# Perception4D/LidarSlam

Hardware: AMD Instinct MI355X
Metric: LiDAR frames/sec (AddFrame end-to-end), VLS-128 scan (higher is better)
Workload: dtype f32+f64; 1 GPU; VLS-128 synthetic spinning scan, street canyon, 5 m/s, EgoMotion=MOTION_EXTRAPOLATION_AND_REGISTRATION, Undistortion=REFINED, library defaults; points_per_frame=255802, sequences=1, parallelism=1 sequence per GPU x 1, frames_resident_in_hbm=False

## Files before the change

### include/lidarslam_amd.h

```cpp
#ifndef LIDARSLAM_AMD_H
#define LIDARSLAM_AMD_H

#include <stddef.h>
#include <stdint.h>

#ifdef __cplusplus
extern "C" {
#endif

#define LSA_OK 0
#define LSA_E_NO_DEVICE (-1)
#define LSA_E_HIP (-2)
#define LSA_E_ARG (-3)
#define LSA_E_STATE (-4)
#define LSA_E_CAPACITY (-5)
#define LSA_E_GATE (-6)

#define LSA_EDGE 0
#define LSA_PLANE 1
#define LSA_BLOB 2

typedef struct lsa_point_t
{
  float x, y, z, w;
// ... 151 lines not shown

int lsa_download_match(lsa_ctx* ctx, int type, uint8_t* status, double* weights, double* records, int capacity);
int lsa_upload_match(lsa_ctx* ctx, int type, const uint8_t* status, const double* records, int n, double saturation);
#define LSA_KNN_MAX 16
int lsa_download_knn(lsa_ctx* ctx, int type, int* idx, float* d2, int* cnt, int capacity);

int lsa_accumulate(lsa_ctx* ctx, unsigned type_mask, const double w[6], int want_jacobian, double* cost, double g[6],
                   double H[36], int* n_valid);
int lsa_mailbox_active(const lsa_ctx* ctx);

int lsa_solve(lsa_ctx* ctx, unsigned type_mask, const double prior[16], int lm_max_iter, int two_d_mode, double optimized[16],
              int summary[4], double costs[2]);
typedef struct lsa_solve_result
{
  double pose[6];
  double initial_cost, final_cost;
  double cost, g[6], H[36];
  int num_successful_steps;
  int num_unsuccessful_steps;
  int num_iterations;
  int num_evaluations;
  int num_matches;
  int skipped;
  int termination;
  const char* message;
} lsa_solve_result_t;
int lsa_solve_device(lsa_ctx* ctx, unsigned type_mask, const double prior[6], int two_d_mode, int lm_max_iter, int min_matches,
                     lsa_solve_result_t* out);
int lsa_solve_device_begin(lsa_ctx* ctx, unsigned type_mask, const double prior[6], int two_d_mode, int lm_max_iter, int min_matches);
int lsa_solve_device_end(lsa_ctx* ctx, lsa_solve_result_t* out);
int lsa_solve_device_drop(lsa_ctx* ctx);

int lsa_icp_gate(lsa_ctx* ctx);
int lsa_icp_post(lsa_ctx* ctx, int ticket, const double pose[16], const double prior[6], const double H0[16], const double H1[16], double t0, double t1);
int lsa_icp_cancel(lsa_ctx* ctx, int ticket);
int lsa_icp_abandon(lsa_ctx* ctx);
int lsa_match_types_gated(lsa_ctx* ctx, int slot, unsigned type_mask, int query_set, const lsa_match_params_t* p, int undistort);

typedef struct lsa_icp_link
{
  int refine_undistortion;
  int first;
  int have_log;
  double prev_time, cur_time;
  double max_extrapolation_ratio;
  double previous_world[16];
  double motion[16];
} lsa_icp_link_t;
int lsa_icp_link(lsa_ctx* ctx);
int lsa_solve_device_begin_linked(lsa_ctx* ctx, unsigned type_mask, const double prior[6], int two_d_mode, int lm_max_iter, int min_matches,
                                  int leave_ticket, const lsa_icp_link_t* link);
int lsa_icp_link_peek(lsa_ctx* ctx, int ticket, unsigned long long words[64]);
int lsa_icp_link_expected(const double x[6], int skipped, int successful_steps, const lsa_icp_link_t* link, unsigned long long words[64], double motion_after[16]);

int lsa_solve_device_trace(lsa_ctx* ctx, unsigned long long out[12]);
int lsa_debug_set(lsa_ctx* ctx, const char* name, int value);
int lsa_solve_device_shape(const lsa_ctx* ctx, int out[4]);
int lsa_accumulate_shape(const lsa_ctx* ctx, int out[4]);
int lsa_solve_device_fallbacks(const lsa_ctx* ctx);
int lsa_solve_device_interlude(lsa_ctx* ctx, void (*fn)(void*), void* arg);
int lsa_registration_error(lsa_ctx* ctx, unsigned type_mask, const double pose[16], int two_d_mode, double cov[36], double err[2]);

typedef struct lsa_sensor_terms_t
{
  int wheel;
  double wheel_weight;
  double p[3];
  double d;
  int gravity;
  double gravity_weight;
  double g_ref[3];
  double g_cur[3];
} lsa_sensor_terms_t;
int lsa_set_sensor_terms(lsa_ctx* ctx, const lsa_sensor_terms_t* terms);
int lsa_sensor_terms_eval(const lsa_sensor_terms_t* terms, const double w[6], double sums[29]);

typedef struct lsa_sensors lsa_sensors;
lsa_sensors* lsa_sensors_create(void);
void lsa_sensors_destroy(lsa_sensors* s);
int lsa_sensors_add_wheel_odom(lsa_sensors* s, double time, double distance);
int lsa_sensors_add_gravity(lsa_sensors* s, double time, const double acc[3]);
int lsa_sensors_set_weights(lsa_sensors* s, double wheel_weight, double gravity_weight);
int lsa_sensors_set_time_offset(lsa_sensors* s, double offset);
int lsa_sensors_clear(lsa_sensors* s);
int lsa_sensors_compute(lsa_sensors* s, double lidar_time, lsa_sensor_terms_t* out);
int lsa_sensors_gravity_ref(const lsa_sensors* s, double g[3]);


int lsa_reset_working_keypoints(lsa_ctx* ctx);

int lsa_undistort(lsa_ctx* ctx, const double H0[16], const double H1[16], double t0, double t1);

int lsa_localization_begin(lsa_ctx* ctx, const double H0[16], const double H1[16], double t0, double t1, const double box_pose[16]);
int lsa_arm_localization_boxes(lsa_ctx* ctx);

int lsa_working_time_range(lsa_ctx* ctx, double* tmin, double* tmax);
int lsa_keypoint_time_range(lsa_ctx* ctx, int set, double* tmin, double* tmax);
int lsa_working_bbox(lsa_ctx* ctx, int type, const double pose[16], float mn[3], float mx[3]);
int lsa_working_bboxes(lsa_ctx* ctx, const double pose[16], float mn[9], float mx[9]);
int lsa_keypoint_bboxes_begin(lsa_ctx* ctx, int set, const double pose[16]);
int lsa_keypoint_bboxes_begin_interp(lsa_ctx* ctx, int set, const double H0[16], const double H1[16], double t0, double t1);
int lsa_keypoint_bboxes_end(lsa_ctx* ctx, float mn[9], float mx[9]);
int lsa_keypoint_boxes_predicted_mark(lsa_ctx* ctx);
int lsa_keypoint_boxes_predicted(lsa_ctx* ctx, int set, const double H0[16], const double H1[16], double t0, double t1);

int lsa_download_transformed(lsa_ctx* ctx, int set, int type, const double pose[16], lsa_point_t* out, int capacity);
// ... 50 lines not shown
int lsa_slam_add_frames(lsa_slam* s, const lsa_point_t* const* pts, const int* n, const uint64_t* stamp_us, const uint32_t* seq, int nframes);
int lsa_slam_set_extractor_param(lsa_slam* s, int device_id, const char* name, double value);
int lsa_slam_get_extractor_param(const lsa_slam* s, int device_id, const char* name, double* value);
int lsa_slam_set_base_to_lidar_offset(lsa_slam* s, const double T[16], int device_id);
int lsa_slam_get_base_to_lidar_offset(const lsa_slam* s, double T[16], int device_id);
int lsa_slam_set_world_transform_from_guess(lsa_slam* s, const double T[16]);
int lsa_slam_get_trajectory(const lsa_slam* s, double* poses, double* covariances, int capacity);
int lsa_slam_get_debug_information(lsa_slam* s, double out[10]);
int lsa_slam_get_map(lsa_slam* s, int type, int clean, lsa_point_t* out, int capacity);
int lsa_slam_get_target_submap(lsa_slam* s, int type, lsa_point_t* out, int capacity);
lsa_ctx* lsa_slam_context(lsa_slam* s);
int lsa_slam_add_wheel_odom_measurement(lsa_slam* s, double time, double distance);
int lsa_slam_add_gravity_measurement(lsa_slam* s, double time, const double acc[3]);
int lsa_slam_clear_sensor_measurements(lsa_slam* s);
int lsa_slam_sensor_terms(const lsa_slam* s, lsa_sensor_terms_t* out);
int lsa_slam_add_map_points(lsa_slam* s, int type, const lsa_point_t* pts, int n, int fixed, double time);
int lsa_slam_save_maps_pcd(lsa_slam* s, const char* prefix, int format, int filtered);
int lsa_slam_load_maps_pcd(lsa_slam* s, const char* prefix, int reset_maps, double time);
int lsa_slam_map_io_counts(const lsa_slam* s, int counts[3]);
int lsa_slam_set_trajectory_and_rebuild_maps(lsa_slam* s, const double* poses17, int n);
int lsa_slam_logged_frames(const lsa_slam* s);
int lsa_slam_get_logged_keypoints(lsa_slam* s, int frame, int type, lsa_point_t* out, int capacity);


typedef struct lsa_device_grid lsa_device_grid;
int lsa_device_grid_create(lsa_ctx* ctx, lsa_device_grid** out);
void lsa_device_grid_destroy(lsa_device_grid* g);
int lsa_device_grid_set(lsa_device_grid* g, const char* name, double value);
double lsa_device_grid_get_param(const lsa_device_grid* g, const char* name);
int lsa_device_grid_reset(lsa_device_grid* g, const float position[3]);
int lsa_device_grid_clear(lsa_device_grid* g);
int lsa_device_grid_size(lsa_device_grid* g);
int lsa_device_grid_add(lsa_device_grid* g, const lsa_point_t* pts, int n, int fixed, double time, int roll);
int lsa_device_grid_add_keypoints(lsa_device_grid* g, int set, int type, const double pose[16], double time);
int lsa_device_grid_stage_keypoints(lsa_device_grid* g, int set, int type, const double pose[16]);
int lsa_device_grid_add_staged(lsa_device_grid* g, double time);
int lsa_device_grid_stage_keypoints_all(lsa_device_grid* const* grids, const int* types, int count, int set, const double pose[16]);
int lsa_device_grid_add_staged_all(lsa_device_grid* const* grids, int count, double time);
int lsa_device_grid_roll(lsa_device_grid* g, const float min_point[3], const float max_point[3]);
int lsa_device_grid_clear_old_points(lsa_device_grid* g, double current_time);
int lsa_device_grid_get(lsa_device_grid* g, int clean, lsa_point_t* out, int capacity);
int lsa_device_grid_build_submap(lsa_device_grid* g, const float min_point[3], const float max_point[3], int min_nb_points, int slot, int type);
int lsa_device_grid_build_submap_begin(lsa_device_grid* g, const float min_point[3], const float max_point[3], int min_nb_points, int slot, int type);
int lsa_device_grid_build_submap_begin_for_keypoints(lsa_device_grid* g, int box_type, int min_nb_points, int slot, int type);
int lsa_device_grid_build_submap_end(lsa_device_grid* g);
int lsa_device_grid_submap_valid(lsa_device_grid* g);
int lsa_device_grid_submap_ahead_begin(lsa_device_grid* g, int box_type, int min_nb_points, int type);
int lsa_device_grid_submap_ahead_poll(lsa_device_grid* g);
int lsa_device_grid_submap_ahead_poll_all(lsa_device_grid* const* grids, int count);
int lsa_device_grid_submap_ahead_wait(lsa_device_grid* g);
int lsa_device_grid_submap_ahead_take(lsa_device_grid* g, int box_type, int min_nb_points, int slot, int type, int* taken);
int lsa_device_grid_submap_ahead_take_begin(lsa_device_grid* g, int box_type, int min_nb_points, int slot, int type);
int lsa_device_grid_submap_ahead_take_end(lsa_device_grid* g, int* taken);
int lsa_device_grid_add_pcd(lsa_device_grid* g, const char* path, int fixed, double time, int roll_first);
int lsa_device_grid_save_pcd(lsa_device_grid* g, const char* path, int format, int clean);
int lsa_pcd_io_times(const lsa_ctx* ctx, double out[8]);

int lsa_kplog_append(lsa_ctx* ctx);
int lsa_kplog_append_points(lsa_ctx* ctx, const lsa_point_t* const pts[3], const int n[3]);
int lsa_kplog_pop_front(lsa_ctx* ctx);
int lsa_kplog_clear(lsa_ctx* ctx);
int lsa_kplog_size(const lsa_ctx* ctx);
int lsa_kplog_count(const lsa_ctx* ctx, int frame, int type);
int lsa_kplog_get(lsa_ctx* ctx, int frame, int type, lsa_point_t* out, int capacity);
unsigned long long lsa_kplog_bytes(const lsa_ctx* ctx);
int lsa_kplog_stopped(const lsa_ctx* ctx);
int lsa_kplog_replay(lsa_ctx* ctx, unsigned type_mask, const double* poses, const double* times, int n, int undistort, lsa_point_t* const out[3],
                     float last_min[3][3], float last_max[3][3]);
long long lsa_kplog_replayed(const lsa_ctx* ctx, int type, const lsa_point_t** pts);
int lsa_kplog_replay_to_grids(lsa_ctx* ctx, unsigned type_mask, const double* poses, const double* times, int n, int undistort, lsa_device_grid* const grids[3],
                              float last_min[3][3], float last_max[3][3]);

typedef struct lsa_rolling_grid lsa_rolling_grid;
lsa_rolling_grid* lsa_rolling_grid_create(void);
void lsa_rolling_grid_destroy(lsa_rolling_grid* g);
int lsa_rolling_grid_set(lsa_rolling_grid* g, const char* name, double value);
void lsa_rolling_grid_reset(lsa_rolling_grid* g, const float position[3]);
void lsa_rolling_grid_clear(lsa_rolling_grid* g);
int lsa_rolling_grid_size(const lsa_rolling_grid* g);
void lsa_rolling_grid_roll(lsa_rolling_grid* g, const float min_point[3], const float max_point[3]);
int lsa_rolling_grid_add(lsa_rolling_grid* g, const lsa_point_t* pts, int n, int fixed, double current_time, int roll);
void lsa_rolling_grid_clear_old_points(lsa_rolling_grid* g, double current_time);
int lsa_rolling_grid_get(const lsa_rolling_grid* g, int clean, lsa_point_t* out, int capacity);
int lsa_rolling_grid_build_submap(lsa_rolling_grid* g, const float min_point[3], const float max_point[3], int min_nb_points);
int lsa_rolling_grid_submap_valid(const lsa_rolling_grid* g);
int lsa_rolling_grid_submap(const lsa_rolling_grid* g, lsa_point_t* out, int capacity);

int lsa_pcd_info(const char* path, int* n, int* format);
int lsa_pcd_read(const char* path, lsa_point_t* out, int capacity);
int lsa_pcd_write(const char* path, const lsa_point_t* pts, int n, int format);
const char* lsa_pcd_last_error(void);
int lsa_lzf_compress(const void* in, size_t n, void* out, size_t capacity, size_t* written);
int lsa_lzf_decompress(const void* in, size_t n, void* out, size_t capacity, size_t* written);

int lsa_synth_sensor(int model, int* nrings, int* ncols, double* el_min_deg, double* el_max_deg);
int lsa_synth_frame(int model, uint64_t seed, int frame, lsa_point_t* out, int capacity, uint64_t* stamp_us);
void lsa_synth_pose(int frame, double T[16]);

#ifdef __cplusplus
}
#endif
#endif
```

### lidarslam_amd/__init__.py

```python
import ctypes as C
import os

import numpy as np

from ._native import (
    BLOB,
    EDGE,
    LIB_PATH,
    MATCH_NSTATUS,
    PLANE,
    POINT_DTYPE,
    SET_RAW_CURRENT,
    SET_RAW_PREVIOUS,
    SET_WORKING,
    ExtractParams,
    KernelStat,
    MatchParams,
    pose16,
    ptr,
    synth_frame,
    synth_pose,
)

__all__ = ["Context", "Slam", "ExtractParams", "MatchParams", "POINT_DTYPE", "lib", "LsaError", "read_pcd", "write_pcd"]

TARGET_MAP, TARGET_PREVIOUS = 0, 1
KNN_MAX = 16

DEBUG_INFORMATION_NAMES = [
    "EgoMotion: edges used", "EgoMotion: planes used", "Localization: edges used", "Localization: planes used",
    "Localization: blobs used", "Localization: position error", "Localization: orientation error",
    "Confidence: overlap", "Confidence: comply motion limits", "latency",
]

DEBUG_NAMES = [
    "sin_angle", "saliency", "depth_gap", "intensity_gap", "edge_keypoint", "plane_keypoint", "blob_keypoint",
    "edge_validity", "plane_validity", "blob_validity",
]

ABI_SYMBOLS = [
    "lsa_device_count", "lsa_bind_host_to_device", "lsa_ctx_create", "lsa_ctx_destroy", "lsa_last_error", "lsa_sync", "lsa_upload_frame", "lsa_upload_wire_frame", "lsa_upload_polydata_frame",
    "lsa_frame_store_put", "lsa_frame_store_use", "lsa_frame_size", "lsa_get_azimuthal_resolution",
    "lsa_set_azimuthal_resolution", "lsa_extract_keypoints", "lsa_extract_keypoints_more", "lsa_extract_prefetch", "lsa_extract_prefetch_adopted", "lsa_transform_frame_at", "lsa_set_keypoint_types", "lsa_download_keypoints", "lsa_keypoint_count",
    "lsa_download_debug", "lsa_nb_laser_rings", "lsa_transform_keypoints", "lsa_set_target", "lsa_set_target_from_set", "lsa_prepare_previous_targets", "lsa_prepared_targets_adopted", "lsa_target_staging", "lsa_set_target_staged", "lsa_stage_target_ahead", "lsa_drop_target_ahead", "lsa_staged_targets_adopted",
    "lsa_target_size", "lsa_download_target", "lsa_set_target_cell_size", "lsa_set_knn_lanes", "lsa_set_fused_match", "lsa_set_knn_rounds", "lsa_match_slow_queries", "lsa_match_exhaustive_queries", "lsa_match_route_stats", "lsa_match_trace", "lsa_set_keypoints", "lsa_match", "lsa_match_types", "lsa_match_types_undistorted",
    "lsa_download_match", "lsa_upload_match", "lsa_download_knn", "lsa_overlap", "lsa_accumulate", "lsa_mailbox_active", "lsa_solve", "lsa_solve_device", "lsa_solve_device_fallbacks", "lsa_solve_device_begin", "lsa_solve_device_end", "lsa_solve_device_drop", "lsa_icp_gate", "lsa_icp_link", "lsa_solve_device_begin_linked", "lsa_icp_link_peek", "lsa_icp_link_expected", "lsa_icp_post", "lsa_icp_cancel", "lsa_icp_abandon", "lsa_debug_set", "lsa_solve_device_shape", "lsa_accumulate_shape", "lsa_match_types_gated", "lsa_solve_device_trace", "lsa_registration_error", "lsa_selftest_math", "lsa_selftest_numerics", "lsa_selftest_labels", "lsa_reset_working_keypoints", "lsa_undistort", "lsa_working_time_range",
    "lsa_working_bbox", "lsa_working_bboxes", "lsa_localization_begin", "lsa_arm_localization_boxes", "lsa_keypoint_bboxes_begin", "lsa_keypoint_bboxes_begin_interp", "lsa_keypoint_boxes_predicted_mark", "lsa_keypoint_boxes_predicted", "lsa_keypoint_time_range", "lsa_keypoint_bboxes_end", "lsa_download_transformed", "lsa_stage_transformed", "lsa_staged_transformed", "lsa_transform_frame", "lsa_profile_enable", "lsa_profile_select", "lsa_profile_reset",
    "lsa_profile_get", "lsa_slam_create", "lsa_slam_destroy", "lsa_slam_last_error", "lsa_slam_set_param",
    "lsa_slam_get_param", "lsa_slam_reset", "lsa_slam_clear_maps", "lsa_slam_add_frame", "lsa_slam_store_frame", "lsa_slam_add_stored_frame", "lsa_slam_hint_next_stored_frame", "lsa_slam_hint_next_frame", "lsa_upload_frame_begin", "lsa_upload_frame_ready", "lsa_upload_frame_adopt", "lsa_upload_frame_forget", "lsa_profile_event_overhead_us", "lsa_upload_robosense_frame", "lsa_pin_host_memory", "lsa_unpin_host_memory", "lsa_collect_garbage", "lsa_uploads_adopted", "lsa_extract_prefetch_uploaded",
    "lsa_slam_get_world_transform", "lsa_slam_get_covariance", "lsa_slam_get_keypoints", "lsa_slam_get_registered_frame",
    "lsa_slam_get_match_status", "lsa_slam_get_stats", "lsa_slam_context", "lsa_slam_get_latency_compensated_world_transform",
    "lsa_slam_set_world_transform_from_guess", "lsa_slam_get_trajectory", "lsa_slam_get_debug_information", "lsa_slam_get_map",
    "lsa_slam_get_target_submap", "lsa_slam_set_base_to_lidar_offset", "lsa_slam_get_base_to_lidar_offset", "lsa_slam_add_frames", "lsa_slam_set_extractor_param", "lsa_slam_get_extractor_param", "lsa_match_serial", "lsa_match_histogram", "lsa_synth_sensor", "lsa_synth_frame",
    "lsa_synth_pose",
    "lsa_selftest_keep_busy", "lsa_solve_device_interlude", "lsa_device_grid_create", "lsa_device_grid_destroy", "lsa_device_grid_set", "lsa_device_grid_get_param", "lsa_device_grid_reset", "lsa_device_grid_clear",
    "lsa_device_grid_size", "lsa_device_grid_add", "lsa_device_grid_add_keypoints", "lsa_device_grid_roll", "lsa_device_grid_clear_old_points",
    "lsa_device_grid_get", "lsa_device_grid_build_submap", "lsa_device_grid_submap_valid", "lsa_device_grid_stage_keypoints", "lsa_device_grid_stage_keypoints_all", "lsa_device_grid_add_staged", "lsa_device_grid_add_staged_all",
    "lsa_device_grid_build_submap_begin", "lsa_device_grid_build_submap_begin_for_keypoints", "lsa_device_grid_build_submap_end",
    "lsa_device_grid_submap_ahead_begin", "lsa_device_grid_submap_ahead_poll", "lsa_device_grid_submap_ahead_poll_all", "lsa_device_grid_submap_ahead_wait", "lsa_device_grid_submap_ahead_take", "lsa_device_grid_submap_ahead_take_begin", "lsa_device_grid_submap_ahead_take_end",
    "lsa_rolling_grid_create", "lsa_rolling_grid_destroy", "lsa_rolling_grid_set", "lsa_rolling_grid_reset", "lsa_rolling_grid_clear",
    "lsa_rolling_grid_size", "lsa_rolling_grid_roll", "lsa_rolling_grid_add", "lsa_rolling_grid_clear_old_points", "lsa_rolling_grid_get",
    "lsa_rolling_grid_build_submap", "lsa_rolling_grid_submap_valid", "lsa_rolling_grid_submap",
    "lsa_set_sensor_terms", "lsa_sensor_terms_eval", "lsa_sensors_create", "lsa_sensors_destroy", "lsa_sensors_add_wheel_odom",
    "lsa_sensors_add_gravity", "lsa_sensors_set_weights", "lsa_sensors_set_time_offset", "lsa_sensors_clear", "lsa_sensors_compute",
    "lsa_sensors_gravity_ref", "lsa_slam_add_wheel_odom_measurement", "lsa_slam_add_gravity_measurement",
    "lsa_slam_clear_sensor_measurements", "lsa_slam_sensor_terms",
    "lsa_pcd_info", "lsa_pcd_read", "lsa_pcd_write", "lsa_pcd_last_error", "lsa_lzf_compress", "lsa_lzf_decompress",
    "lsa_device_grid_add_pcd", "lsa_device_grid_save_pcd", "lsa_pcd_io_times",
    "lsa_slam_add_map_points", "lsa_slam_save_maps_pcd", "lsa_slam_load_maps_pcd", "lsa_slam_map_io_counts",
    "lsa_kplog_append", "lsa_kplog_append_points", "lsa_kplog_pop_front", "lsa_kplog_clear", "lsa_kplog_size", "lsa_kplog_count", "lsa_kplog_get",
    "lsa_kplog_bytes", "lsa_kplog_stopped", "lsa_kplog_replay", "lsa_kplog_replayed", "lsa_kplog_replay_to_grids",
    "lsa_slam_set_trajectory_and_rebuild_maps", "lsa_slam_logged_frames", "lsa_slam_get_logged_keypoints",
]

PCD_ASCII, PCD_BINARY, PCD_BINARY_COMPRESSED = 0, 1, 2
PCD_FORMAT_NAMES = ["ascii", "binary", "binary_compressed"]


class LsaError(RuntimeError):
    code = None


E_NO_DEVICE, E_HIP, E_ARG, E_STATE, E_CAPACITY = -1, -2, -3, -4, -5


def _error(what, rc, message):
    e = LsaError(f"{what} failed ({rc}): {message}")
    e.code = rc
    return e


class IcpLink(C.Structure):

    _fields_ = [
        ("refine_undistortion", C.c_int), ("first", C.c_int), ("have_log", C.c_int),
        ("prev_time", C.c_double), ("cur_time", C.c_double), ("max_extrapolation_ratio", C.c_double),
        ("previous_world", C.c_double * 16), ("motion", C.c_double * 16),
    ]

# ... 1241 lines not shown
```

### lidarslam_amd/csrc/host/lsa_slam_core.cpp

```cpp
#include "lsa_slam_core.h"
#include <algorithm>
#include <chrono>
#include <cmath>
#include <cstdlib>
#include <cstdio>
#include <cstring>
#include <ctime>
#include "lsa_pcd.h"

namespace lsa
{
namespace host
{
constexpr unsigned kChainMax = 6;
namespace
{
#define ICP_TRACE(...) do { if (lsa_icp_trace_on()) std::fprintf(stderr, __VA_ARGS__); } while (0)
struct Tick
{
  std::chrono::steady_clock::time_point t0 = std::chrono::steady_clock::now();
  double Stop() const { return std::chrono::duration<double>(std::chrono::steady_clock::now() - t0).count(); }
};
inline double StampToSec(uint64_t us) { return us * 1e-6; }
}
// ... 529 lines not shown
  return lsa_prepare_previous_targets(Ctx, (1u << LSA_EDGE) | (1u << LSA_PLANE));
}

lsa_match_params_t SlamCore::EgoMatchParams() const
{
  lsa_match_params_t p;
  std::memset(&p, 0, sizeof(p));
  p.single_edge_per_ring = 1;
  p.max_neighbors_distance = EgoMotionMaxNeighborsDistance;
  p.edge_nb_neighbors = EgoMotionEdgeNbNeighbors;
  p.edge_min_nb_neighbors = EgoMotionEdgeMinNbNeighbors;
  p.edge_max_model_error = EgoMotionEdgeMaxModelError;
  p.plane_nb_neighbors = EgoMotionPlaneNbNeighbors;
  p.planarity_threshold = EgoMotionPlanarityThreshold;
  p.plane_max_model_error = EgoMotionPlaneMaxModelError;
  p.blob_nb_neighbors = 10;
  p.saturation_distance = 1.;
  return p;
}
lsa_match_params_t SlamCore::LocMatchParams() const
{
  lsa_match_params_t p;
  std::memset(&p, 0, sizeof(p));
  p.single_edge_per_ring = 0;
  p.max_neighbors_distance = LocalizationMaxNeighborsDistance;
  p.edge_nb_neighbors = LocalizationEdgeNbNeighbors;
  p.edge_min_nb_neighbors = LocalizationEdgeMinNbNeighbors;
  p.edge_max_model_error = LocalizationEdgeMaxModelError;
  p.plane_nb_neighbors = LocalizationPlaneNbNeighbors;
  p.planarity_threshold = LocalizationPlanarityThreshold;
  p.plane_max_model_error = LocalizationPlaneMaxModelError;
  p.blob_nb_neighbors = LocalizationBlobNbNeighbors;
  p.saturation_distance = 1.;
  return p;
}

struct SlamCore::IcpLoopSpec
{
  const char* name;
  int target, set;
  unsigned matchMask, solveMask;
  unsigned maxIter, lmMaxIter;
  double initSaturation, finalSaturation;
  lsa_match_params_t match;
  int loopBit;
  bool linksOk, gatesOk;
  int undistortAhead;
  lsa_icp_link_t link;
  long long* matchSerial;
  double FrameStats::*icpSeconds;
  double FrameStats::*lmSeconds;
  int FrameStats::*iterations;
  bool countSkippedEvals;
};
struct SlamCore::IcpUndistortion
{
  Pose d0 = Pose::Identity(), d1 = Pose::Identity();
  bool pending = false;
  bool posted = false;
};

namespace
{
constexpr auto kNothing = [](auto&&...) { return LSA_OK; };
const bool kAheadWithHostMaps = std::getenv("LSA_ICP_AHEAD_HOSTMAPS") != nullptr;
const int kAheadLoops = std::getenv("LSA_ICP_AHEAD_LOOPS") ? std::atoi(std::getenv("LSA_ICP_AHEAD_LOOPS")) : 3;
const bool kGateDebug = std::getenv("LSA_GATE_DEBUG") != nullptr;
}

template <class Top, class Enqueued, class Solved, class Skipped, class Accepted, class Finished>
int SlamCore::RunIcpLoop(const IcpLoopSpec& spec, Pose& pose, const Top& top, const Enqueued& enqueued, const Solved& solved, const Skipped& skipped,
                         const Accepted& accepted, const Finished& finished)
{
  TotalMatchedKeypoints = 0;
  lsa_match_params_t mp = spec.match;
  auto saturation = [&](unsigned icpIter) {
    const double iterRatio = icpIter / static_cast<double>(spec.maxIter - 1);
    return (1 - iterRatio) * spec.initSaturation + iterRatio * spec.finalSaturation;
  };
  const bool aheadOk = ICPAhead >= 1 && DeviceLM && FusedMatch && (kAheadLoops & spec.loopBit);
  bool chain = aheadOk && ICPAhead >= 2 && spec.maxIter <= kChainMax && spec.linksOk;
  bool ahead = aheadOk && !chain && spec.gatesOk;
  if (ahead || chain) lsa_icp_abandon(Ctx);
  unsigned chained = 0;
  long long chainSerial[kChainMax][3] = {};
  bool enqueuedAhead = false;
  long long aheadSerial[3] = {0, 0, 0};
  int ticket = -1;
  IcpUndistortion undistortion;
  unsigned icpIter = 0;

  auto callOffRest = [&](bool all) {
    if (ticket >= 0)
    {
      lsa_icp_cancel(Ctx, ticket);
      lsa_solve_device_drop(Ctx);
      ticket = -1;
    }
    if (all || icpIter + 1 < chained)
    {
      lsa_icp_abandon(Ctx);
      chained = 0;
    }
  };
  struct AtExit { decltype(callOffRest)& callOffRest; bool failed; ~AtExit() { callOffRest(failed); } } atExit{callOffRest, true};

  auto takeSerials = [&](long long* serial) {
    for (int k = 0; k < 3; ++k)
      if ((spec.matchMask >> k) & 1u) serial[k] = lsa_match_serial(Ctx, k);
  };
  auto setSerials = [&](const long long* serial) {
    for (int k = 0; k < 3; ++k)
      if ((spec.matchMask >> k) & 1u) spec.matchSerial[k] = serial[k];
  };
  auto matchInLine = [&]() -> int {
    if (undistortion.pending)
      LSA_TRY(lsa_match_types_undistorted(Ctx, spec.target, spec.matchMask, &mp, pose.m, nullptr, undistortion.d0.m, undistortion.d1.m, Motion.Time0, Motion.Time1));
    else
      LSA_TRY(lsa_match_types(Ctx, spec.target, spec.matchMask, spec.set, &mp, pose.m, nullptr));
    undistortion.pending = false;
    takeSerials(spec.matchSerial);
    return LSA_OK;
  };
  auto matchAhead = [&](unsigned iter, long long* serial) -> int {
    lsa_match_params_t next = mp;
    next.saturation_distance = saturation(iter);
    const int rc = lsa_match_types_gated(Ctx, spec.target, spec.matchMask, spec.set, &next, spec.undistortAhead);
    if (rc == 0) takeSerials(serial);
    return rc;
  };

  for (; icpIter < spec.maxIter; ++icpIter)
  {
    Tick ticp;
    if (const int rc = top(icpIter); rc < 0) return rc;
    mp.saturation_distance = saturation(icpIter);
    LocalOptimizer optimizer(Ctx);
    optimizer.SetDeviceLoop(DeviceLM);
    optimizer.SetTwoDMode(TwoDMode);
    optimizer.SetLMMaxIter(spec.lmMaxIter);
    optimizer.SetMinMatches(MinNbMatchedKeypoints);
    optimizer.UseDeviceResiduals(spec.solveMask);
    optimizer.SetPosePrior(pose);
    bool begun = enqueuedAhead;
    if (icpIter < chained)
    {
      begun = true;
      setSerials(chainSerial[icpIter]);
    }
    else if (!enqueuedAhead)
    {
      if (const int rc = matchInLine(); rc < 0) return rc;
      if (chain)
      {
        double prior[6];
        ToXYZRPY(pose, prior);
        lsa_icp_link_t link = spec.link;
        for (unsigned j = icpIter; j < spec.maxIter; ++j)
        {
          int leave = j + 1 < spec.maxIter ? lsa_icp_link(Ctx) : -1;
          if (leave < 0) leave = -1;
          link.first = j == icpIter ? 1 : 0;
          const int rc = lsa_solve_device_begin_linked(Ctx, spec.solveMask, j == icpIter ? prior : nullptr, TwoDMode ? 1 : 0, static_cast<int>(spec.lmMaxIter), static_cast<int>(MinNbMatchedKeypoints), leave,
                                                       leave >= 0 ? &link : nullptr);
          if (rc < 0) return Fail(rc, "lsa_solve_device_begin_linked");
          chained = j + 1;
          if (leave < 0) break;
          const int mrc = matchAhead(j + 1, chainSerial[j + 1]);
          if (mrc < 0) return Fail(mrc, "lsa_match_types_gated");
          if (mrc != 0) { lsa_icp_cancel(Ctx, leave); break; }
        }
        chain = false;
        begun = true;
      }
      else if (ahead)
      {
        LSA_TRY(optimizer.Begin(false));
        begun = true;
      }
    }
    else
      setSerials(aheadSerial);
    ICP_TRACE("[%s %u] top: ahead %d begun %d enqueued %d\n", spec.name, icpIter, (int)ahead, (int)begun, (int)enqueuedAhead);
    enqueuedAhead = false;
    if (ahead && begun && icpIter + 1 < spec.maxIter)
    {
      ticket = lsa_icp_gate(Ctx);
      ICP_TRACE("[%s %u] gate ticket %d\n", spec.name, icpIter, ticket);
      if (ticket < 0) { ticket = -1; ahead = false; }
      else
      {
        const char* call = "lsa_match_types_gated";
        int rc = matchAhead(icpIter + 1, aheadSerial);
        if (rc == 0)
        {
          call = "lsa_solve_device_begin";
          rc = lsa_solve_device_begin(Ctx, spec.solveMask, nullptr, TwoDMode ? 1 : 0, static_cast<int>(spec.lmMaxIter), static_cast<int>(MinNbMatchedKeypoints));
        }
        if (rc != 0)
        {
          lsa_icp_cancel(Ctx, ticket);
          ticket = -1;
          ahead = false;
          if (rc < 0) return Fail(rc, call);
        }
      }
    }
    if (const int rc = enqueued(icpIter); rc < 0) return rc;
    if (!begun) ArmLookaheadInterlude();
    Stats.*spec.icpSeconds += ticp.Stop();
    (Stats.*spec.iterations)++;

    Tick tlm;
    SolveSummary summary;
    if (begun)
    {
      Tick tdbg;
      const int irc = InterludeWork();
      const double dbgInterlude = tdbg.Stop();
      int rc = optimizer.End(summary);
      ICP_TRACE("[%s %u] End rc %d irc %d ticket %d\n", spec.name, icpIter, rc, irc, ticket);
      if (kGateDebug && tdbg.Stop() > 0.01)
        std::fprintf(stderr, "[gate debug] %s iteration %u: enqueue %.3f ms, interlude %.3f ms, until the result %.3f ms, rc %d\n", spec.name, icpIter, 1e3 * Stats.*spec.icpSeconds, 1e3 * dbgInterlude,
                     1e3 * tdbg.Stop(), rc);
      if (rc == LSA_E_GATE)
      {
        callOffRest(true);
        ahead = false;
        IcpGateTimeouts++;
        undistortion.pending = undistortion.posted;
        rc = matchInLine();
        if (rc < 0) return rc;
        rc = optimizer.Solve(summary);
      }
      if (rc < 0) return Fail(rc, "LocalOptimizer::End / Solve");
      if (rc == 1) { ticket = -1; ahead = false; chained = 0; }
      if (irc < 0) return irc;
    }
    else
    {
      LSA_TRY(optimizer.Solve(summary));
      LSA_TRY(FinishLookaheadInterlude());
    }
    TotalMatchedKeypoints = summary.num_matches;
    if (lsa_icp_trace_on())
      std::fprintf(stderr, "[icp] frame %u %s %u: matches %d evals %d steps %d cost %.17g -> %.17g%s\n", NbrFrameProcessed, spec.name, icpIter, summary.num_matches, summary.num_evaluations,
                   summary.num_successful_steps, summary.initial_cost, summary.final_cost, summary.skipped ? " skipped" : "");
    if (const int rc = solved(); rc < 0) return rc;
    if (!summary.skipped || spec.countSkippedEvals) Stats.lm_evals += summary.num_evaluations;
    if (!summary.skipped) pose = optimizer.GetOptimizedPose();
    const bool last = summary.skipped || summary.num_successful_steps == 1 || icpIter + 1 == spec.maxIter;
    if (last) callOffRest(false);
    const int rc = summary.skipped ? skipped() : accepted(last, undistortion);
    Stats.*spec.lmSeconds += tlm.Stop();
    if (rc < 0) return rc;
    if (last)
    {
      if (const int frc = summary.skipped ? LSA_OK : finished(optimizer); frc < 0) return frc;
      break;
    }
    if (ticket >= 0)
    {
      double prior[6];
      ToXYZRPY(pose, prior);
      const int prc = lsa_icp_post(Ctx, ticket, pose.m, prior, undistortion.pending ? undistortion.d0.m : nullptr, undistortion.pending ? undistortion.d1.m : nullptr, Motion.Time0, Motion.Time1);
      if (prc < 0) return Fail(prc, "lsa_icp_post");
      ticket = -1;
      undistortion.posted = undistortion.pending;
      undistortion.pending = false;
      enqueuedAhead = true;
    }
    else if (icpIter + 1 < chained)
      undistortion.pending = false;
  }
  atExit.failed = false;
  return LSA_OK;
}

int SlamCore::DownloadMatchDebug(int set, unsigned typeMask, MatchDebug* debug)
{
  for (int k = 0; k < 3; ++k)
  {
    if (!((typeMask >> k) & 1u)) continue;
    const int n = lsa_keypoint_count(Ctx, set, k);
    debug[k].status.assign(n, LSA_MATCH_UNKOWN);
    debug[k].weights.assign(n, 0.);
    if (n > 0) LSA_TRY(lsa_download_match(Ctx, k, debug[k].status.data(), debug[k].weights.data(), nullptr, n));
  }
  return LSA_OK;
}

int SlamCore::ComputeEgoMotion()
{
  Tick tpre;
  Trelative = Pose::Identity();
  if (AheadStatus < 0) { const int rc = AheadStatus; AheadStatus = 0; return Fail(rc, "lsa_prepare_previous_targets (look-ahead thread)"); }
  if (LogTrajectory.size() >= 2 &&
      (EgoMotion == EgoMotionMode::MOTION_EXTRAPOLATION || EgoMotion == EgoMotionMode::MOTION_EXTRAPOLATION_AND_REGISTRATION))
  {
    const double t = StampToSec(CurrentStamp);
    const double t1 = LogTrajectory[LogTrajectory.size() - 1].time;
    const double t0 = LogTrajectory[LogTrajectory.size() - 2].time;
    if (!(std::abs((t - t1) / (t1 - t0)) > MaxExtrapolationRatio))
    {
      const Pose next = LinearInterpolation(PreviousTworld, Tworld, t, t0, t1);
      Trelative = Inverse(Tworld) * next;
    }
  }
  const bool registers = EgoMotion == EgoMotionMode::REGISTRATION || EgoMotion == EgoMotionMode::MOTION_EXTRAPOLATION_AND_REGISTRATION;
  {
    const int rc = BeginSubMapSpeculation(Tworld * Trelative);
    if (rc < 0) return rc;
    HoldLookahead = false;
  }
  if (!registers) return LSA_OK;

  for (int k : {LSA_EDGE, LSA_PLANE})
  {
    lsa_set_target_cell_size(Ctx, LSA_TARGET_PREVIOUS, k, static_cast<float>(k == LSA_EDGE ? KnnCellSizeEgoMotionEdges : KnnCellSizeEgoMotion));
    LSA_TRY(lsa_set_target_from_set(Ctx, LSA_TARGET_PREVIOUS, k, LSA_SET_RAW_PREVIOUS));
  }
  IcpLoopSpec spec = {};
  spec.name = "ego";
  spec.target = LSA_TARGET_PREVIOUS;
  spec.set = LSA_SET_RAW_CURRENT;
  spec.matchMask = spec.solveMask = (1u << LSA_EDGE) | (1u << LSA_PLANE);
  spec.maxIter = EgoMotionICPMaxIter;
  spec.lmMaxIter = EgoMotionLMMaxIter;
  spec.initSaturation = EgoMotionInitSaturationDistance;
  spec.finalSaturation = EgoMotionFinalSaturationDistance;
  spec.match = EgoMatchParams();
  spec.loopBit = 1;
  spec.linksOk = true;
  spec.gatesOk = DeviceMapsInUse() || MapUpdate == MappingMode::NONE || kAheadWithHostMaps;
  spec.matchSerial = EgoMatchSerial;
  spec.icpSeconds = &FrameStats::ego_icp;
  spec.lmSeconds = &FrameStats::ego_lm;
  spec.iterations = &FrameStats::ego_iters;
  spec.countSkippedEvals = true;
  auto enqueued = [&](unsigned icpIter) -> int {
    if (icpIter == 0 && BuildTargetsAhead)
    {
      AheadStatus = 0;
      AheadWorker.Submit([this] { AheadStatus = PrepareNextEgoMotionTargets(); });
    }
    if (!SpecPending) LSA_TRY(StageSpeculativeSubMaps());
    return LSA_OK;
  };
  auto solved = [&]() -> int { return SpecPending ? FinishSubMapSpeculation() : LSA_OK; };
  DbgAcc[2] += tpre.Stop();
  if (const int rc = RunIcpLoop(spec, Trelative, kNothing, enqueued, solved, kNothing, kNothing, kNothing); rc < 0) return rc;
  if (KeepMatchDebug) return DownloadMatchDebug(LSA_SET_RAW_CURRENT, spec.matchMask, EgoDebug);
  return LSA_OK;
}

int SlamCore::Localization()
{
  Tick tloc;
  struct AtExit { SlamCore* c; Tick* t; ~AtExit() { c->DbgAcc[5] += t->Stop() - (c->Stats.loc_icp + c->Stats.loc_lm + c->Stats.submap + c->Stats.undistort); } } atExit{this, &tloc};
  const bool sensorTerms = LocSensorTerms.wheel || LocSensorTerms.gravity;
  if (sensorTerms) lsa_set_sensor_terms(Ctx, &LocSensorTerms);
  struct SensorTermsGuard { lsa_ctx* ctx; bool on; ~SensorTermsGuard() { if (on) lsa_set_sensor_terms(ctx, nullptr); } } sensorGuard{Ctx, sensorTerms};
  PreviousTworld = Tworld;
  Tworld = PreviousTworld * Trelative;
  const bool oneLaunch = LocalizationStartFused && DeviceMapsInUse() && MapUpdate != MappingMode::NONE;
  bool boxesEnqueued = false;
  if (oneLaunch)
  {
    Tick t;
    Pose d0 = Pose::Identity(), d1 = Pose::Identity();
    if (Undistortion)
    {
      double t0, t1;
      LSA_TRY(lsa_keypoint_time_range(Ctx, LSA_SET_RAW_CURRENT, &t0, &t1));
      InitUndistortion(t0, t1);
      RefineUndistortion(&d0, &d1);
    }
    LSA_TRY(lsa_localization_begin(Ctx, Undistortion ? d0.m : nullptr, Undistortion ? d1.m : nullptr, Motion.Time0, Motion.Time1, Tworld.m));
    boxesEnqueued = true;
    Stats.undistort += t.Stop();
  }
  else
  {
    LSA_TRY(lsa_reset_working_keypoints(Ctx));
    if (Undistortion)
    {
      Tick t;
      int rc = InitUndistortion();
      if (rc < 0) return rc;
      rc = RefineUndistortion();
      if (rc < 0) return rc;
      Stats.undistort += t.Stop();
    }
  }

  if (DeviceMapsInUse())
  {
    Tick t;
    for (auto& w : MapWorker) w.Wait();
    {
      Tick tw;
      while (DevSpecRunning.load(std::memory_order_acquire)) std::this_thread::yield();
      const bool tried = DevSpec[0] || DevSpec[1] || DevSpec[2];
      if (tried && SubMapsAheadAdaptive && tw.Stop() > 80e-6)
      {
        DevSpecGood = 0;
        if (++DevSpecLate >= 2)
        {
          DevSpecBackoff = DevSpecPenalty;
          DevSpecPenalty = std::min(2 * DevSpecPenalty, 64);
          DevSpecLate = 0;
        }
      }
      else if (tried)
      {
        DevSpecLate = 0;
        if (++DevSpecGood >= 8) DevSpecPenalty = 4;
      }
    }
    Stats.maps_wait = t.Stop();
    if (DevSpecStatus < 0) { const int rc = DevSpecStatus; DevSpecStatus = 0; return Fail(rc, "sub-maps ahead of time (look-ahead thread)"); }
    Stats.maps_async = std::max(MapJobSeconds[0], std::max(MapJobSeconds[1], MapJobSeconds[2]));
    for (int k = 0; k < 3; ++k)
      if (MapJobFailed[k]) { MapJobFailed[k] = 0; return Fail(LSA_E_HIP, "lsa_device_grid_add_staged (map worker)"); }
    bool need[3], checking[3] = {false, false, false}, any = false;
    for (int k = 0; k < 3; ++k)
    {
      need[k] = UseKeypoints[k] && !lsa_device_grid_submap_valid(DevMaps[k]);
      any = any || need[k];
    }
    if (any && MapUpdate != MappingMode::NONE && !boxesEnqueued) LSA_TRY(lsa_keypoint_bboxes_begin(Ctx, LSA_SET_WORKING, Tworld.m));
    for (int k = 0; k < 3; ++k)
    {
      if (!need[k]) continue;
      lsa_set_target_cell_size(Ctx, LSA_TARGET_MAP, k, static_cast<float>((k == LSA_EDGE ? KnnCellScaleMapsEdges : KnnCellScaleMaps) * LocalMaps[k]->GetLeafSize()));
      if (MapUpdate == MappingMode::NONE) LSA_TRY(lsa_device_grid_build_submap_begin(DevMaps[k], nullptr, nullptr, -1, LSA_TARGET_MAP, k));
      else
      {
        if (DevSpec[k] && lsa_device_grid_submap_ahead_take_begin(DevMaps[k], k, KeypointCounts[k] / 2, LSA_TARGET_MAP, k) == 1) { checking[k] = true; continue; }
        if (LocalMaps[k]->IsTimeThreshold()) LSA_TRY(lsa_device_grid_clear_old_points(DevMaps[k], CurrentTime));
        LSA_TRY(lsa_device_grid_build_submap_begin_for_keypoints(DevMaps[k], k, KeypointCounts[k] / 2, LSA_TARGET_MAP, k));
      }
    }
    for (int k = 0; k < 3; ++k)
    {
      if (!checking[k]) continue;
      int taken = 0;
      LSA_TRY(lsa_device_grid_submap_ahead_take_end(DevMaps[k], &taken));
      if (taken) { need[k] = false; Stats.submap_spec_hits++; SubMapSpecHitsTotal++; continue; }
      if (LocalMaps[k]->IsTimeThreshold()) LSA_TRY(lsa_device_grid_clear_old_points(DevMaps[k], CurrentTime));
      LSA_TRY(lsa_device_grid_build_submap_begin_for_keypoints(DevMaps[k], k, KeypointCounts[k] / 2, LSA_TARGET_MAP, k));
    }
    for (bool& b : DevSpec) b = false;
    for (int k = 0; k < 3; ++k)
      if (need[k]) LSA_TRY(lsa_device_grid_build_submap_end(DevMaps[k]));
    Stats.submap += t.Stop();
    HoldLookahead = false;
  }
  else
  {
    Tick t;
    if (SpecPending)
    {
      const int rc = FinishSubMapSpeculation();
      if (rc < 0) return rc;
    }
    WaitMaps();
    Stats.maps_wait = t.Stop();
    Stats.maps_async = std::max(MapJobSeconds[0], std::max(MapJobSeconds[1], MapJobSeconds[2]));
    bool fresh[3], rebuild[3] = {false, false, false};
    bool any = false;
    for (int k = 0; k < 3; ++k)
    {
      fresh[k] = UseKeypoints[k] && SpecBuilt[k];
      rebuild[k] = UseKeypoints[k] && !fresh[k] && !LocalMaps[k]->IsSubMapValid();
      any = any || fresh[k] || rebuild[k];
      SpecBuilt[k] = false;
    }
    float mn[9], mx[9];
    if (any && MapUpdate != MappingMode::NONE) LSA_TRY(lsa_working_bboxes(Ctx, Tworld.m, mn, mx));
    for (int k = 0; k < 3; ++k)
    {
      const bool holds = fresh[k] && MapUpdate != MappingMode::NONE && LocalMaps[k]->SubMapBuiltFor(mn + 3 * k, mx + 3 * k, KeypointCounts[k] / 2);
      if (SpecStaged[k] && !holds) LSA_TRY(lsa_drop_target_ahead(Ctx, LSA_TARGET_MAP, k));
      SpecStaged[k] = false;
      SpecDone[k].store(false);
    }
    for (int k = 0; k < 3; ++k)
    {
      if (!fresh[k] && !rebuild[k]) continue;
      RollingGrid* map = LocalMaps[k].get();
      const int minPts = KeypointCounts[k] / 2;
      if (fresh[k])
      {
        if (map->SubMapBuiltFor(mn + 3 * k, mx + 3 * k, minPts)) { Stats.submap_spec_hits++; SubMapSpecHitsTotal++; rebuild[k] = true; continue; }
        rebuild[k] = true;
      }

      if (MapUpdate == MappingMode::NONE)
        MapWorker[k].Submit([map] { map->BuildSubMap(); });
      else
      {
        const bool clear = map->IsTimeThreshold();
        const double now = CurrentTime;
        const float* lo3 = mn + 3 * k;
        const float* hi3 = mx + 3 * k;
        MapWorker[k].Submit([map, clear, now, minPts, mn0 = lo3[0], mn1 = lo3[1], mn2 = lo3[2], mx0 = hi3[0], mx1 = hi3[1], mx2 = hi3[2]] {
          if (clear) map->ClearOldPoints(now);
          const float lo[3] = {mn0, mn1, mn2}, hi[3] = {mx0, mx1, mx2};
          map->BuildSubMap(lo, hi, minPts);
        });
      }
    }
    for (int k = 0; k < 3; ++k)
    {
      if (!rebuild[k]) continue;
      MapWorker[k].Wait();
      lsa_set_target_cell_size(Ctx, LSA_TARGET_MAP, k, static_cast<float>((k == LSA_EDGE ? KnnCellScaleMapsEdges : KnnCellScaleMaps) * LocalMaps[k]->GetLeafSize()));
      LSA_TRY(lsa_set_target_staged(Ctx, LSA_TARGET_MAP, k, static_cast<int>(LocalMaps[k]->SubMapSize())));
    }
    Stats.submap += t.Stop();
  }

  const bool refined = Undistortion == UNDISTORTION_REFINED;
  IcpLoopSpec spec = {};
  spec.name = "loc";
  spec.target = LSA_TARGET_MAP;
  spec.set = LSA_SET_WORKING;
  for (int k = 0; k < 3; ++k)
    if (UseKeypoints[k]) spec.matchMask |= 1u << k;
  spec.solveMask = 7u;
  spec.maxIter = LocalizationICPMaxIter;
  spec.lmMaxIter = LocalizationLMMaxIter;
  spec.initSaturation = LocalizationInitSaturationDistance;
  spec.finalSaturation = LocalizationFinalSaturationDistance;
  spec.match = LocMatchParams();
  spec.loopBit = 2;
  spec.linksOk = spec.gatesOk = !refined || UndistortInSearch;
  spec.undistortAhead = refined ? 1 : 0;
  spec.link.refine_undistortion = refined ? 1 : 0;
  spec.link.have_log = LogTrajectory.empty() ? 0 : 1;
  spec.link.prev_time = LogTrajectory.empty() ? 0. : LogTrajectory.back().time;
  spec.link.cur_time = StampToSec(CurrentStamp);
  spec.link.max_extrapolation_ratio = MaxExtrapolationRatio;
  std::memcpy(spec.link.previous_world, PreviousTworld.m, sizeof(spec.link.previous_world));
  {
    double* m = spec.link.motion;
    m[0] = Motion.Time0; m[1] = Motion.Time1;
    m[2] = Motion.Rot0.w; m[3] = Motion.Rot0.x; m[4] = Motion.Rot0.y; m[5] = Motion.Rot0.z;
    m[6] = Motion.Rot1.w; m[7] = Motion.Rot1.x; m[8] = Motion.Rot1.y; m[9] = Motion.Rot1.z;
    for (int i = 0; i < 3; ++i) { m[10 + i] = Motion.Trans0[i]; m[13 + i] = Motion.Trans1[i]; }
  }
  spec.matchSerial = LocMatchSerial;
  spec.icpSeconds = &FrameStats::loc_icp;
  spec.lmSeconds = &FrameStats::loc_lm;
  spec.iterations = &FrameStats::loc_iters;
  spec.countSkippedEvals = false;
  auto top = [&](unsigned icpIter) -> int {
    if (WorkerPrewake && DeviceMapsInUse() && icpIter + 1 == LocalizationICPMaxIter && MapUpdate != MappingMode::NONE) MapWorker[0].Expect(300e-6);
    return LSA_OK;
  };
  auto skipped = [&]() -> int {
    Trelative = Pose::Identity();
    Tworld = PreviousTworld;
    if (Undistortion) Motion.SetTransforms(Pose::Identity(), Pose::Identity());
    LastError = "Not enough keypoints matched, Localization skipped for this frame.";
    return LSA_OK;
  };
  auto accepted = [&](bool last, IcpUndistortion& undistortion) -> int {
    Trelative = Inverse(PreviousTworld) * Tworld;
    if (!refined) return LSA_OK;
    if (UndistortInSearch && !last)
    {
      undistortion.pending = true;
      return RefineUndistortion(&undistortion.d0, &undistortion.d1);
    }
    return RefineUndistortion();
  };
  auto finished = [&](LocalOptimizer& optimizer) -> int {
    Tick terr;
    LSA_TRY(optimizer.EstimateRegistrationError(LocalizationUncertainty));
    DbgAcc[4] += terr.Stop();
    return LSA_OK;
  };
  if (const int rc = RunIcpLoop(spec, Tworld, top, kNothing, kNothing, skipped, accepted, finished); rc < 0) return rc;
  if (KeepMatchDebug) return DownloadMatchDebug(LSA_SET_WORKING, 7u, LocDebug);
  return LSA_OK;
}

int SlamCore::BeginSubMapSpeculation(const Pose& predicted)
{
  SpecPending = false;
  for (bool& b : DevSpec) b = false;
  if (MapUpdate == MappingMode::NONE) return LSA_OK;
  const bool onDevice = DeviceMapsInUse();
  if (onDevice)
  {
    bool any = false;
    for (int k = 0; k < 3; ++k) any = any || (UseKeypoints[k] && KeypointCounts[k] > 0);
    if (!SubMapsAhead || !any || LocalMaps[0]->IsTimeThreshold()) return LSA_OK;
    if (DevSpecBackoff > 0) { --DevSpecBackoff; return LSA_OK; }
  }
  bool interpolated = false;
  Pose begin = predicted, end = predicted;
  double t0 = 0., t1 = 0.;
  if (Undistortion && !LogTrajectory.empty())
  {
    LSA_TRY(lsa_keypoint_time_range(Ctx, LSA_SET_RAW_CURRENT, &t0, &t1));
    const double prevPoseTime = LogTrajectory.back().time;
    const double currPoseTime = StampToSec(CurrentStamp);
    if (t1 - t0 >= 1e-6 && currPoseTime != prevPoseTime)
    {
      auto scanPose = [&](double time) {
        if (std::abs(time / (currPoseTime - prevPoseTime)) > MaxExtrapolationRatio) return predicted;
        return LinearInterpolation(Tworld, predicted, currPoseTime + time, prevPoseTime, currPoseTime);
      };
      begin = scanPose(t0);
      end = scanPose(t1);
      interpolated = true;
    }
  }
  if (onDevice)
  {
    int minPts[3];
    bool use[3];
    for (int k = 0; k < 3; ++k)
    {
      use[k] = UseKeypoints[k] && KeypointCounts[k] > 0;
      minPts[k] = KeypointCounts[k] / 2;
      if (use[k]) lsa_set_target_cell_size(Ctx, LSA_TARGET_MAP, k, static_cast<float>((k == LSA_EDGE ? KnnCellScaleMapsEdges : KnnCellScaleMaps) * LocalMaps[k]->GetLeafSize()));
      DevSpec[k] = use[k];
    }
    DevSpecStatus = 0;
    LSA_TRY(lsa_keypoint_boxes_predicted_mark(Ctx));
    DevSpecRunning.store(true, std::memory_order_release);
    AheadWorker.Submit([this, interpolated, begin, end, t0, t1, use0 = use[0], use1 = use[1], use2 = use[2], m0 = minPts[0], m1 = minPts[1], m2 = minPts[2]] {
      const bool use[3] = {use0, use1, use2};
      const int minPts[3] = {m0, m1, m2};
      for (auto& w : MapWorker) w.Wait();
// ... 506 lines not shown
  if (!HaveFrame) return 0;
  if (!CurrentFrames.empty())
  {
    size_t total = 0;
    for (const HeldFrame& f : CurrentFrames) total += static_cast<size_t>(f.n);
    out.resize(total);
    size_t at = 0;
    for (const HeldFrame& f : CurrentFrames)
    {
      LSA_TRY(lsa_frame_store_use(Ctx, f.slot));
      const Pose offset = GetBaseToLidarOffset(f.device);
      if (Undistortion)
      {
        const Pose H0 = (Tworld * Motion.GetH0()) * offset;
        const Pose H1 = (Tworld * Motion.GetH1()) * offset;
        LSA_TRY(lsa_transform_frame_at(Ctx, 1, H0.m, H1.m, Motion.Time0, Motion.Time1, f.timeOffset, out.data() + at, f.n));
      }
      else
      {
        const Pose tf = Tworld * offset;
        LSA_TRY(lsa_transform_frame_at(Ctx, 0, tf.m, nullptr, 0., 0., f.timeOffset, out.data() + at, f.n));
      }
      at += static_cast<size_t>(f.n);
    }
    return static_cast<int>(total);
  }
  const int n = lsa_frame_size(Ctx);
  if (n <= 0) return 0;
  out.resize(n);
  if (Undistortion)
  {
    const Pose H0 = (Tworld * Motion.GetH0()) * BaseToLidarOffset;
    const Pose H1 = (Tworld * Motion.GetH1()) * BaseToLidarOffset;
    LSA_TRY(lsa_transform_frame(Ctx, 1, H0.m, H1.m, Motion.Time0, Motion.Time1, out.data(), n));
  }
  else
  {
    const Pose tf = Tworld * BaseToLidarOffset;
    LSA_TRY(lsa_transform_frame(Ctx, 0, tf.m, nullptr, 0., 0., out.data(), n));
  }
  return n;
}

#define LSA_PARAMS(X)                                                                                   \
  X("UseBlobs", UseKeypoints[LSA_BLOB], bool)                                                          \
  X("UseEdges", UseKeypoints[LSA_EDGE], bool)                                                          \
  X("UsePlanes", UseKeypoints[LSA_PLANE], bool)                                                        \
  X("TwoDMode", TwoDMode, bool)                                                                        \
  X("BuildTargetsAhead", BuildTargetsAhead, bool)                                                      \
  X("DeviceLM", DeviceLM, bool)                                                                        \
  X("MapsOnDevice", MapsOnDevice, bool)                                                                \
  X("SubMapsAhead", SubMapsAhead, bool)                                                                \
  X("SubMapsAheadAdaptive", SubMapsAheadAdaptive, bool)                                                \
  X("LocalizationStartFused", LocalizationStartFused, bool)                                            \
  X("WorkerPrewake", WorkerPrewake, bool)                                                              \
  X("ICPAhead", ICPAhead, int)                                                                         \
  X("UndistortInSearch", UndistortInSearch, bool)                                                      \
  X("SpecBoxesOnLookahead", SpecBoxesOnLookahead, bool)                                                \
  X("SpecGridsTogether", SpecGridsTogether, bool)                                                      \
  X("FusedMatch", FusedMatch, bool)                                                                    \
  X("EgoMotionICPMaxIter", EgoMotionICPMaxIter, unsigned)                                              \
  X("LocalizationICPMaxIter", LocalizationICPMaxIter, unsigned)                                        \
  X("EgoMotionLMMaxIter", EgoMotionLMMaxIter, unsigned)                                                \
  X("LocalizationLMMaxIter", LocalizationLMMaxIter, unsigned)                                          \
  X("EgoMotionMaxNeighborsDistance", EgoMotionMaxNeighborsDistance, double)                            \
  X("LocalizationMaxNeighborsDistance", LocalizationMaxNeighborsDistance, double)                      \
  X("EgoMotionEdgeNbNeighbors", EgoMotionEdgeNbNeighbors, unsigned)                                    \
  X("EgoMotionEdgeMinNbNeighbors", EgoMotionEdgeMinNbNeighbors, unsigned)                              \
  X("EgoMotionEdgeMaxModelError", EgoMotionEdgeMaxModelError, double)                                  \
  X("EgoMotionPlaneNbNeighbors", EgoMotionPlaneNbNeighbors, unsigned)                                  \
  X("EgoMotionPlanarityThreshold", EgoMotionPlanarityThreshold, double)                                \
  X("EgoMotionPlaneMaxModelError", EgoMotionPlaneMaxModelError, double)                                \
  X("EgoMotionInitSaturationDistance", EgoMotionInitSaturationDistance, double)                        \
  X("EgoMotionFinalSaturationDistance", EgoMotionFinalSaturationDistance, double)                      \
  X("LocalizationEdgeNbNeighbors", LocalizationEdgeNbNeighbors, unsigned)                              \
  X("LocalizationEdgeMinNbNeighbors", LocalizationEdgeMinNbNeighbors, unsigned)                        \
  X("LocalizationEdgeMaxModelError", LocalizationEdgeMaxModelError, double)                            \
  X("LocalizationPlaneNbNeighbors", LocalizationPlaneNbNeighbors, unsigned)                            \
  X("LocalizationPlanarityThreshold", LocalizationPlanarityThreshold, double)                          \
  X("LocalizationPlaneMaxModelError", LocalizationPlaneMaxModelError, double)                          \
  X("LocalizationBlobNbNeighbors", LocalizationBlobNbNeighbors, unsigned)                              \
  X("LocalizationInitSaturationDistance", LocalizationInitSaturationDistance, double)                  \
  X("LocalizationFinalSaturationDistance", LocalizationFinalSaturationDistance, double)                \
  X("MaxExtrapolationRatio", MaxExtrapolationRatio, double)                                            \
  X("MinNbMatchedKeypoints", MinNbMatchedKeypoints, unsigned)                                          \
  X("KfDistanceThreshold", KfDistanceThreshold, double)                                                \
  X("KfAngleThreshold", KfAngleThreshold, double)                                                      \
  X("KeepMatchDebug", KeepMatchDebug, bool)                                                            \
  X("KnnCellSizeEgoMotion", KnnCellSizeEgoMotion, double)                                              \
  X("KnnCellScaleMaps", KnnCellScaleMaps, double)                                                      \
  X("KnnCellSizeEgoMotionEdges", KnnCellSizeEgoMotionEdges, double)                                    \
  X("KnnCellScaleMapsEdges", KnnCellScaleMapsEdges, double)                                            \
  X("KnnLanesEdges", KnnLanesEdges, int)                                                               \
  X("KnnLanesPlanes", KnnLanesPlanes, int)                                                             \
  X("KnnLanesBlobs", KnnLanesBlobs, int)                                                               \
  X("KnnRoundsEdges", KnnRoundsEdges, int)                                                             \
  X("KnnRoundsPlanes", KnnRoundsPlanes, int)                                                           \
  X("KnnRoundsBlobs", KnnRoundsBlobs, int)                                                             \
  X("NeighborWidth", ExtractParams.neighbor_width, int)                                                \
  X("MinDistanceToSensor", ExtractParams.min_distance_to_sensor, float)                                \
  X("MinBeamSurfaceAngle", ExtractParams.min_beam_surface_angle, float)                                \
  X("PlaneSinAngleThreshold", ExtractParams.plane_sin_angle_threshold, float)                          \
  X("EdgeSinAngleThreshold", ExtractParams.edge_sin_angle_threshold, float)                            \
  X("DistToLineThreshold", ExtractParams.dist_to_line_threshold, float)                                \
  X("EdgeDepthGapThreshold", ExtractParams.edge_depth_gap_threshold, float)                            \
  X("EdgeSaliencyThreshold", ExtractParams.edge_saliency_threshold, float)                             \
// ... 76 lines not shown
  auto dev = [&](int k, const char* what, double value) { if (DevMaps[k]) lsa_device_grid_set(DevMaps[k], what, value); };
  if (name == "VoxelGridLeafSizeEdges") { LocalMaps[LSA_EDGE]->SetLeafSize(v); dev(LSA_EDGE, "LeafSize", v); return LSA_OK; }
  if (name == "VoxelGridLeafSizePlanes") { LocalMaps[LSA_PLANE]->SetLeafSize(v); dev(LSA_PLANE, "LeafSize", v); return LSA_OK; }
  if (name == "VoxelGridLeafSizeBlobs") { LocalMaps[LSA_BLOB]->SetLeafSize(v); dev(LSA_BLOB, "LeafSize", v); return LSA_OK; }
  if (name == "VoxelGridSize") { for (int k = 0; k < 3; ++k) { LocalMaps[k]->SetGridSize(static_cast<int>(v)); dev(k, "GridSize", v); } return LSA_OK; }
  if (name == "VoxelGridResolution") { for (int k = 0; k < 3; ++k) { LocalMaps[k]->SetVoxelResolution(v); dev(k, "VoxelResolution", v); } return LSA_OK; }
  if (name == "VoxelGridMinFramesPerVoxel") { for (int k = 0; k < 3; ++k) { LocalMaps[k]->SetMinFramesPerVoxel(static_cast<unsigned>(v)); dev(k, "MinFramesPerVoxel", v); } return LSA_OK; }
  if (name == "VoxelGridDecayingThreshold") { for (int k = 0; k < 3; ++k) { LocalMaps[k]->SetDecayingThreshold(v); dev(k, "DecayingThreshold", v); } return LSA_OK; }
  if (name == "VoxelGridSamplingMode") { for (int k = 0; k < 3; ++k) { LocalMaps[k]->SetSampling(static_cast<SamplingMode>(static_cast<int>(v))); dev(k, "Sampling", v); } return LSA_OK; }
  if (name == "OrderedMaps")
  {
    OrderedMaps = v != 0;
    for (auto& m : LocalMaps) m->SetOrdered(OrderedMaps);
    for (int k = 0; k < 3; ++k)
      if (DevMaps[k] && lsa_device_grid_set(DevMaps[k], "Ordered", OrderedMaps ? 1. : 0.) != LSA_OK) return Fail(LSA_E_HIP, "lsa_device_grid_set(Ordered)");
    return LSA_OK;
  }
  LastError = "unknown parameter " + name;
  return LSA_E_ARG;
}

int SlamCore::GetParam(const std::string& name, double* v) const
{
  if (!v) return LSA_E_ARG;
#define X(NAME, MEMBER, TYPE) if (name == NAME) { *v = static_cast<double>(MEMBER); return LSA_OK; }
  LSA_PARAMS(X)
#undef X
  if (name == "EgoMotion") { *v = static_cast<int>(EgoMotion); return LSA_OK; }
  if (name == "Undistortion") { *v = static_cast<int>(Undistortion); return LSA_OK; }
  if (name == "MapUpdate") { *v = static_cast<int>(MapUpdate); return LSA_OK; }
  if (name == "WheelOdomWeight") { *v = SensorManagers.GetWheelOdomWeight(); return LSA_OK; }
  if (name == "GravityWeight") { *v = SensorManagers.GetGravityWeight(); return LSA_OK; }
  if (name == "SensorTimeOffset") { *v = SensorManagers.GetTimeOffset(); return LSA_OK; }
  if (name == "AzimuthalResolution") { *v = Ctx ? lsa_get_azimuthal_resolution(Ctx) : 0.; return LSA_OK; }
  if (name == "VoxelGridLeafSizeEdges") { *v = LocalMaps[LSA_EDGE]->GetLeafSize(); return LSA_OK; }
  if (name == "VoxelGridLeafSizePlanes") { *v = LocalMaps[LSA_PLANE]->GetLeafSize(); return LSA_OK; }
  if (name == "VoxelGridLeafSizeBlobs") { *v = LocalMaps[LSA_BLOB]->GetLeafSize(); return LSA_OK; }
  if (name == "VoxelGridSize") { *v = LocalMaps[0]->GetGridSize(); return LSA_OK; }
  if (name == "VoxelGridResolution") { *v = LocalMaps[0]->GetVoxelResolution(); return LSA_OK; }
  if (name == "VoxelGridSamplingMode") { *v = static_cast<int>(LocalMaps[0]->GetSampling()); return LSA_OK; }
  if (name == "VoxelGridDecayingThreshold") { *v = LocalMaps[0]->GetDecayingThreshold(); return LSA_OK; }
  if (name == "VoxelGridMinFramesPerVoxel") { *v = LocalMaps[0]->GetMinFramesPerVoxel(); return LSA_OK; }
  if (name == "NbrFrameProcessed") { *v = NbrFrameProcessed; return LSA_OK; }
  if (name == "TotalMatchedKeypoints") { *v = TotalMatchedKeypoints; return LSA_OK; }
  if (name == "OverlapSamplingRatio") { *v = OverlapSamplingRatio; return LSA_OK; }
  if (name == "OverlapEstimation") { *v = OverlapEstimation; return LSA_OK; }
  if (name == "SubMapSpeculationHits") { *v = SubMapSpecHitsTotal; return LSA_OK; }
  if (name == "LookaheadAdopted") { *v = Ctx ? lsa_extract_prefetch_adopted(Ctx) : 0; return LSA_OK; }
  if (name == "OrderedMaps") { *v = OrderedMaps ? 1. : 0.; return LSA_OK; }
  if (name == "DeviceMapsInUse") { *v = DeviceMapsInUse() ? 1. : 0.; return LSA_OK; }
  if (name == "UploadsAdopted") { *v = Ctx ? lsa_uploads_adopted(Ctx) : 0; return LSA_OK; }
  if (name == "DeviceSolveFallbacks") { *v = Ctx ? lsa_solve_device_fallbacks(Ctx) : 0; return LSA_OK; }
  if (name == "IcpGateTimeouts") { *v = IcpGateTimeouts; return LSA_OK; }
  if (name == "TargetsBuiltAheadAdopted") { *v = Ctx ? lsa_prepared_targets_adopted(Ctx) : 0; return LSA_OK; }
  if (name == "SubMapsStagedAheadAdopted") { *v = Ctx ? lsa_staged_targets_adopted(Ctx) : 0; return LSA_OK; }
  if (name == "MapAddThreads") { *v = LocalMaps[LSA_PLANE]->GetAddThreads(); return LSA_OK; }
  if (name == "MapAddThreadsEdges") { *v = LocalMaps[LSA_EDGE]->GetAddThreads(); return LSA_OK; }
  if (name == "LoggingTimeout") { *v = LoggingTimeout; return LSA_OK; }
  if (name == "LoggingStorage") { *v = LoggingStorage; return LSA_OK; }
  if (name == "LoggedKeypointsBytes") { *v = Ctx ? static_cast<double>(lsa_kplog_bytes(Ctx)) : 0.; return LSA_OK; }
  if (name == "LoggedFrames") { *v = LoggedFrames(); return LSA_OK; }
  if (name == "TimeWindowDuration") { *v = TimeWindowDuration; return LSA_OK; }
  if (name == "VelocityLimitLinear") { *v = VelocityLimits[0]; return LSA_OK; }
  if (name == "VelocityLimitAngular") { *v = VelocityLimits[1]; return LSA_OK; }
  if (name == "AccelerationLimitLinear") { *v = AccelerationLimits[0]; return LSA_OK; }
  if (name == "AccelerationLimitAngular") { *v = AccelerationLimits[1]; return LSA_OK; }
  if (name == "ComplyMotionLimits") { *v = ComplyMotionLimits ? 1. : 0.; return LSA_OK; }
  if (name == "Latency") { *v = Latency; return LSA_OK; }
  return LSA_E_ARG;
}

}
}
```

### lidarslam_amd/csrc/host/lsa_slam_core.h

```cpp
#pragma once
#include <array>
#include <atomic>
#include <condition_variable>
#include <deque>
#include <limits>
#include <map>
#include <functional>
#include <memory>
#include <mutex>
#include <string>
#include <thread>
#include <vector>
#include "../../../include/lidarslam_amd.h"
#include "lsa_hostmath.h"
#include "lsa_lm.h"
#include "lsa_rolling_grid.h"
#include "lsa_sensor_constraints.h"

namespace lsa
{
namespace host
{

enum UndistortionMode { UNDISTORTION_NONE = 0, UNDISTORTION_ONCE = 1, UNDISTORTION_REFINED = 2 };
// ... 126 lines not shown
  float OverlapSamplingRatio = 0.f;
  float OverlapEstimation = -1.f;
  float VelocityLimits[2] = {std::numeric_limits<float>::max(), std::numeric_limits<float>::max()};
  float AccelerationLimits[2] = {std::numeric_limits<float>::max(), std::numeric_limits<float>::max()};
  float TimeWindowDuration = 0.f;
  bool ComplyMotionLimits = true;
  double LoggingTimeout = 0.;
  int LoggingStorage = 0;
  double Latency = 0.;
  Pose BaseToLidarOffset = Pose::Identity();
  lsa_extract_params_t ExtractParams;
  struct DeviceExtractor
  {
    lsa_extract_params_t params;
    float azimuthalResolution = 0.f;
  };
  std::map<int, DeviceExtractor> OtherExtractors;
  std::map<int, Pose> OtherBaseToLidarOffsets;
  double KnnCellSizeEgoMotion = 0.25;
  double KnnCellSizeEgoMotionEdges = 0.5;
  double KnnCellScaleMaps = 1.0;
  double KnnCellScaleMapsEdges = 2.5;
  int KnnLanesEdges = 16, KnnLanesPlanes = 8, KnnLanesBlobs = 8;
  int KnnRoundsEdges = 2, KnnRoundsPlanes = 2, KnnRoundsBlobs = 2;
  bool BuildTargetsAhead = true;
  bool DeviceLM = true;
  bool FusedMatch = true;
  bool KeepMatchDebug = false;

  std::shared_ptr<RollingGrid> LocalMaps[3];
  lsa_device_grid* DevMaps[3] = {nullptr, nullptr, nullptr};
  bool MapsOnDevice = true;
  bool SubMapsAhead = true;
  bool SubMapsAheadAdaptive = true;
  bool LocalizationStartFused = true;
  int IcpGateTimeouts = 0;
  int ICPAhead = 2;
  bool UndistortInSearch = true;
  bool SpecBoxesOnLookahead = true;
  bool SpecGridsTogether = true;
  bool DevSpec[3] = {false, false, false};
  bool OrderedMaps = true;
  bool DeviceMapsInUse() const { return MapsOnDevice && DevMaps[0]; }
  int MigrateMaps(bool fromDevice);
  int SetParamValue(const std::string& name, double v);
  int GetMap(int k, bool clean, std::vector<lsa_point_t>& out);
  int GetTargetSubMap(int k, std::vector<lsa_point_t>& out);

  Pose Tworld, PreviousTworld, Trelative;
  RegistrationError LocalizationUncertainty;
  unsigned TotalMatchedKeypoints = 0;
  unsigned NbrFrameProcessed = 0;
  unsigned SubMapSpecHitsTotal = 0;
  int KfCounter = 0;
  FrameStats Stats;
  std::deque<StampedPose> LogTrajectory;
  std::deque<std::array<double, 36>> LogCovariances;
  int KeypointCounts[3] = {0, 0, 0};

private:
  int ProcessCurrentFrame(uint64_t stampUs);
  int ExtractKeypoints();
  int ComputeEgoMotion();
  int Localization();
  struct IcpLoopSpec;
  struct IcpUndistortion;
  template <class Top, class Enqueued, class Solved, class Skipped, class Accepted, class Finished>
  int RunIcpLoop(const IcpLoopSpec& spec, Pose& pose, const Top& top, const Enqueued& enqueued, const Solved& solved, const Skipped& skipped,
                 const Accepted& accepted, const Finished& finished);
  int DownloadMatchDebug(int set, unsigned typeMask, MatchDebug* debug);
  SensorConstraints SensorManagers;
  lsa_sensor_terms_t LocSensorTerms = {};
  int UpdateMapsUsingTworld();
  int EstimateOverlap();
  void CheckMotionLimits();
  float PreviousVelocity[2] = {0.f, 0.f};
  long long EgoMatchSerial[3] = {0, 0, 0}, LocMatchSerial[3] = {0, 0, 0};
  void LogCurrentFrameState(double time);
  bool KpLogStopped = false;
  Pose InterpolateScanPose(double time) const;
  int InitUndistortion();
  void InitUndistortion(double t0, double t1);
  int RefineUndistortion(Pose* outD0 = nullptr, Pose* outD1 = nullptr);
  int Fail(int rc, const char* where);
  lsa_match_params_t EgoMatchParams() const;
  lsa_match_params_t LocMatchParams() const;

  struct HeldFrame
  {
    int slot;
    int n;
    int device;
    double timeOffset;
  };
  std::vector<HeldFrame> CurrentFrames;
  float Device0AzimuthalResolution = 0.f;
  int ExtractFrames();
  int PrepareNextEgoMotionTargets();
  void ArmLookaheadInterlude();
  int InterludeWork();
  int DevSpecStatus = 0;
  std::atomic<bool> DevSpecRunning{false};
  int DevSpecBackoff = 0;
  int DevSpecLate = 0;
  int DevSpecGood = 0, DevSpecPenalty = 4;
  int FinishLookaheadInterlude();
// ... 37 lines not shown
```

### lidarslam_amd/csrc/lsa_ctx.h

```cpp
#pragma once
#include <hip/hip_runtime.h>
#include <cstdint>
#include <cstdio>
#include <cstdlib>
#include <cstring>
#include <string>
#include <atomic>
#include <condition_variable>
#include <deque>
#include <mutex>
#include <thread>
#include <vector>
#include "../../include/lidarslam_amd.h"

namespace lsa
{

constexpr int kMaxRings = 512;
constexpr int kMaxRingPoints = 8192;
constexpr int kBucketChunk = 1024;
constexpr int kGridLevels = 3;
constexpr int kCellCap = 1 << 22;
__host__ __device__ constexpr int grid_level_cells(int level) { return level == 0 ? kCellCap : level == 1 ? (kCellCap >> 6) + 64 : (kCellCap >> 12) + 64; }
constexpr int kKnnMax = 16;
constexpr int kAccumBlocks = 96;
constexpr int kAccumBlocksMax = 256;
constexpr int kMailboxStride = 64;
constexpr int kLmBlocksMax = 128;
constexpr int kLmBlocks = 64;
constexpr int kLmThreads = 512;
constexpr int kLmOut = 48;
constexpr int kLmMailRing = 8;
constexpr int kHistRing = 256;
constexpr int kAccumVals = 29;
constexpr int kGateRing = 8;
constexpr int kGateWords = 64;
constexpr int kGateGranules = 128;

struct GridDesc
{
  float origin[3];
  float cell;
  float inv_cell;
  int dims[3];
  int ncells;
  int npoints;
};

struct GridLevel
{
  float4* sorted = nullptr;
  uint32_t* cell_of = nullptr;
  uint32_t* cell_start = nullptr;
  uint32_t* cell_fill = nullptr;
  uint32_t* block_sums = nullptr;
  int max_cells = 0;
};

struct Target
{
  lsa_point_t* pts = nullptr;
  float4* xyzl = nullptr;
  GridLevel lv[kGridLevels];
  GridDesc* desc = nullptr;
  int* bbox_bits = nullptr;
  int m = 0;
  int cap = 0;
  float cell_hint = 1.0f;
  bool dirty = false;
};

struct MatchBuf
{
  double* rec = nullptr;
  uint8_t* status = nullptr;
  int* knn_idx = nullptr;
  float* knn_d2 = nullptr;
  int* knn_cnt = nullptr;
  int* slow_list = nullptr;
  float4* slow_pts = nullptr;
  int k = 0;
  int knn_n = 0;
  int knn_k = 0;
  int cap = 0;
  double sat = 1.0;
  bool valid = false;
};

struct FrameInbox
// ... 69 lines not shown
  int* extract_out_next = nullptr;
  int* host_next = nullptr;
  bool prefetch_pending = false;
  int prefetch_adopted = 0;
  const lsa_point_t* prefetch_frame = nullptr;
  int prefetch_n = 0;
  lsa_extract_params_t prefetch_params{};
  float prefetch_az = 0.f;
  unsigned prefetch_mask = 0;
  int* ring_meta = nullptr;
  float* score[4] = {nullptr, nullptr, nullptr, nullptr};
  uint8_t* valid = nullptr;
  uint8_t* label = nullptr;
  int* ring_counts = nullptr;
  int* kp_count_dev = nullptr;
  unsigned kp_type_mask = 7;

  lsa_point_t* kp[3][3] = {};
  int kp_n[3][3] = {};
  double kp_time[3][2] = {};
  bool kp_time_valid[3] = {false, false, false};

  lsa_point_t* tstage[6] = {};
  int tstage_cap[6] = {};
  lsa::Target target[12];
  bool map_ahead_ready[3] = {false, false, false};
  int map_ahead_adopted = 0;
  hipEvent_t ev_map_ahead[3] = {nullptr, nullptr, nullptr};
  unsigned long long kp_clock = 0;
  unsigned long long kp_ver[3][3] = {{0, 0, 0}, {0, 0, 0}, {0, 0, 0}};
  unsigned long long spare_ver[3] = {0, 0, 0};
  bool spare_ready[3] = {false, false, false};
  int spare_adopted = 0;
  hipEvent_t ev_spare = nullptr, ev_kp_ready = nullptr;
  lsa::MatchBuf match[3];

  int accum_blocks = lsa::kAccumBlocks;
  double* partials = nullptr;
  double* reduce_out = nullptr;
  double* host_pinned = nullptr;
  unsigned long long* mailbox = nullptr;
  unsigned long long mailbox_seq = 0;
  bool mailbox_check = false;
  unsigned long long* lm_xchg = nullptr;
  unsigned long long* lm_mailbox = nullptr;
  unsigned lm_tag = 0;
  unsigned long long lm_seq = 0;
  int lm_blocks = lsa::kLmBlocks;
  unsigned long long* gate_host = nullptr;
  unsigned long long* gate_dev = nullptr;
  unsigned gate_seq = 0;
  int gate_current = -1;
  struct GateSaved { double sat[3]; int hist_pos[3]; long long hist_serial[3]; int k[3]; bool valid[3]; unsigned mask; bool used; bool link; unsigned seq; } gate_saved[lsa::kGateRing] = {};
  double* motion_dev = nullptr;
  int debug_gate_give_up_every = 0;
  int debug_lm_give_up_block = -1;
  std::deque<unsigned> lm_pending;
  std::deque<int> lm_pending_wait;
  hipStream_t map_stream = nullptr;
  int map_stream_users = 0;
  void (*solve_hook)(void*) = nullptr;
  void* solve_hook_arg = nullptr;
  int lm_records = 512;
  int lm_cache_slots = 0;
  int lm_cache_capacity = 0;
  struct ShapeKnobs { int lm_blocks, lm_records, lm_cache_slots, accum_blocks; bool mailbox_check; } created_knobs = {};
  int lm_shape[4] = {0, 0, 0, 0};
  int accum_shape[4] = {0, 0, 0, 0};
  int lm_fallbacks = 0;
  lsa_sensor_terms_t sensor_terms = {};
  int* hist_dev = nullptr;
  int hist_pos[3] = {0, 0, 0};
  long long hist_serial[3] = {0, 0, 0};
  int last_match_type = 0;
  int knn_lanes[3] = {16, 8, 8};
  int knn_rounds[3] = {2, 2, 2};
  bool fused_match = true;
  bool fused_model = true;
  void* trace_dev = nullptr;
  bool route_stats = false;
  hipStream_t side_stream[2] = {nullptr, nullptr};
  hipEvent_t ev_fork = nullptr, ev_join[2] = {nullptr, nullptr};
  void* scratch_out = nullptr;
  size_t scratch_cap = 0;
  unsigned long long* range_bits = nullptr;
  hipEvent_t ev_bbox = nullptr;
  hipEvent_t ev_pred = nullptr;
  lsa_point_t* stage[3] = {nullptr, nullptr, nullptr};
  int stage_cap[3] = {0, 0, 0}, stage_n[3] = {0, 0, 0};
  hipEvent_t ev_stage = nullptr;
  bool stage_pending = false;
  bool bbox_pending = false;
  bool bbox_copied = true;
  bool loc_boxes = false;
  bool loc_armed = false;
  bool pred_on_lookahead = false;
  void* pcd_pinned[2] = {nullptr, nullptr};
  void* pcd_dev[2] = {nullptr, nullptr};
  size_t pcd_piece = 0;
  hipEvent_t pcd_ev_copy[2] = {nullptr, nullptr}, pcd_ev_kernel[2] = {nullptr, nullptr};
  int pcd_lds = -1;
  double pcd_times[8] = {0, 0, 0, 0, 0, 0, 0, 0};
  std::mutex prof_mutex;
  std::mutex grave_mutex;
  std::vector<void*> grave_dev, grave_host;
  int bbox_n[3] = {0, 0, 0};
// ... 90 lines not shown
```

### lidarslam_amd/csrc/lsa_ctx.hip

```cpp
#include <algorithm>
#include <cctype>
#include <sched.h>
#include "lsa_ctx.h"

using namespace lsa;

namespace lsa
{

template <typename T> static hipError_t dev_alloc(lsa_ctx* ctx, T** p, size_t count)
{
  if (*p) { retire_dev(ctx, *p); *p = nullptr; }
  return hipMalloc((void**)p, std::max<size_t>(count, 1) * sizeof(T));
}

int ensure_capacity(lsa_ctx* ctx, int n)
{
  if (n <= ctx->cap_n) return LSA_OK;
  int cap = std::max(n + n / 8, 4096);
  LSA_HIP(ctx, hipStreamSynchronize(ctx->stream));
  if (ctx->prefetch_stream) LSA_HIP(ctx, hipStreamSynchronize(ctx->prefetch_stream));
  ctx->prefetch_pending = false;
  for (int k = 0; k < 3; ++k) LSA_HIP(ctx, dev_alloc(ctx, &ctx->kp_next[k], (size_t)cap));
  lsa_point_t* old_kp[3][3];
// ... 116 lines not shown
  if (hipGetDeviceCount(&n) != hipSuccess) return 0;
  return n;
}

int lsa_ctx_create(int device_id, lsa_ctx** out)
{
  if (!out) return LSA_E_ARG;
  *out = nullptr;
  int n = 0;
  if (hipGetDeviceCount(&n) != hipSuccess || n <= 0 || device_id < 0 || device_id >= n)
    return LSA_E_NO_DEVICE;
  if (hipSetDevice(device_id) != hipSuccess) return LSA_E_HIP;
  lsa_ctx* ctx = new lsa_ctx;
  ctx->device = device_id;
  g_live_contexts.fetch_add(1, std::memory_order_relaxed);
  if (hipStreamCreateWithFlags(&ctx->stream, hipStreamNonBlocking) != hipSuccess) { g_live_contexts.fetch_sub(1, std::memory_order_relaxed); delete ctx; return LSA_E_HIP; }
  bool ok = true;
  ok &= hipStreamCreateWithFlags(&ctx->prefetch_stream, hipStreamNonBlocking) == hipSuccess;
  ok &= hipStreamCreateWithFlags(&ctx->copy_stream, hipStreamNonBlocking) == hipSuccess;
  for (int i = 0; i < 2; ++i) ok &= hipEventCreateWithFlags(&ctx->ev_join[i], hipEventDisableTiming) == hipSuccess;
  ok &= hipEventCreateWithFlags(&ctx->ev_fork, hipEventDisableTiming) == hipSuccess;
  ok &= hipEventCreateWithFlags(&ctx->ev_bbox, hipEventDisableTiming) == hipSuccess;
  ok &= hipEventCreateWithFlags(&ctx->ev_pred, hipEventDisableTiming) == hipSuccess;
  ok &= hipEventCreateWithFlags(&ctx->ev_stage, hipEventDisableTiming) == hipSuccess;
  ok &= hipMalloc((void**)&ctx->ring_start, (kMaxRings + 1) * sizeof(int)) == hipSuccess;
  ok &= hipMalloc((void**)&ctx->ring_len, kMaxRings * sizeof(int)) == hipSuccess;
  ok &= hipMalloc((void**)&ctx->extract_out, 16 * sizeof(int)) == hipSuccess;
  ok &= hipMalloc((void**)&ctx->extract_out_next, 16 * sizeof(int)) == hipSuccess;
  ok &= hipHostMalloc((void**)&ctx->host_next, 16 * sizeof(int), hipHostMallocDefault) == hipSuccess;
  ok &= hipEventCreateWithFlags(&ctx->ev_prefetch, hipEventDisableTiming) == hipSuccess;
  ok &= hipEventCreateWithFlags(&ctx->ev_spare, hipEventDisableTiming) == hipSuccess;
  for (int k = 0; k < 3; ++k) ok &= hipEventCreateWithFlags(&ctx->ev_map_ahead[k], hipEventDisableTiming) == hipSuccess;
  ok &= hipEventCreateWithFlags(&ctx->ev_kp_ready, hipEventDisableTiming) == hipSuccess;
  if (ok) { ctx->kp_count_dev = ctx->extract_out; ctx->ring_meta = ctx->extract_out + 4; }
  ok &= hipMalloc((void**)&ctx->ring_counts, kMaxRings * 3 * sizeof(int)) == hipSuccess;
  ok &= hipMalloc((void**)&ctx->partials, (size_t)kAccumBlocksMax * kAccumVals * sizeof(double)) == hipSuccess;
  ok &= hipMalloc((void**)&ctx->reduce_out, 64 * sizeof(double)) == hipSuccess;
  if (ok) ok &= hipMemset(ctx->reduce_out, 0, 64 * sizeof(double)) == hipSuccess;
  ok &= hipMalloc((void**)&ctx->hist_dev, 3 * kHistRing * 16 * sizeof(int)) == hipSuccess;
  if (ok) ok &= hipMemset(ctx->hist_dev, 0, 3 * kHistRing * 16 * sizeof(int)) == hipSuccess;
  ok &= hipMalloc((void**)&ctx->range_bits, 48 * sizeof(unsigned long long)) == hipSuccess;
  ok &= hipHostMalloc((void**)&ctx->host_pinned, 512 * sizeof(double), hipHostMallocDefault) == hipSuccess;
  if (hipHostMalloc((void**)&ctx->mailbox, (size_t)kAccumBlocksMax * kMailboxStride * sizeof(unsigned long long), hipHostMallocCoherent | hipHostMallocMapped) == hipSuccess)
    std::memset(ctx->mailbox, 0, (size_t)kAccumBlocksMax * kMailboxStride * sizeof(unsigned long long));
  else
    ctx->mailbox = nullptr;
  if (hipHostMalloc((void**)&ctx->lm_mailbox, (size_t)kLmMailRing * 2 * kLmOut * sizeof(unsigned long long), hipHostMallocCoherent | hipHostMallocMapped) == hipSuccess)
    std::memset(ctx->lm_mailbox, 0, (size_t)kLmMailRing * 2 * kLmOut * sizeof(unsigned long long));
  else
    ctx->lm_mailbox = nullptr;
  if (ctx->lm_mailbox && hipHostMalloc((void**)&ctx->gate_host, (size_t)kGateRing * kGateGranules * sizeof(unsigned long long), hipHostMallocCoherent | hipHostMallocMapped) == hipSuccess)
  {
    std::memset(ctx->gate_host, 0, (size_t)kGateRing * kGateGranules * sizeof(unsigned long long));
    if (hipMalloc((void**)&ctx->gate_dev, (size_t)kGateRing * kGateWords * sizeof(unsigned long long)) != hipSuccess ||
        hipMemset(ctx->gate_dev, 0, (size_t)kGateRing * kGateWords * sizeof(unsigned long long)) != hipSuccess)
    {
      (void)hipHostFree(ctx->gate_host);
      ctx->gate_host = nullptr;
      ctx->gate_dev = nullptr;
    }
  }
  else
    ctx->gate_host = nullptr;
  if (ctx->gate_dev && (hipMalloc((void**)&ctx->motion_dev, 16 * sizeof(double)) != hipSuccess || hipMemset(ctx->motion_dev, 0, 16 * sizeof(double)) != hipSuccess))
    ctx->motion_dev = nullptr;
  ok &= hipMalloc((void**)&ctx->lm_xchg, (size_t)2 * kLmBlocksMax * kMailboxStride * sizeof(unsigned long long)) == hipSuccess;
  if (ok) ok &= hipMemset(ctx->lm_xchg, 0, (size_t)2 * kLmBlocksMax * kMailboxStride * sizeof(unsigned long long)) == hipSuccess;
  if (const char* e = std::getenv("LSA_ACCUM_BLOCKS")) ctx->accum_blocks = std::min(std::max(std::atoi(e), 1), kAccumBlocksMax);
  ctx->lm_cache_capacity = lm_cache_capacity();
  ctx->lm_cache_slots = ctx->lm_cache_capacity;
  if (const char* e = std::getenv("LSA_LM_CACHE")) ctx->lm_cache_slots = std::min(std::max(std::atoi(e), 0), ctx->lm_cache_slots);
  if (const char* e = std::getenv("LSA_LM_BLOCKS")) ctx->lm_blocks = std::min(std::max(std::atoi(e), 1), kLmBlocksMax);
  if (const char* e = std::getenv("LSA_LM_RECORDS")) ctx->lm_records = std::min(std::max(std::atoi(e), 256), 4096);
  if (const char* e = std::getenv("LSA_ROUTE_STATS")) ctx->route_stats = std::atoi(e) != 0;
  if (ctx->route_stats) ok &= hipMalloc(&ctx->trace_dev, ((size_t)8192 * 12 + 16) * sizeof(unsigned long long)) == hipSuccess && hipMemset(ctx->trace_dev, 0, ((size_t)8192 * 12 + 16) * sizeof(unsigned long long)) == hipSuccess;
  if (const char* e = std::getenv("LSA_FUSED_MATCH")) ctx->fused_match = std::atoi(e) != 0;
  if (const char* e = std::getenv("LSA_FUSED_MODEL")) ctx->fused_model = std::atoi(e) != 0;
  if (const char* e = std::getenv("LSA_MAILBOX_CHECK")) ctx->mailbox_check = std::atoi(e) != 0;
  ctx->created_knobs = {ctx->lm_blocks, ctx->lm_records, ctx->lm_cache_slots, ctx->accum_blocks, ctx->mailbox_check};
  if (!ok) { lsa_ctx_destroy(ctx); return LSA_E_HIP; }
  *out = ctx;
  return LSA_OK;
}

void lsa_ctx_destroy(lsa_ctx* ctx)
{
  if (!ctx) return;
  (void)hipSetDevice(ctx->device);
  if (ctx->stream) (void)hipStreamSynchronize(ctx->stream);
  for (int i = 0; i < 2; ++i)
    if (ctx->side_stream[i]) (void)hipStreamSynchronize(ctx->side_stream[i]);
  if (ctx->prefetch_stream) (void)hipStreamSynchronize(ctx->prefetch_stream);
  if (ctx->uploader.joinable())
  {
    {
      std::lock_guard<std::mutex> l(ctx->up_mutex);
      ctx->up_quit = true;
    }
    ctx->up_cv.notify_all();
    ctx->up_help_cv.notify_all();
    ctx->up_help_done.notify_all();
    ctx->uploader.join();
    for (auto& h : ctx->up_helpers) h.join();
    ctx->up_helpers.clear();
  }
  (void)lsa_collect_garbage(ctx);
  if (ctx->copy_stream) { (void)hipStreamSynchronize(ctx->copy_stream); (void)hipStreamDestroy(ctx->copy_stream); }
  for (auto& in : ctx->inbox)
// ... 130 lines not shown
```

### lidarslam_amd/csrc/lsa_device_grid.hip

```cpp
#include <algorithm>
#include <cfloat>
#include <cmath>
#include <chrono>
#include <cstdlib>
#include <cstring>
#include <limits>
#include <string.h>
#include <vector>
#include "lsa_ctx.h"
#include "lsa_compact.h"
#include "lsa_device_grid_io.h"
#include "host/lsa_map_order.h"
#include "lsa_device_math.h"

using namespace lsa;

namespace lsa
{
__global__ void k_copy_int(int* __restrict__ dst, const int* __restrict__ src) { if (threadIdx.x == 0 && blockIdx.x == 0) *dst = *src; }
}

namespace
{
constexpr u64 kNoKey = ~0ull;
// ... 848 lines not shown
    if (range)
    {
#pragma unroll
      for (int d = 0; d < 3; ++d)
        if (c[d] < range[d] || c[d] > range[3 + d]) return false;
    }
    else
#pragma unroll
    for (int d = 0; d < 3; ++d)
    {
      const float lo_f = ctx_box ? ordered_to_float(ctx_box[d]) : box.mn[d];
      const float hi_f = ctx_box ? ordered_to_float(ctx_box[3 + d]) : box.mx[d];
      const float origin = __int_as_float(st[kStPosX + d]) - (float)((double)(g / 2) * resolution_d);
      const int lo = round_to_int((lo_f - origin) / resolution), hi = round_to_int((hi_f - origin) / resolution);
      if (c[d] < (lo > 0 ? lo : 0) || c[d] > (hi < g - 1 ? hi : g - 1)) return false;
    }
    if (mode == 0) return true;
    const unsigned label = (__float_as_uint(pts[2 * (size_t)i + 1].w) >> 24) & 0xffu;
    if (mode == 1) return count[i] >= min_frames || label == 1;
    return st[kStSubFirst] < min_points && count[i] < min_frames && label != 1;
  }
};
struct PointEmit
{
  const float4* pts;
  float4* out;
  __device__ void operator()(int i, int at) const
  {
    out[2 * (size_t)at] = pts[2 * (size_t)i];
    out[2 * (size_t)at + 1] = pts[2 * (size_t)i + 1];
  }
};
__global__ void k_set_int(int* __restrict__ p, int v) { if (threadIdx.x == 0 && blockIdx.x == 0) *p = v; }
__device__ __forceinline__ void box_voxels(const unsigned* __restrict__ words, int grid_size, float resolution, double resolution_d, const int* __restrict__ st, int lo[3],
                                           int hi[3])
{
#pragma unroll
  for (int d = 0; d < 3; ++d)
  {
    const float origin = __int_as_float(st[kStPosX + d]) - (float)((double)(grid_size / 2) * resolution_d);
    const int a = round_to_int((ordered_to_float(words[d]) - origin) / resolution), b = round_to_int((ordered_to_float(words[3 + d]) - origin) / resolution);
    lo[d] = a > 0 ? a : 0;
    hi[d] = b < grid_size - 1 ? b : grid_size - 1;
  }
}
__global__ void k_pred_box(const unsigned* __restrict__ words, int grid_size, float resolution, double resolution_d, int* __restrict__ st)
{
  if (threadIdx.x != 0 || blockIdx.x != 0) return;
  int lo[3], hi[3];
  box_voxels(words, grid_size, resolution, resolution_d, st, lo, hi);
  for (int d = 0; d < 3; ++d) { st[kStPred + d] = lo[d]; st[kStPred + 3 + d] = hi[d]; }
}
__global__ void k_box_check(const unsigned* __restrict__ words, int grid_size, float resolution, double resolution_d, int* __restrict__ st, u64* __restrict__ host_out,
                            unsigned tag)
{
  if (threadIdx.x != 0 || blockIdx.x != 0) return;
  int lo[3], hi[3];
  box_voxels(words, grid_size, resolution, resolution_d, st, lo, hi);
  bool same = true;
  for (int d = 0; d < 3; ++d) same = same && lo[d] == st[kStPred + d] && hi[d] == st[kStPred + 3 + d];
  if (same) st[kStUpdated] = 0;
  __hip_atomic_store(host_out, ((u64)tag << 32) | (same ? 1u : 0u), __ATOMIC_RELAXED, __HIP_MEMORY_SCOPE_SYSTEM);
}

}

struct lsa_device_grid
{
  lsa_ctx* ctx = nullptr;
  int GridSize = 50;
  double VoxelResolution = 10.;
  double LeafSize = 0.2;
  unsigned MinFramesPerVoxel = 0;
  int Sampling = 2;
  double DecayingThreshold = -1.;
  MapView buf[2] = {};
  int cur = 0;
  int cap = 0;
  int n_upper = 0;
  int* st = nullptr;
  int* host_st = nullptr;
  hipEvent_t ev_state = nullptr;
  hipStream_t stream = nullptr;
  bool own_stream = false, shared_stream = false;
  hipEvent_t ev_in = nullptr, ev_out = nullptr, ev_sub = nullptr, ev_ahead = nullptr;
  u64* host_sub = nullptr;
  unsigned sub_tag = 0;
  int sub_target = -1;
  bool sub_pending = false;
  u64* host_ahead = nullptr;
  unsigned ahead_tag = 0;
  int ahead_phase = 0;
  int ahead_type = -1, ahead_min = 0, ahead_m = 0;
  bool take_pending = false;
  int take_slot = 0;
  int staged = 0;
  bool submap_valid = false;
  int submap_count = 0;
  int bcap = 0;
  float4* batch = nullptr;
  u64 *bkeys = nullptr, *skeys = nullptr;
  unsigned *border = nullptr, *sorder = nullptr;
  int *heads = nullptr, *fresh_flag = nullptr, *chunks = nullptr;
  int* vrank = nullptr;
  int* old_local = nullptr;
  MapView fresh = {};
  int chunk_cap = 0;
  bool Ordered = true;
  lsa::host::KeyShadow shadow;
  int rec_kind = 0;
  int rec_grid = 0;
  int rec_voxels = 0;
  hipEvent_t ev_rec = nullptr;
  int* rec_st = nullptr;
// ... 946 lines not shown
    if (g->ahead_phase != 1) continue;
    if (ctx && (g->ctx != ctx || g->stream != st)) return g->ctx->fail(LSA_E_ARG, "lsa_device_grid_submap_ahead_poll_all: maps of different contexts or streams");
    ctx = g->ctx;
    st = g->stream;
    v[i] = __atomic_load_n(g->host_ahead, __ATOMIC_ACQUIRE);
    if ((unsigned)(v[i] >> 32) != g->ahead_tag) return 1;
    pending[i] = any = true;
  }
  if (!any) return 2;
  LSA_HIP(ctx, hipSetDevice(ctx->device));
  int tis[3], nt = 0;
  for (int i = 0; i < count; ++i)
  {
    if (!pending[i]) continue;
    lsa_device_grid* g = grids[i];
    const int type = g->ahead_type;
    Target& t = ctx->target[9 + type];
    g->ahead_m = (int)(unsigned)(v[i] & 0xffffffffull);
    t.m = g->ahead_m;
    t.cell_hint = ctx->target[LSA_TARGET_MAP * 3 + type].cell_hint;
    t.dirty = false;
    if (t.m > 0) tis[nt++] = 9 + type;
  }
  if (nt > 0)
  {
    const int rc = build_target_grids(ctx, tis, nt, st);
    if (rc) return rc;
  }
  for (int i = 0; i < count; ++i)
  {
    if (!pending[i]) continue;
    LSA_HIP(ctx, hipEventRecord(ctx->ev_map_ahead[grids[i]->ahead_type], st));
    grids[i]->ahead_phase = 2;
  }
  return 2;
}
int lsa_device_grid_submap_ahead_wait(lsa_device_grid* g)
{
  if (!g) return LSA_E_ARG;
  const auto t0 = std::chrono::steady_clock::now();
  unsigned spins = 0;
  while (g->ahead_phase == 1)
  {
    const int rc = lsa_device_grid_submap_ahead_poll(g);
    if (rc < 0) return rc;
    if (rc == 1 && (++spins & 255u) == 0 && std::chrono::steady_clock::now() - t0 > std::chrono::milliseconds(500))
      return g->ctx->fail(LSA_E_HIP, "lsa_device_grid_submap_ahead_wait: the extraction's size did not arrive");
#if defined(__x86_64__)
    __builtin_ia32_pause();
#endif
  }
  return g->ahead_phase;
}
int lsa_device_grid_submap_ahead_take_begin(lsa_device_grid* g, int box_type, int min_nb_points, int slot, int type)
{
  if (!g || box_type < 0 || box_type > 2 || slot < 0 || slot > 1 || type < 0 || type > 2)
    return g ? g->ctx->fail(LSA_E_ARG, "lsa_device_grid_submap_ahead_take: bad argument") : LSA_E_ARG;
  lsa_ctx* ctx = g->ctx;
  g->take_pending = false;
  if (g->ahead_phase == 1)
  {
    const int rc = lsa_device_grid_submap_ahead_poll(g);
    if (rc < 0) return rc;
  }
  const bool fits = g->ahead_phase == 2 && g->ahead_type == type && g->ahead_min == min_nb_points && g->sub_target < 0 &&
                    ctx->target[9 + type].cell_hint == ctx->target[slot * 3 + type].cell_hint;
  g->ahead_phase = 0;
  if (!fits) return 0;
  G_HIP(hipSetDevice(ctx->device));
  G_HIP(hipStreamWaitEvent(ctx->stream, ctx->ev_map_ahead[type], 0));
  const unsigned tag = ++g->ahead_tag;
  const unsigned* words = lsa::current_box_words(ctx) + 6 * box_type;
  hipLaunchKernelGGL(k_box_check, dim3(1), dim3(64), 0, ctx->stream, words, g->GridSize, (float)g->VoxelResolution, g->VoxelResolution, g->st, g->host_ahead + 1, tag);
  g->take_pending = true;
  g->take_slot = slot;
  return 1;
}
int lsa_device_grid_submap_ahead_take_end(lsa_device_grid* g, int* taken)
{
  if (!g || !taken) return LSA_E_ARG;
  *taken = 0;
  if (!g->take_pending) return LSA_OK;
  g->take_pending = false;
  lsa_ctx* ctx = g->ctx;
  const int type = g->ahead_type, slot = g->take_slot;
  const unsigned tag = g->ahead_tag;
  const auto t0 = std::chrono::steady_clock::now();
  unsigned spins = 0;
  u64 v;
  while ((unsigned)((v = __atomic_load_n(g->host_ahead + 1, __ATOMIC_ACQUIRE)) >> 32) != tag)
    if ((++spins & 1023u) == 0 && std::chrono::steady_clock::now() - t0 > std::chrono::seconds(2))
    {
      G_HIP(hipStreamSynchronize(ctx->stream));
      return ctx->fail(LSA_E_HIP, "lsa_device_grid_submap_ahead_take: the comparison did not arrive");
    }
  if (!(v & 1ull)) return LSA_OK;
  ctx->bbox_pending = false;
  std::swap(ctx->target[slot * 3 + type], ctx->target[9 + type]);
  ctx->target[slot * 3 + type].dirty = false;
  g->submap_valid = true;
  g->submap_count = g->ahead_m;
  G_HIP(hipEventSynchronize(g->ev_state));
  g->host_st[kStUpdated] = 0;
  G_HIP(hipEventRecord(g->ev_sub, ctx->stream));
  *taken = 1;
  return g->ahead_m;
}
int lsa_device_grid_submap_ahead_take(lsa_device_grid* g, int box_type, int min_nb_points, int slot, int type, int* taken)
{
  if (!taken) return LSA_E_ARG;
  *taken = 0;
  const int rc = lsa_device_grid_submap_ahead_take_begin(g, box_type, min_nb_points, slot, type);
  return rc <= 0 ? rc : lsa_device_grid_submap_ahead_take_end(g, taken);
}

int lsa_device_grid_submap_valid(lsa_device_grid* g)
{
  if (!g) return 0;
  if (hipSetDevice(g->ctx->device) != hipSuccess || hipEventSynchronize(g->ev_state) != hipSuccess) return 0;
  if (g->host_st[kStUpdated]) g->submap_valid = false;
  return g->submap_valid && g->submap_count > 0 ? 1 : 0;
}

static int readd_everything(lsa_device_grid* g, int ordered)
{
  std::vector<lsa_point_t> all(std::max(g->n_upper, 1));
  const int n = g->n_upper > 0 ? lsa_device_grid_get(g, 0, all.data(), (int)all.size()) : 0;
  if (n < 0) return n;
  if (ordered >= 0)
  {
    if (!ordered)
    {
      g->shadow.Fresh();
      g->rec_kind = 0;
      g->rec_voxels = 0;
      g->order_stale = true;
// ... 11 lines not shown
```

### lidarslam_amd/csrc/lsa_lm.hip

```cpp
#include <chrono>
#include <cmath>
#include "lsa_accum.h"
#include "lsa_device_math.h"
#include "lsa_sensor_terms.h"
#include "../../include/lsa_pmath.h"

using namespace lsa;

namespace
{

typedef unsigned long long u64;
#ifndef LSA_RECORD_PREFETCH
#define LSA_RECORD_PREFETCH 1
#endif
constexpr bool kRecordPrefetch = LSA_RECORD_PREFETCH != 0;

struct LmParams
{
  RecordSet set;
  double x0[6];
  int two_d;
  int max_iter;
  int min_matches;
  unsigned tag_base;
  int cslots;
  int give_up_block;
  const IcpGate* gate;
  IcpGate* leave;
  int link_refine;
  int motion_from_args;
  posemath::ScanPoseClock clock;
  Rigid previous_world;
  double motion0[16];
  double* motion_dev;
  lsa_sensor_terms_t sensors;
  int sensors_on;
};

constexpr int kResPose = 0, kResInitial = 6, kResFinal = 7, kResSums = 8, kResSuccessful = 37, kResUnsuccessful = 38, kResIterations = 39,
              kResEvaluations = 40, kResSkipped = 41, kResCode = 42, kResMatches = 43, kResFailed = 44, kResCount = 45;
static_assert(kResCount <= kLmOut, "result does not fit the mailbox");

__device__ __forceinline__ constexpr int hidx(int a, int b) { return 7 + a * 6 - (a * (a - 1)) / 2 + (b - a); }
__device__ __forceinline__ constexpr int hsym(int a, int b) { return a <= b ? hidx(a, b) : hidx(b, a); }

struct LmState
{
  int cur_buf;
  double x[6], scale[6], diag[6];
  double radius, decrease_factor, x_norm, model_cost_change, delta_norm, initial_cost;
  int reuse_diagonal, consecutive_invalid, iter;
  int evaluations, successful, unsuccessful, iterations, code, skipped, matches;
};

struct Shared
{
  double wsum[kLmThreads / 64][kAccumVals];
  double part[kAccumVals][8];
  double sums[2][kAccumVals];
  double Hs[36], gs[6];
  double w[6];
  double rot[39];
  LmState lm;
  int failed;
  int stop;
  unsigned long long lap[6], tk;
  unsigned long long sub[4], st0;
};

__device__ __forceinline__ double uniform(double v)
{
  const long long b = __double_as_longlong(v);
  const int lo = __builtin_amdgcn_readfirstlane((int)(b & 0xffffffffll)), hi = __builtin_amdgcn_readfirstlane((int)(b >> 32));
  return __longlong_as_double(((long long)hi << 32) | (long long)(unsigned)lo);
}

__device__ __forceinline__ double lane_value(double v, int lane)
{
  const long long b = __double_as_longlong(v);
  const int lo = __shfl((int)(b & 0xffffffffll), lane), hi = __shfl((int)(b >> 32), lane);
  return __longlong_as_double(((long long)hi << 32) | (long long)(unsigned)lo);
}

__device__ __forceinline__ void lm_lap(Shared& sh, int slot)
{
  if (threadIdx.x == 0)
  {
// ... 335 lines not shown
  if (part == 1 && !p.link_refine) return;
  const double half = lm.x[3 + (lane < 6 ? lane % 3 : 0)] * 0.5;
  const double v = lane < 3 ? lsa_cos(half) : lsa_sin(half);
  const double cx = lane_value(v, 0), cy = lane_value(v, 1), cz = lane_value(v, 2);
  const double sx = lane_value(v, 3), sy = lane_value(v, 4), sz = lane_value(v, 5);
  double x[6];
#pragma unroll
  for (int a = 0; a < 6; ++a) x[a] = lm.x[a];
  const Pose T = FromXYZRPYTrig(x, cx, sx, cy, sy, cz, sz);
  if (part == 0)
  {
    if (lane != 0) return;
    double x0[6];
    ToXYZRPY(T, x0);
    g->in.pose = ToRigid(T);
#pragma unroll
    for (int a = 0; a < 6; ++a) g->in.x0[a] = x0[a];
    g->go = 1ull;
    return;
  }
  WithinFrameMotion m;
  double mv[16];
#pragma unroll
  for (int i = 0; i < 16; ++i) mv[i] = p.motion0[i];
  if (!p.motion_from_args)
  {
#pragma unroll
    for (int i = 0; i < 16; ++i) mv[i] = p.motion_dev[i];
  }
  m.Time0 = mv[0]; m.Time1 = mv[1];
  m.Rot0 = {mv[2], mv[3], mv[4], mv[5]};
  m.Rot1 = {mv[6], mv[7], mv[8], mv[9]};
#pragma unroll
  for (int i = 0; i < 3; ++i) { m.Trans0[i] = mv[10 + i]; m.Trans1[i] = mv[13 + i]; }
  const Pose previous = FromRigid(p.previous_world);
  const Pose mine = InterpolateScanPose(p.clock, previous, T, lane == 1 ? m.Time1 : m.Time0);
  Pose worldToBaseEnd = Pose::Identity();
#pragma unroll
  for (int i = 0; i < 3; ++i)
#pragma unroll
    for (int j = 0; j < 4; ++j) worldToBaseEnd(i, j) = lane_value(mine(i, j), 1);
  if (lane != 0) return;
  Pose d0, d1;
  RefineUndistortionFrom(m, mine, worldToBaseEnd, T, d0, d1);
  g->in.ic = MakeInterpConst(d0, d1, m.Time0, m.Time1);
  double* o = p.motion_dev;
  o[0] = m.Time0; o[1] = m.Time1;
  o[2] = m.Rot0.w; o[3] = m.Rot0.x; o[4] = m.Rot0.y; o[5] = m.Rot0.z;
  o[6] = m.Rot1.w; o[7] = m.Rot1.x; o[8] = m.Rot1.y; o[9] = m.Rot1.z;
#pragma unroll
  for (int i = 0; i < 3; ++i) { o[10 + i] = m.Trans0[i]; o[13 + i] = m.Trans1[i]; }
}

__global__ __launch_bounds__(kLmThreads) void k_lm_solve(LmParams p, u64* __restrict__ xchg, u64* __restrict__ mailbox, unsigned out_tag, unsigned long long* trace)
{
  __shared__ Shared sh;
  extern __shared__ double lm_cache[];
  const bool tr = trace != nullptr && blockIdx.x == 0;
  RecordRegs pre;
  if (kRecordPrefetch && p.cslots > 0) record_load(p.set, blockIdx.x * blockDim.x + threadIdx.x, pre);
  if (p.gate)
  {
    const unsigned long long go = p.gate->go;
    if (go != 1ull)
    {
      if (go == 2ull && blockIdx.x == 0 && threadIdx.x < 2 * kResCount)
      {
        const double r = (threadIdx.x >> 1) == kResFailed ? 2. : 0.;
        const u64 bits = (u64)__double_as_longlong(r);
        const unsigned word = (threadIdx.x & 1) ? (unsigned)(bits >> 32) : (unsigned)(bits & 0xffffffffull);
        __hip_atomic_store(mailbox + threadIdx.x, ((u64)out_tag << 32) | word, __ATOMIC_RELAXED, __HIP_MEMORY_SCOPE_SYSTEM);
      }
      if (p.leave && blockIdx.x == 0 && threadIdx.x == 0) p.leave->go = 0ull;
      return;
    }
  }
  if (threadIdx.x == 0)
  {
    for (int i = 0; i < 6; ++i) sh.lap[i] = 0;
    for (int i = 0; i < 4; ++i) sh.sub[i] = 0;
    sh.st0 = 0;
    sh.tk = wall_clock64();
    sh.lap[5] = sh.tk;
    LmState& lm = sh.lm;
#pragma unroll
    for (int v = 0; v < kAccumVals; ++v) sh.sums[0][v] = 0.;
    lm.cur_buf = 0;
    double x0[6];
#pragma unroll
    for (int a = 0; a < 6; ++a) x0[a] = p.x0[a];
    if (p.gate)
    {
#pragma unroll
      for (int a = 0; a < 6; ++a) x0[a] = p.gate->in.x0[a];
    }
#pragma unroll
    for (int a = 0; a < 6; ++a) { lm.x[a] = x0[a]; lm.scale[a] = 1.; lm.diag[a] = 0.; }
    lm.radius = 1e4; lm.decrease_factor = 2.0; lm.x_norm = 0.; lm.model_cost_change = 0.; lm.delta_norm = 0.; lm.initial_cost = 0.;
    lm.reuse_diagonal = 0; lm.consecutive_invalid = 0; lm.iter = 0;
    lm.evaluations = 1; lm.successful = 0; lm.unsuccessful = 0; lm.iterations = 0; lm.code = kCodeNone; lm.skipped = 0; lm.matches = 0;
    set_point(sh, x0);
    sh.stop = 0;
  }
  if (threadIdx.x < 64) finish_point(sh);
  if (kRecordPrefetch && p.cslots > 0) record_stash(pre, lm_cache, p.cslots * kLmThreads, threadIdx.x);
  __syncthreads();
  bool failed = false;
  for (unsigned epoch = 1;; ++epoch)
  {
    if (!lm_evaluate(p, epoch, xchg, sh, lm_cache, tr)) { failed = true; break; }
    if (threadIdx.x < 64)
    {
      if (threadIdx.x == 0 && tr) sh.st0 = wall_clock64();
      if (p.two_d) lm_step<3>(p, sh, epoch == 1);
      else lm_step<6>(p, sh, epoch == 1);
      asm volatile("s_waitcnt lgkmcnt(0)" ::: "memory");
      if (!sh.stop) finish_point(sh);
    }
    __syncthreads();
    if (tr) lm_lap(sh, 3);
    if (sh.stop) break;
  }
  if (blockIdx.x != 0) return;
  if (tr && threadIdx.x == 0)
  {
    for (int i = 0; i < 4; ++i) trace[i] += sh.lap[i];
    trace[4] += (unsigned long long)sh.lm.evaluations;
    trace[5] += wall_clock64() - sh.lap[5];
    trace[6] += 1;
    trace[7] += sh.lap[4];
    for (int i = 0; i < 4; ++i) trace[8 + i] += sh.sub[i];
  }
  if (p.leave && threadIdx.x >= 64 && threadIdx.x < 192) leave_link(p, sh.lm, failed, (threadIdx.x >> 6) - 1);
  if (threadIdx.x < 2 * kResCount)
  {
    const LmState& lm = sh.lm;
    const int v = threadIdx.x >> 1, half = threadIdx.x & 1;
    double r = 0.;
    if (v < kResInitial) r = lm.x[v - kResPose];
    else if (v == kResInitial) r = lm.initial_cost;
    else if (v == kResFinal) r = sh.sums[lm.cur_buf][0];
    else if (v < kResSums + kAccumVals) r = sh.sums[lm.cur_buf][v - kResSums];
    else if (v == kResSuccessful) r = lm.successful;
    else if (v == kResUnsuccessful) r = lm.unsuccessful;
    else if (v == kResIterations) r = lm.iterations;
    else if (v == kResEvaluations) r = lm.evaluations;
    else if (v == kResSkipped) r = lm.skipped;
    else if (v == kResCode) r = lm.code;
    else if (v == kResMatches) r = lm.matches;
    else if (v == kResFailed) r = failed ? 1. : 0.;
    const u64 bits = (u64)__double_as_longlong(r);
    const unsigned word = half ? (unsigned)(bits >> 32) : (unsigned)(bits & 0xffffffffull);
    __hip_atomic_store(mailbox + threadIdx.x, ((u64)out_tag << 32) | word, __ATOMIC_RELAXED, __HIP_MEMORY_SCOPE_SYSTEM);
  }
}

__global__ __launch_bounds__(kGateGranules) void k_icp_gate(const u64* __restrict__ host_granules, u64* __restrict__ dev_words, unsigned seq, int give_up)
{
  __shared__ unsigned halves[kGateGranules];
  __shared__ int state;
  const int t = threadIdx.x;
  if (t == 0) state = give_up ? 2 : 0;
  __syncthreads();
  const unsigned long long t0 = wall_clock64();
  while (state == 0)
  {
    const u64 g = __hip_atomic_load(host_granules + t, __ATOMIC_RELAXED, __HIP_MEMORY_SCOPE_SYSTEM);
    const bool mine = (unsigned)(g >> 32) == seq;
    if (mine) halves[t] = (unsigned)(g & 0xffffffffull);
    const int all = __syncthreads_and(mine ? 1 : 0);
    if (t == 0)
    {
      if (all) state = 1;
      else if (wall_clock64() - t0 > 5000000ull) state = 2;
    }
    __syncthreads();
    if (state == 0) __builtin_amdgcn_s_sleep(1);
  }
  if (state == 1)
  {
    if (t < kGateWords)
    {
      const u64 w = ((u64)halves[2 * t + 1] << 32) | halves[2 * t];
      if (t == 0 || (halves[0] | halves[1]) != 0u) dev_words[t] = w;
    }
  }
  else if (t == 0)
    dev_words[0] = 2ull;
}

const char* const kMessages[] = {"", "not enough matches", "gradient tolerance (iteration 0)", "max iterations", "gradient tolerance",
                                 "min trust region radius", "too many invalid steps", "parameter tolerance", "function tolerance"};

}

namespace lsa
{
std::atomic<int> g_live_contexts{0};
int lm_blocks_share()
{
  static const int cus = [] {
    hipDeviceProp_t prop;
    int dev = 0;
    if (hipGetDevice(&dev) != hipSuccess || hipGetDeviceProperties(&prop, dev) != hipSuccess) return 256;
    return std::max(prop.multiProcessorCount, 8);
  }();
  static const int queues = [] {
    const char* e = std::getenv("GPU_MAX_HW_QUEUES");
    const int q = e ? std::atoi(e) : 4;
    return std::max(q, 1);
  }();
  const int side_by_side = std::max(1, std::min(g_live_contexts.load(std::memory_order_relaxed), queues));
  return std::max(cus / side_by_side, 8);
}
InterpConst make_interp_const(const double H0[16], const double H1[16], double t0, double t1);
int lm_cache_capacity()
{
  const size_t layer = (size_t)17 * kLmThreads * sizeof(double);
  size_t limit = 0, static_bytes = 0;
  {
    hipDeviceProp_t prop;
    int dev = 0;
    if (hipGetDevice(&dev) == hipSuccess && hipGetDeviceProperties(&prop, dev) == hipSuccess) limit = std::max(prop.sharedMemPerBlock, (size_t)prop.maxSharedMemoryPerMultiProcessor);
    hipFuncAttributes attr;
    if (hipFuncGetAttributes(&attr, reinterpret_cast<const void*>(k_lm_solve)) == hipSuccess) static_bytes = attr.sharedSizeBytes;
  }
  int slots = 0;
  for (int want = 3; want >= 1 && slots == 0; --want)
    if ((limit == 0 || static_bytes + want * layer <= limit) &&
        hipFuncSetAttribute(reinterpret_cast<const void*>(k_lm_solve), hipFuncAttributeMaxDynamicSharedMemorySize, (int)(want * layer)) == hipSuccess)
      slots = want;
  (void)hipGetLastError();
  return slots;
}
}

extern "C" {

static int solve_device_begin(lsa_ctx* ctx, unsigned type_mask, const double prior[6], int two_d_mode, int lm_max_iter, int min_matches, int leave_ticket, const lsa_icp_link_t* link)
{
  if (!ctx) return LSA_E_ARG;
  if (leave_ticket >= 0 && (leave_ticket >= kGateRing || !link || !ctx->gate_dev || !ctx->gate_saved[leave_ticket].used || !ctx->gate_saved[leave_ticket].link))
    return ctx->fail(LSA_E_ARG, "lsa_solve_device_begin_linked: no such link (lsa_icp_link)");
  if (!prior && ctx->gate_current < 0) return ctx->fail(LSA_E_ARG, "lsa_solve_device_begin: no start point and no gate to wait behind");
  if (!ctx->lm_mailbox) return ctx->fail(LSA_E_STATE, "lsa_solve_device: no coherent host memory for the result");
  LSA_HIP(ctx, hipSetDevice(ctx->device));
  LmParams p;
  int total = 0;
  for (int k = 0; k < 3; ++k)
  {
    MatchBuf& mb = ctx->match[k];
    const bool use = (type_mask >> k) & 1u && mb.valid && mb.k > 0;
    p.set.rec[k] = mb.rec; p.set.status[k] = mb.status; p.set.cap[k] = mb.cap;
    p.set.count[k] = use ? mb.k : 0;
    p.set.sat2[k] = mb.sat * mb.sat;
    total += p.set.count[k];
  }
  for (int a = 0; a < 6; ++a) p.x0[a] = prior ? prior[a] : 0.;
  p.give_up_block = ctx->debug_lm_give_up_block;
  ctx->debug_lm_give_up_block = -1;
  p.gate = prior ? nullptr : reinterpret_cast<const IcpGate*>(ctx->gate_dev + (size_t)ctx->gate_current * kGateWords);
  p.leave = nullptr;
  p.link_refine = 0;
  p.motion_from_args = 0;
  p.motion_dev = ctx->motion_dev;
  std::memset(&p.clock, 0, sizeof(p.clock));
  std::memset(&p.previous_world, 0, sizeof(p.previous_world));
  std::memset(p.motion0, 0, sizeof(p.motion0));
  if (leave_ticket >= 0)
  {
    p.leave = reinterpret_cast<IcpGate*>(ctx->gate_dev + (size_t)leave_ticket * kGateWords);
    p.link_refine = link->refine_undistortion ? 1 : 0;
    p.motion_from_args = link->first ? 1 : 0;
    p.clock.have_log = link->have_log ? 1 : 0;
    p.clock.prev_time = link->prev_time;
    p.clock.cur_time = link->cur_time;
    p.clock.max_ratio = link->max_extrapolation_ratio;
    row_major_to_rt(link->previous_world, p.previous_world.R, p.previous_world.t);
    std::memcpy(p.motion0, link->motion, sizeof(p.motion0));
  }
  p.sensors = ctx->sensor_terms;
  p.sensors_on = (ctx->sensor_terms.wheel || ctx->sensor_terms.gravity) ? 1 : 0;
  p.two_d = two_d_mode ? 1 : 0;
  p.max_iter = lm_max_iter < 0 ? 0 : lm_max_iter;
  p.min_matches = min_matches;
  p.tag_base = ctx->lm_tag;
  ctx->lm_tag += (unsigned)p.max_iter + 4u;
  const unsigned out_tag = (unsigned)(++ctx->lm_seq);
  const int nb = std::min(std::max((total + ctx->lm_records - 1) / ctx->lm_records, 1), std::min(std::min(ctx->lm_blocks, kLmBlocksMax), lm_blocks_share()));
  const int per_thread = (total + nb * kLmThreads - 1) / (nb * kLmThreads);
  const size_t slot_bytes = (size_t)17 * kLmThreads * sizeof(double);
  p.cslots = std::min(per_thread, std::max(ctx->lm_cache_slots, 0));
  ctx->lm_shape[0] = nb; ctx->lm_shape[1] = per_thread; ctx->lm_shape[2] = p.cslots; ctx->lm_shape[3] = total;
  {
    ProfScope ps(ctx, "lm_solve", 0.);
    hipLaunchKernelGGL(k_lm_solve, dim3(nb), dim3(kLmThreads), p.cslots * slot_bytes, ctx->stream, p, ctx->lm_xchg, ctx->lm_mailbox + (size_t)(out_tag % kLmMailRing) * 2 * kLmOut, out_tag,
                       ctx->route_stats && ctx->trace_dev ? reinterpret_cast<unsigned long long*>(ctx->trace_dev) + (size_t)8192 * 12 : nullptr);
  }
  ctx->lm_pending.push_back(out_tag);
  ctx->lm_pending_wait.push_back(prior ? -1 : ctx->gate_current);
  if (leave_ticket >= 0) ctx->gate_current = leave_ticket;
  if (lsa_icp_trace_on()) std::fprintf(stderr, "[lm begin] tag %u gated %d leaves %d sat2 %.6g %.6g counts %d %d\n", out_tag, prior ? 0 : 1, leave_ticket, p.set.sat2[0], p.set.sat2[1], p.set.count[0], p.set.count[1]);
  return LSA_OK;
}

int lsa_solve_device_begin(lsa_ctx* ctx, unsigned type_mask, const double prior[6], int two_d_mode, int lm_max_iter, int min_matches)
{
  return solve_device_begin(ctx, type_mask, prior, two_d_mode, lm_max_iter, min_matches, -1, nullptr);
}

int lsa_solve_device_begin_linked(lsa_ctx* ctx, unsigned type_mask, const double prior[6], int two_d_mode, int lm_max_iter, int min_matches, int leave_ticket, const lsa_icp_link_t* link)
{
  if (ctx && (int)ctx->lm_pending.size() >= kLmMailRing - 1) return ctx->fail(LSA_E_STATE, "lsa_solve_device_begin_linked: too many solves in flight");
  return solve_device_begin(ctx, type_mask, prior, two_d_mode, lm_max_iter, min_matches, leave_ticket, link);
}

int lsa_solve_device_drop(lsa_ctx* ctx)
{
  if (!ctx || ctx->lm_pending.empty()) return LSA_E_ARG;
  ctx->lm_pending.pop_back();
  ctx->lm_pending_wait.pop_back();
  return LSA_OK;
}

int lsa_solve_device_end(lsa_ctx* ctx, lsa_solve_result_t* out)
{
  if (!ctx || !out) return ctx ? ctx->fail(LSA_E_ARG, "lsa_solve_device_end: bad argument") : LSA_E_ARG;
  if (ctx->lm_pending.empty()) return ctx->fail(LSA_E_STATE, "lsa_solve_device_end: no solve in flight");
  const unsigned out_tag = ctx->lm_pending.front();
  ctx->lm_pending.pop_front();
  const int waited_behind = ctx->lm_pending_wait.front();
  ctx->lm_pending_wait.pop_front();
  if (lsa_icp_trace_on()) std::fprintf(stderr, "[lm end] waits for tag %u (%zu more in flight)\n", out_tag, ctx->lm_pending.size());
  double res[kResCount];
  const unsigned long long* box = ctx->lm_mailbox + (size_t)(out_tag % kLmMailRing) * 2 * kLmOut;
  {
    const auto t0 = std::chrono::steady_clock::now();
    unsigned spins = 0;
    for (int v = 0; v < kResCount; ++v)
    {
      unsigned long long g[2];
      for (int h = 0; h < 2; ++h)
        while (((g[h] = __atomic_load_n(box + 2 * v + h, __ATOMIC_RELAXED)) >> 32) != out_tag)
        {
          if ((++spins & 0x3ff) == 0 && std::chrono::steady_clock::now() - t0 > std::chrono::milliseconds(2000))
          {
            (void)lsa_icp_abandon(ctx);
            LSA_HIP(ctx, hipStreamSynchronize(ctx->stream));
            return ctx->fail(LSA_E_STATE, "lsa_solve_device: no result from the device");
          }
#if defined(__x86_64__)
          __builtin_ia32_pause();
#endif
        }
      const unsigned long long bits = ((g[1] & 0xffffffffull) << 32) | (g[0] & 0xffffffffull);
      std::memcpy(&res[v], &bits, sizeof(double));
    }
  }
  if (lsa_icp_trace_on()) std::fprintf(stderr, "[lm end] tag %u: failed %g code %g evals %g matches %g\n", out_tag, res[kResFailed], res[kResCode], res[kResEvaluations], res[kResMatches]);
  if (res[kResFailed] == 2.) return ctx->fail(LSA_E_GATE, "lsa_solve_device: the gate in front of the solve gave up waiting for the host");
  if (res[kResFailed] != 0.)
  {
    (void)lsa_icp_abandon(ctx);
    LSA_HIP(ctx, hipStreamSynchronize(ctx->stream));
    ctx->lm_fallbacks++;
    return ctx->fail(LSA_E_STATE, "lsa_solve_device: a block waited too long for the others");
  }
// ... 134 lines not shown
  for (int i = 0; i < kGateWords; ++i)
  {
    __atomic_store_n(g + 2 * i, ((unsigned long long)seq << 32) | (words[i] & 0xffffffffull), __ATOMIC_RELAXED);
    __atomic_store_n(g + 2 * i + 1, ((unsigned long long)seq << 32) | (words[i] >> 32), __ATOMIC_RELAXED);
  }
  if (lsa_icp_trace_on()) std::fprintf(stderr, "[gate] ticket %d seq %u %s\n", ticket, seq, block ? "posted" : "called off");
  ctx->gate_saved[ticket].used = false;
  if (ctx->gate_current == ticket) ctx->gate_current = -1;
  return LSA_OK;
}

int lsa_icp_post(lsa_ctx* ctx, int ticket, const double pose[16], const double prior[6], const double H0[16], const double H1[16], double t0, double t1)
{
  if (!ctx || !pose || !prior || ((H0 == nullptr) != (H1 == nullptr))) return ctx ? ctx->fail(LSA_E_ARG, "lsa_icp_post: bad argument") : LSA_E_ARG;
  IcpGate g;
  std::memset(&g, 0, sizeof(g));
  g.go = 1;
  row_major_to_rt(pose, g.in.pose.R, g.in.pose.t);
  for (int a = 0; a < 6; ++a) g.in.x0[a] = prior[a];
  if (H0) g.in.ic = make_interp_const(H0, H1, t0, t1);
  return gate_release(ctx, ticket, &g);
}

int lsa_icp_cancel(lsa_ctx* ctx, int ticket)
{
  if (!ctx || ticket < 0 || ticket >= kGateRing) return LSA_E_ARG;
  const lsa_ctx::GateSaved sv = ctx->gate_saved[ticket];
  if (sv.link)
  {
    if (!sv.used) return ctx->fail(LSA_E_ARG, "lsa_icp_cancel: no such link");
    ctx->gate_saved[ticket].used = false;
    if (ctx->gate_current == ticket) ctx->gate_current = -1;
  }
  else
  {
    const int rc = gate_release(ctx, ticket, nullptr);
    if (rc) return rc;
  }
  for (int k = 0; k < 3; ++k)
    if ((sv.mask >> k) & 1u)
    {
      ctx->match[k].sat = sv.sat[k];
      ctx->match[k].k = sv.k[k];
      ctx->match[k].valid = sv.valid[k];
      ctx->hist_pos[k] = sv.hist_pos[k];
      ctx->hist_serial[k] = sv.hist_serial[k];
    }
  return LSA_OK;
}

int lsa_icp_abandon(lsa_ctx* ctx)
{
  if (!ctx) return LSA_E_ARG;
  while (true)
  {
    int youngest = -1;
    for (int t = 0; t < kGateRing; ++t)
      if (ctx->gate_saved[t].used && (youngest < 0 || (int)(ctx->gate_saved[t].seq - ctx->gate_saved[youngest].seq) > 0)) youngest = t;
    if (youngest < 0) break;
    if (lsa_icp_cancel(ctx, youngest) != LSA_OK) ctx->gate_saved[youngest].used = false;
  }
  ctx->lm_pending.clear();
  ctx->lm_pending_wait.clear();
  ctx->gate_current = -1;
  return LSA_OK;
}

int lsa_debug_set(lsa_ctx* ctx, const char* name, int value)
{
  if (!ctx || !name) return LSA_E_ARG;
  const std::string n(name);
  const lsa_ctx::ShapeKnobs& c = ctx->created_knobs;
  if (n == "gate_give_up_every") ctx->debug_gate_give_up_every = value;
  else if (n == "lm_give_up_block") ctx->debug_lm_give_up_block = value;
  else if (n == "lm_blocks") ctx->lm_blocks = value < 0 ? c.lm_blocks : std::min(std::max(value, 1), kLmBlocksMax);
  else if (n == "lm_records") ctx->lm_records = value < 0 ? c.lm_records : std::min(std::max(value, 256), 4096);
  else if (n == "lm_cache") ctx->lm_cache_slots = value < 0 ? c.lm_cache_slots : std::min(value, ctx->lm_cache_capacity);
  else if (n == "accum_blocks") ctx->accum_blocks = value < 0 ? c.accum_blocks : std::min(std::max(value, 1), kAccumBlocksMax);
  else if (n == "mailbox_check") ctx->mailbox_check = value < 0 ? c.mailbox_check : value != 0;
  else if (n == "pcd_lds") ctx->pcd_lds = value < 0 ? -1 : (value != 0);
  else if (n == "kplog_chunk_kib") ctx->kplog_chunk_bytes = value < 0 ? ((size_t)32 << 20) : (size_t)std::max(value, 1) << 10;
  else if (n == "kplog_fail_alloc") ctx->debug_kplog_fail_alloc = value > 0 ? 1 : 0;
  else return ctx->fail(LSA_E_ARG, "lsa_debug_set: no such knob");
  return LSA_OK;
}

int lsa_solve_device_shape(const lsa_ctx* ctx, int out[4])
{
  if (!ctx || !out) return LSA_E_ARG;
  std::memcpy(out, ctx->lm_shape, sizeof(ctx->lm_shape));
  return LSA_OK;
}

int lsa_accumulate_shape(const lsa_ctx* ctx, int out[4])
{
  if (!ctx || !out) return LSA_E_ARG;
  std::memcpy(out, ctx->accum_shape, sizeof(ctx->accum_shape));
  return LSA_OK;
}

int lsa_solve_device_fallbacks(const lsa_ctx* ctx) { return ctx ? ctx->lm_fallbacks : 0; }

int lsa_set_sensor_terms(lsa_ctx* ctx, const lsa_sensor_terms_t* terms)
{
  if (!ctx) return LSA_E_ARG;
  if (terms) ctx->sensor_terms = *terms;
// ... 22 lines not shown
```

### lidarslam_amd/csrc/lsa_match.hip

```cpp
#include <cmath>
#include <cstring>
#include "lsa_ctx.h"
#include "lsa_device_math.h"
#include "lsa_knn.h"
#include "lsa_match_internal.h"

using namespace lsa;

namespace
{

__global__ void k_fill_status(uint8_t* __restrict__ status, double* __restrict__ rec, int cap, int n, uint8_t v)
{
  const int i = blockIdx.x * blockDim.x + threadIdx.x;
  if (i < n) { status[i] = v; rec[(size_t)15 * cap + i] = 0.; }
}

__global__ void k_records_to_aos(const double* __restrict__ rec, const uint8_t* __restrict__ status, int cap, int n, double* __restrict__ out,
                                 double* __restrict__ weights)
{
  const int i = blockIdx.x * blockDim.x + threadIdx.x;
  if (i >= n) return;
  const bool ok = status[i] == LSA_MATCH_SUCCESS;
  if (out)
    for (int f = 0; f < 16; ++f) out[(size_t)i * 16 + f] = ok ? rec[(size_t)f * cap + i] : 0.;
  weights[i] = ok ? rec[(size_t)15 * cap + i] : 0.;
}

}

static int* hist_block(lsa_ctx* ctx, int type, int pos) { return ctx->hist_dev + ((size_t)type * kHistRing + pos) * 16; }

int lsa::next_hist_block(lsa_ctx* ctx, int type, hipStream_t st, int** hist)
{
  constexpr int half = kHistRing / 2;
  ++ctx->hist_serial[type];
  if (++ctx->hist_pos[type] >= kHistRing) ctx->hist_pos[type] = 0;
  const int pos = ctx->hist_pos[type];
  if (pos % half == 0) LSA_HIP(ctx, hipMemsetAsync(hist_block(ctx, type, pos), 0, (size_t)half * 16 * sizeof(int), st));
  *hist = hist_block(ctx, type, pos);
  return LSA_OK;
}

static hipError_t read_hist_block(lsa_ctx* ctx, int type, int pos, int offset, int* out, int n)
{
  const hipError_t e = hipStreamSynchronize(ctx->stream);
  return e != hipSuccess ? e : hipMemcpy(out, hist_block(ctx, type, pos) + offset, (size_t)n * sizeof(int), hipMemcpyDeviceToHost);
}

struct TypeParams { int k; bool bad; };
static TypeParams type_params(const lsa_match_params_t& p, int type)
{
  if (type == LSA_EDGE) return {p.edge_nb_neighbors, p.edge_nb_neighbors < 2 || p.edge_min_nb_neighbors < 2};
  if (type == LSA_PLANE) return {p.plane_nb_neighbors, p.plane_nb_neighbors < 3};
  return {p.blob_nb_neighbors, p.blob_nb_neighbors < 4};
}

extern "C" {

int lsa_set_fused_match(lsa_ctx* ctx, int on)
{
  if (!ctx) return LSA_E_ARG;
  ctx->fused_match = on != 0;
  ctx->fused_model = on != 2;
  return LSA_OK;
}

static int match_prepare(lsa_ctx* ctx, int slot, int type, int query_set, const lsa_match_params_t* p, hipStream_t st, MatchPrep& out)
{
  const int nq = ctx->kp_n[query_set][type];
  MatchBuf& mb = ctx->match[type];
  int* hist = nullptr;
  {
    const int rc = next_hist_block(ctx, type, st, &hist);
    if (rc) return rc;
  }
  mb.k = nq;
  mb.knn_n = 0;
  mb.sat = p->saturation_distance;
  mb.valid = true;
  ctx->last_match_type = type;
  if (nq == 0) return 0;
  const int ti = slot * 3 + type;
  Target& t = ctx->target[ti];
  if (t.m == 0)
  {
    hipLaunchKernelGGL(k_fill_status, dim3((nq + 255) / 256), dim3(256), 0, st, mb.status, mb.rec, mb.cap, nq, (uint8_t)LSA_MATCH_UNKOWN);
    return 0;
  }
  MatchConst mc;
  mc.type = type;
  mc.single_edge_per_ring = p->single_edge_per_ring;
  mc.min_neighbors = p->edge_min_nb_neighbors;
  mc.max_dist2 = p->max_neighbors_distance * p->max_neighbors_distance;
  mc.planarity = p->planarity_threshold;
  const TypeParams tp = type_params(*p, type);
  mc.k = tp.k;
  mc.bad_param = tp.bad ? 1 : 0;
  mc.max_model_err = type == LSA_EDGE ? p->edge_max_model_error : type == LSA_PLANE ? p->plane_max_model_error : 0.;
  const double e2 = p->edge_max_model_error * p->edge_max_model_error;
  mc.ransac_sq_inlier = (float)e2;
  if (mc.k < 1) mc.k = 1;
  float far_d2 = INFINITY;
  if (type != LSA_EDGE && t.m >= mc.k) far_d2 = (float)(mc.max_dist2 * 1.0001);
  out.type = type;
  out.ti = ti;
  out.queries = ctx->kp[query_set][type];
  out.nq = nq;
  out.mc = mc;
  out.far_d2 = far_d2;
  out.hist = hist;
  return 1;
}

static int match_check(lsa_ctx* ctx, int type, const lsa_match_params_t* p)
{
  if (type_params(*p, type).k > kKnnMax) return ctx->fail(LSA_E_ARG, "lsa_match: more than 16 neighbours requested");
  return LSA_OK;
}

int lsa_match(lsa_ctx* ctx, int slot, int type, int query_set, const lsa_match_params_t* p, const double pose[16], int histogram[LSA_MATCH_NSTATUS])
{
  if (!ctx || !p || !pose || slot < 0 || slot > 1 || type < 0 || type > 2 || query_set < 0 || query_set > 2)
    return ctx ? ctx->fail(LSA_E_ARG, "lsa_match: bad argument") : LSA_E_ARG;
  int hist3[3 * LSA_MATCH_NSTATUS];
  const int rc = lsa_match_types(ctx, slot, 1u << type, query_set, p, pose, histogram ? hist3 : nullptr);
  if (rc == LSA_OK && histogram) std::memcpy(histogram, hist3 + type * LSA_MATCH_NSTATUS, LSA_MATCH_NSTATUS * sizeof(int));
  return rc;
}

static int match_types_impl(lsa_ctx* ctx, int slot, unsigned type_mask, int query_set, const lsa_match_params_t* p, const double pose[16], int* histograms,
                            const InterpConst* undistort, int gate = -1, bool gate_undistorts = false)
{
  if (!ctx || !p || (!pose && gate < 0) || slot < 0 || slot > 1 || (type_mask & ~7u) || query_set < 0 || query_set > 2)
    return ctx ? ctx->fail(LSA_E_ARG, "lsa_match_types: bad argument") : LSA_E_ARG;
  LSA_HIP(ctx, hipSetDevice(ctx->device));
  if (histograms) std::memset(histograms, 0, 3 * LSA_MATCH_NSTATUS * sizeof(int));
  int types[3], nt = 0;
  for (int k = 0; k < 3; ++k)
    if ((type_mask >> k) & 1u)
    {
      int rc = match_check(ctx, k, p);
      if (rc) return rc;
      rc = ensure_match(ctx, k, ctx->kp_n[query_set][k]);
      if (rc) return rc;
      types[nt++] = k;
    }
  if (nt == 0) return LSA_OK;
  {
    const int rc = flush_grids(ctx);
    if (rc) return rc;
  }
  if (ctx->fused_match)
  {
    MatchPrep preps[3];
    int np = 0;
    for (int i = 0; i < nt; ++i)
    {
      if (gate >= 0)
      {
        lsa_ctx::GateSaved& sv = ctx->gate_saved[gate];
        const int k = types[i];
        sv.mask |= 1u << k;
        sv.sat[k] = ctx->match[k].sat; sv.k[k] = ctx->match[k].k; sv.valid[k] = ctx->match[k].valid;
        sv.hist_pos[k] = ctx->hist_pos[k]; sv.hist_serial[k] = ctx->hist_serial[k];
      }
      const int rc = match_prepare(ctx, slot, types[i], query_set, p, ctx->stream, preps[np]);
      if (rc < 0) return rc;
      if (rc > 0) ++np;
    }
    if (np > 0)
    {
      const int rc = enqueue_fused_match(ctx, preps, np, pose, ctx->stream, undistort, gate, gate_undistorts);
      if (rc) return rc;
    }
  }
  else
  {
    for (int i = 0; i + 1 < nt; ++i)
      if (!ctx->side_stream[i]) LSA_HIP(ctx, hipStreamCreateWithFlags(&ctx->side_stream[i], hipStreamNonBlocking));
    if (nt > 1) LSA_HIP(ctx, hipEventRecord(ctx->ev_fork, ctx->stream));
    for (int i = 0; i < nt; ++i)
    {
      hipStream_t st = i == 0 ? ctx->stream : ctx->side_stream[i - 1];
      if (i > 0) LSA_HIP(ctx, hipStreamWaitEvent(st, ctx->ev_fork, 0));
      MatchPrep mp;
      const int rc = match_prepare(ctx, slot, types[i], query_set, p, st, mp);
      if (rc < 0) return rc;
      if (rc > 0) enqueue_staged_match(ctx, mp, pose, st);
      if (i > 0) LSA_HIP(ctx, hipEventRecord(ctx->ev_join[i - 1], st));
    }
    for (int i = 1; i < nt; ++i) LSA_HIP(ctx, hipStreamWaitEvent(ctx->stream, ctx->ev_join[i - 1], 0));
  }
  if (histograms)
  {
    int* hp = reinterpret_cast<int*>(ctx->host_pinned) + 32;
    for (int i = 0; i < nt; ++i)
      LSA_HIP(ctx, hipMemcpyAsync(hp + types[i] * 16, hist_block(ctx, types[i], ctx->hist_pos[types[i]]), 16 * sizeof(int),
                                  hipMemcpyDeviceToHost, ctx->stream));
    LSA_HIP(ctx, hipStreamSynchronize(ctx->stream));
    for (int i = 0; i < nt; ++i)
      for (int s = 0; s < LSA_MATCH_NSTATUS; ++s) histograms[types[i] * LSA_MATCH_NSTATUS + s] = hp[types[i] * 16 + s];
  }
  return LSA_OK;
}

int lsa_match_types(lsa_ctx* ctx, int slot, unsigned type_mask, int query_set, const lsa_match_params_t* p, const double pose[16], int* histograms)
{
  return match_types_impl(ctx, slot, type_mask, query_set, p, pose, histograms, nullptr);
}

static bool search_reaches_every_keypoint(lsa_ctx* ctx, int slot, unsigned type_mask, const lsa_match_params_t* p)
{
  bool reach = ctx->fused_match;
  for (int k = 0; k < 3 && reach; ++k)
  {
    if (ctx->kp_n[LSA_SET_WORKING][k] <= 0) continue;
    const TypeParams tp = type_params(*p, k);
    reach = ((type_mask >> k) & 1u) && ctx->target[slot * 3 + k].m > 0 && !tp.bad && tp.k <= kKnnMax;
  }
  return reach;
}

int lsa_match_types_undistorted(lsa_ctx* ctx, int slot, unsigned type_mask, const lsa_match_params_t* p, const double pose[16], int* histograms, const double H0[16],
                                const double H1[16], double t0, double t1)
{
  if (!ctx || !p || !pose || !H0 || !H1 || slot < 0 || slot > 1 || (type_mask & ~7u))
    return ctx ? ctx->fail(LSA_E_ARG, "lsa_match_types_undistorted: bad argument") : LSA_E_ARG;
  if (!search_reaches_every_keypoint(ctx, slot, type_mask, p))
  {
    const int rc = lsa_undistort(ctx, H0, H1, t0, t1);
    return rc ? rc : match_types_impl(ctx, slot, type_mask, LSA_SET_WORKING, p, pose, histograms, nullptr);
  }
  const InterpConst ic = make_interp_const(H0, H1, t0, t1);
  return match_types_impl(ctx, slot, type_mask, LSA_SET_WORKING, p, pose, histograms, &ic);
}

int lsa_match_types_gated(lsa_ctx* ctx, int slot, unsigned type_mask, int query_set, const lsa_match_params_t* p, int undistort)
{
  if (!ctx || !p || slot < 0 || slot > 1 || (type_mask & ~7u) || query_set < 0 || query_set > 2)
    return ctx ? ctx->fail(LSA_E_ARG, "lsa_match_types_gated: bad argument") : LSA_E_ARG;
  if (ctx->gate_current < 0) return ctx->fail(LSA_E_STATE, "lsa_match_types_gated: no gate to wait behind (lsa_icp_gate)");
  if (!ctx->fused_match || !ctx->fused_model) return 1;
  if (undistort && (query_set != LSA_SET_WORKING || !search_reaches_every_keypoint(ctx, slot, type_mask, p))) return 1;
  for (int k = 0; k < 3; ++k)
    if (((type_mask >> k) & 1u) && ctx->kp_n[query_set][k] > 0 && ctx->target[slot * 3 + k].m <= 0) return 1;
  return match_types_impl(ctx, slot, type_mask, query_set, p, nullptr, nullptr, nullptr, ctx->gate_current, undistort != 0);
}

int lsa_download_match(lsa_ctx* ctx, int type, uint8_t* status, double* weights, double* records, int capacity)
{
  if (!ctx || type < 0 || type > 2 || !status || !weights) return ctx ? ctx->fail(LSA_E_ARG, "lsa_download_match: bad argument") : LSA_E_ARG;
  MatchBuf& mb = ctx->match[type];
  if (!mb.valid) return 0;
  const int n = std::min(capacity, mb.k);
  if (n <= 0) return 0;
  const size_t bytes = (size_t)n * (16 + 1) * sizeof(double);
  int rc = ensure_scratch(ctx, bytes);
  if (rc) return rc;
  double* drec = (double*)ctx->scratch_out;
  double* dw = drec + (size_t)n * 16;
  hipLaunchKernelGGL(k_records_to_aos, dim3((n + 255) / 256), dim3(256), 0, ctx->stream, mb.rec, mb.status, mb.cap, n, records ? drec : nullptr, dw);
  if (records) LSA_HIP(ctx, hipMemcpyAsync(records, drec, (size_t)n * 16 * sizeof(double), hipMemcpyDeviceToHost, ctx->stream));
  LSA_HIP(ctx, hipMemcpyAsync(weights, dw, (size_t)n * sizeof(double), hipMemcpyDeviceToHost, ctx->stream));
  LSA_HIP(ctx, hipMemcpyAsync(status, mb.status, (size_t)n, hipMemcpyDeviceToHost, ctx->stream));
  LSA_HIP(ctx, hipStreamSynchronize(ctx->stream));
  return n;
}

int lsa_upload_match(lsa_ctx* ctx, int type, const uint8_t* status, const double* records, int n, double saturation)
{
  if (!ctx || type < 0 || type > 2 || n < 0 || (n > 0 && (!status || !records)) || !std::isfinite(saturation))
    return ctx ? ctx->fail(LSA_E_ARG, "lsa_upload_match: bad argument") : LSA_E_ARG;
  LSA_HIP(ctx, hipSetDevice(ctx->device));
  MatchBuf& mb = ctx->match[type];
  int rc = ensure_match(ctx, type, n);
  if (rc) return rc;
  if (n > 0)
  {
    std::vector<double> soa((size_t)16 * n);
    for (int i = 0; i < n; ++i)
      for (int f = 0; f < 16; ++f) soa[(size_t)f * n + i] = records[(size_t)i * 16 + f];
    LSA_HIP(ctx, hipMemcpy2DAsync(mb.rec, (size_t)mb.cap * sizeof(double), soa.data(), (size_t)n * sizeof(double), (size_t)n * sizeof(double), 16,
                                  hipMemcpyHostToDevice, ctx->stream));
    LSA_HIP(ctx, hipMemcpyAsync(mb.status, status, (size_t)n, hipMemcpyHostToDevice, ctx->stream));
    LSA_HIP(ctx, hipStreamSynchronize(ctx->stream));
  }
  mb.k = n;
  mb.sat = saturation;
  mb.valid = true;
  return LSA_OK;
}

int lsa_download_knn(lsa_ctx* ctx, int type, int* idx, float* d2, int* cnt, int capacity)
{
  static_assert(LSA_KNN_MAX == kKnnMax, "the header's row length is the buffers'");
  if (!ctx || type < 0 || type > 2 || !idx || !d2 || !cnt) return ctx ? ctx->fail(LSA_E_ARG, "lsa_download_knn: bad argument") : LSA_E_ARG;
  LSA_HIP(ctx, hipSetDevice(ctx->device));
  const MatchBuf& mb = ctx->match[type];
  const int n = std::min(capacity, mb.knn_n);
// ... 66 lines not shown
```

### lidarslam_amd/csrc/lsa_transform.hip

```cpp
#include <cfloat>
#include <cmath>
#include <limits>
#include "lsa_ctx.h"
#include "lsa_device_math.h"

using namespace lsa;

namespace
{

__device__ __forceinline__ double point_time(const float4& b) { return __hiloint2double(__float_as_int(b.y), __float_as_int(b.x)); }

struct KpSetsRW
{
  float4* pts[3];
  int n[3];
};
__global__ __launch_bounds__(256) void k_undistort(KpSetsRW s, InterpConst c)
{
  float4* __restrict__ pts = s.pts[blockIdx.y];
  const int i = blockIdx.x * blockDim.x + threadIdx.x;
  if (i >= s.n[blockIdx.y]) return;
  float4 a = pts[2 * (size_t)i];
  const float4 b = pts[2 * (size_t)i + 1];
// ... 209 lines not shown

__global__ __launch_bounds__(256) void k_loc_start(StageOut s, int undistort, InterpConst c, int boxes, Rigid T0, unsigned* __restrict__ bits)
{
  __shared__ unsigned slo[4][3], shi[4][3];
  const int t = blockIdx.y;
  const int n = s.n[t];
  if ((int)(blockIdx.x * blockDim.x) >= n) return;
  const int i = blockIdx.x * blockDim.x + threadIdx.x;
  unsigned lo[3] = {~0u, ~0u, ~0u}, hi[3] = {0u, 0u, 0u};
  if (i < n)
  {
    float4 a = s.in[t][2 * (size_t)i];
    const float4 b = s.in[t][2 * (size_t)i + 1];
    if (undistort)
    {
      Rigid U;
      interp_eval(c, point_time(b), U);
      double ox, oy, oz;
      rigid_apply(U, (double)a.x, (double)a.y, (double)a.z, ox, oy, oz);
      a.x = (float)ox; a.y = (float)oy; a.z = (float)oz;
    }
    s.out[t][2 * (size_t)i] = a;
    s.out[t][2 * (size_t)i + 1] = b;
    if (boxes)
    {
      double ox, oy, oz;
      rigid_apply(T0, (double)a.x, (double)a.y, (double)a.z, ox, oy, oz);
      const float v[3] = {(float)ox, (float)oy, (float)oz};
      for (int d = 0; d < 3; ++d)
        if (v[d] == v[d]) lo[d] = hi[d] = f2ou(v[d]);
    }
  }
  if (!boxes) return;
  for (int d = 0; d < 3; ++d)
    for (int sft = 32; sft > 0; sft >>= 1)
    {
      const unsigned l2 = __shfl_down(lo[d], sft), h2 = __shfl_down(hi[d], sft);
      lo[d] = l2 < lo[d] ? l2 : lo[d];
      hi[d] = h2 > hi[d] ? h2 : hi[d];
    }
  if ((threadIdx.x & 63) == 0)
    for (int d = 0; d < 3; ++d) { slo[threadIdx.x >> 6][d] = lo[d]; shi[threadIdx.x >> 6][d] = hi[d]; }
  __syncthreads();
  if (threadIdx.x < 3)
  {
    const int d = threadIdx.x;
    unsigned l = slo[0][d], h = shi[0][d];
    for (int w = 1; w < 4; ++w) { l = slo[w][d] < l ? slo[w][d] : l; h = shi[w][d] > h ? shi[w][d] : h; }
    atomicMin(&bits[6 * t + d], l);
    atomicMax(&bits[6 * t + 3 + d], h);
  }
}

InterpConst make_interp(const double H0[16], const double H1[16], double t0, double t1)
{
  posemath::Pose a, b;
  std::memcpy(a.m, H0, sizeof(a.m));
  std::memcpy(b.m, H1, sizeof(b.m));
  return posemath::MakeInterpConst(a, b, t0, t1);
}

}

namespace lsa
{
InterpConst make_interp_const(const double H0[16], const double H1[16], double t0, double t1) { return make_interp(H0, H1, t0, t1); }

int enqueue_time_range(lsa_ctx* ctx, int set, const int* counts_dev)
{
  KpSets sets;
  int nmax = 0;
  for (int k = 0; k < 3; ++k)
  {
    sets.pts[k] = reinterpret_cast<const float4*>(ctx->kp[set][k]);
    sets.n[k] = ctx->kp_n[set][k];
    nmax = std::max(nmax, sets.n[k]);
  }
  if (counts_dev) nmax = ctx->frame_n;
  hipLaunchKernelGGL(k_range_init, dim3(1), dim3(64), 0, ctx->stream, ctx->range_bits);
  if (nmax > 0)
    hipLaunchKernelGGL(k_time_range3, dim3((nmax + 255) / 256, 3), dim3(256), 0, ctx->stream, sets, counts_dev, ctx->range_bits);
  return LSA_OK;
}
void finish_time_range(lsa_ctx* ctx, int set, const unsigned long long bits[2])
{
  const int total = ctx->kp_n[set][0] + ctx->kp_n[set][1] + ctx->kp_n[set][2];
  ctx->kp_time[set][0] = total == 0 ? std::numeric_limits<double>::max() : o2d_host(bits[0]);
  ctx->kp_time[set][1] = total == 0 ? std::numeric_limits<double>::lowest() : o2d_host(bits[1]);
  ctx->kp_time_valid[set] = true;
}
}

extern "C" {

int lsa_reset_working_keypoints(lsa_ctx* ctx)
{
  if (!ctx) return LSA_E_ARG;
  LSA_HIP(ctx, hipSetDevice(ctx->device));
  StageOut so;
  int nmax = 0;
  for (int k = 0; k < 3; ++k)
  {
    const int n = ctx->kp_n[LSA_SET_RAW_CURRENT][k];
    ctx->kp_n[LSA_SET_WORKING][k] = n;
    so.in[k] = reinterpret_cast<const float4*>(ctx->kp[LSA_SET_RAW_CURRENT][k]);
    so.out[k] = reinterpret_cast<float4*>(ctx->kp[LSA_SET_WORKING][k]);
// ... 24 lines not shown
  }
  if (nmax <= 0) return LSA_OK;
  ProfScope ps(ctx, "undistort", (double)total * 48);
  hipLaunchKernelGGL(k_undistort, dim3((nmax + 255) / 256, 3), dim3(256), 0, ctx->stream, sets, c);
  return LSA_OK;
}

int lsa_arm_localization_boxes(lsa_ctx* ctx)
{
  if (!ctx) return LSA_E_ARG;
  if (ctx->loc_armed) return LSA_OK;
  LSA_HIP(ctx, hipSetDevice(ctx->device));
  hipLaunchKernelGGL(k_bbox_init, dim3(1), dim3(64), 0, ctx->stream, lsa::loc_box_words(ctx));
  ctx->loc_armed = true;
  return LSA_OK;
}

int lsa_localization_begin(lsa_ctx* ctx, const double H0[16], const double H1[16], double t0, double t1, const double box_pose[16])
{
  if (!ctx || (H0 && !H1)) return ctx ? ctx->fail(LSA_E_ARG, "lsa_localization_begin: bad argument") : LSA_E_ARG;
  LSA_HIP(ctx, hipSetDevice(ctx->device));
  StageOut so;
  int nmax = 0, total = 0;
  for (int k = 0; k < 3; ++k)
  {
    const int n = ctx->kp_n[LSA_SET_RAW_CURRENT][k];
    ctx->kp_n[LSA_SET_WORKING][k] = n;
    so.in[k] = reinterpret_cast<const float4*>(ctx->kp[LSA_SET_RAW_CURRENT][k]);
    so.out[k] = reinterpret_cast<float4*>(ctx->kp[LSA_SET_WORKING][k]);
    so.n[k] = n;
    if (box_pose) ctx->bbox_n[k] = n;
    nmax = std::max(nmax, n);
    total += std::max(n, 0);
  }
  ctx->kp_time_valid[LSA_SET_WORKING] = ctx->kp_time_valid[LSA_SET_RAW_CURRENT];
  ctx->kp_time[LSA_SET_WORKING][0] = ctx->kp_time[LSA_SET_RAW_CURRENT][0];
  ctx->kp_time[LSA_SET_WORKING][1] = ctx->kp_time[LSA_SET_RAW_CURRENT][1];
  ctx->loc_boxes = box_pose != nullptr;
  if (box_pose)
  {
    const int rc = lsa_arm_localization_boxes(ctx);
    if (rc) return rc;
    ctx->loc_armed = false;
    ctx->bbox_pending = true;
    ctx->bbox_copied = false;
  }
  if (nmax <= 0) return LSA_OK;
  InterpConst c{};
  if (H0) c = make_interp(H0, H1, t0, t1);
  Rigid T{};
  if (box_pose) row_major_to_rt(box_pose, T.R, T.t);
  ProfScope ps(ctx, "undistort", (double)total * (H0 ? 64 : 64));
  hipLaunchKernelGGL(k_loc_start, dim3((nmax + 255) / 256, 3), dim3(256), 0, ctx->stream, so, H0 ? 1 : 0, c, box_pose ? 1 : 0, T, lsa::loc_box_words(ctx));
  return LSA_OK;
}

int lsa_working_time_range(lsa_ctx* ctx, double* tmin, double* tmax) { return lsa_keypoint_time_range(ctx, LSA_SET_WORKING, tmin, tmax); }

int lsa_keypoint_time_range(lsa_ctx* ctx, int set, double* tmin, double* tmax)
{
  if (!ctx || !tmin || !tmax || set < 0 || set > 2) return ctx ? ctx->fail(LSA_E_ARG, "lsa_keypoint_time_range: bad argument") : LSA_E_ARG;
  LSA_HIP(ctx, hipSetDevice(ctx->device));
  if (!ctx->kp_time_valid[set])
  {
    int rc = lsa::enqueue_time_range(ctx, set, nullptr);
    if (rc) return rc;
    unsigned long long* hp = reinterpret_cast<unsigned long long*>(ctx->host_pinned + 128);
    LSA_HIP(ctx, hipMemcpyAsync(hp, ctx->range_bits, 2 * sizeof(unsigned long long), hipMemcpyDeviceToHost, ctx->stream));
    LSA_HIP(ctx, hipStreamSynchronize(ctx->stream));
    lsa::finish_time_range(ctx, set, hp);
  }
  *tmin = ctx->kp_time[set][0];
  *tmax = ctx->kp_time[set][1];
  return LSA_OK;
}
static int bboxes_begin(lsa_ctx* ctx, int set, const double pose[16], const double pose_end[16], double t0, double t1)
{
  if (!ctx || !pose || set < 0 || set > 2) return ctx ? ctx->fail(LSA_E_ARG, "lsa_keypoint_bboxes_begin: bad argument") : LSA_E_ARG;
  LSA_HIP(ctx, hipSetDevice(ctx->device));
  KpSets sets;
  int nmax = 0;
  for (int k = 0; k < 3; ++k)
  {
    sets.pts[k] = reinterpret_cast<const float4*>(ctx->kp[set][k]);
    sets.n[k] = ctx->bbox_n[k] = ctx->kp_n[set][k];
    nmax = std::max(nmax, sets.n[k]);
  }
  ctx->bbox_pending = true;
  ctx->pred_on_lookahead = false;
  if (nmax <= 0) return LSA_OK;
  Rigid T;
  row_major_to_rt(pose, T.R, T.t);
  unsigned* bits = reinterpret_cast<unsigned*>(ctx->range_bits + 16);
  hipLaunchKernelGGL(k_bbox_init, dim3(1), dim3(64), 0, ctx->stream, bits);
  InterpConst ic{};
  if (pose_end) ic = make_interp(pose, pose_end, t0, t1);
  hipLaunchKernelGGL(k_bbox3, dim3((nmax + 255) / 256, 3), dim3(256), 0, ctx->stream, sets, T, pose_end ? 1 : 0, ic, bits);
  LSA_HIP(ctx, hipMemcpyAsync(ctx->host_pinned + 160, bits, 18 * sizeof(unsigned), hipMemcpyDeviceToHost, ctx->stream));
  LSA_HIP(ctx, hipEventRecord(ctx->ev_bbox, ctx->stream));
  ctx->bbox_copied = true;
  return LSA_OK;
}
int lsa_keypoint_bboxes_begin(lsa_ctx* ctx, int set, const double pose[16]) { return bboxes_begin(ctx, set, pose, nullptr, 0., 0.); }
int lsa_keypoint_bboxes_begin_interp(lsa_ctx* ctx, int set, const double H0[16], const double H1[16], double t0, double t1)
{
  if (!H1) return ctx ? ctx->fail(LSA_E_ARG, "lsa_keypoint_bboxes_begin_interp: bad argument") : LSA_E_ARG;
// ... 204 lines not shown
```

Before: 1393 frames/s.

## Start localization undistortion and first match ahead during chained ego-motion ICP

Adds a hand-over path: while the ego-motion ICP chain is still running on the device, the host enqueues the localization start kernel and the first map match. The kernel reads the final pose and interpolation constants from a device-side gate block, so it can run without a host round trip. Localization then adopts the precomputed matches and submaps instead of re-enqueuing them. This hides host launch latency and serialization between the two stages, at the cost of considerable state-save/restore complexity and wasted work whenever the hand-over is dropped.

```diff
diff --git a/include/lidarslam_amd.h b/include/lidarslam_amd.h
--- a/include/lidarslam_amd.h
+++ b/include/lidarslam_amd.h
@@ -227,6 +227,21 @@
                                   int leave_ticket, const lsa_icp_link_t* link);
 int lsa_icp_link_peek(lsa_ctx* ctx, int ticket, unsigned long long words[64]);
 int lsa_icp_link_expected(const double x[6], int skipped, int successful_steps, const lsa_icp_link_t* link, unsigned long long words[64], double motion_after[16]);
+
+typedef struct lsa_loc_handover
+{
+  int undistort;
+  int have_log;
+  double prev_time, cur_time, max_extrapolation_ratio;
+  double previous_world[16];
+  double t0, t1;
+} lsa_loc_handover_t;
+int lsa_loc_handover_arm(lsa_ctx* ctx, const lsa_loc_handover_t* h);
+int lsa_loc_handover_start(lsa_ctx* ctx);
+int lsa_match_types_handover(lsa_ctx* ctx, int slot, unsigned type_mask, unsigned spare_mask, const lsa_match_params_t* p);
+int lsa_loc_handover_commit(lsa_ctx* ctx);
+int lsa_loc_handover_drop(lsa_ctx* ctx);
+int lsa_icp_abandon_loop(lsa_ctx* ctx);
 
 int lsa_solve_device_trace(lsa_ctx* ctx, unsigned long long out[12]);
 int lsa_debug_set(lsa_ctx* ctx, const char* name, int value);
@@ -383,6 +398,8 @@
 int lsa_device_grid_submap_ahead_take(lsa_device_grid* g, int box_type, int min_nb_points, int slot, int type, int* taken);
 int lsa_device_grid_submap_ahead_take_begin(lsa_device_grid* g, int box_type, int min_nb_points, int slot, int type);
 int lsa_device_grid_submap_ahead_take_end(lsa_device_grid* g, int* taken);
+int lsa_device_grid_submap_ahead_ready(lsa_device_grid* g, int min_nb_points, int slot, int type);
+int lsa_device_grid_submap_ahead_check_handover(lsa_device_grid* g, int box_type, int min_nb_points, int slot, int type);
 int lsa_device_grid_add_pcd(lsa_device_grid* g, const char* path, int fixed, double time, int roll_first);
 int lsa_device_grid_save_pcd(lsa_device_grid* g, const char* path, int format, int clean);
 int lsa_pcd_io_times(const lsa_ctx* ctx, double out[8]);
diff --git a/lidarslam_amd/__init__.py b/lidarslam_amd/__init__.py
--- a/lidarslam_amd/__init__.py
+++ b/lidarslam_amd/__init__.py
@@ -44,7 +44,8 @@
     "lsa_set_azimuthal_resolution", "lsa_extract_keypoints", "lsa_extract_keypoints_more", "lsa_extract_prefetch", "lsa_extract_prefetch_adopted", "lsa_transform_frame_at", "lsa_set_keypoint_types", "lsa_download_keypoints", "lsa_keypoint_count",
     "lsa_download_debug", "lsa_nb_laser_rings", "lsa_transform_keypoints", "lsa_set_target", "lsa_set_target_from_set", "lsa_prepare_previous_targets", "lsa_prepared_targets_adopted", "lsa_target_staging", "lsa_set_target_staged", "lsa_stage_target_ahead", "lsa_drop_target_ahead", "lsa_staged_targets_adopted",
     "lsa_target_size", "lsa_download_target", "lsa_set_target_cell_size", "lsa_set_knn_lanes", "lsa_set_fused_match", "lsa_set_knn_rounds", "lsa_match_slow_queries", "lsa_match_exhaustive_queries", "lsa_match_route_stats", "lsa_match_trace", "lsa_set_keypoints", "lsa_match", "lsa_match_types", "lsa_match_types_undistorted",
-    "lsa_download_match", "lsa_upload_match", "lsa_download_knn", "lsa_overlap", "lsa_accumulate", "lsa_mailbox_active", "lsa_solve", "lsa_solve_device", "lsa_solve_device_fallbacks", "lsa_solve_device_begin", "lsa_solve_device_end", "lsa_solve_device_drop", "lsa_icp_gate", "lsa_icp_link", "lsa_solve_device_begin_linked", "lsa_icp_link_peek", "lsa_icp_link_expected", "lsa_icp_post", "lsa_icp_cancel", "lsa_icp_abandon", "lsa_debug_set", "lsa_solve_device_shape", "lsa_accumulate_shape", "lsa_match_types_gated", "lsa_solve_device_trace", "lsa_registration_error", "lsa_selftest_math", "lsa_selftest_numerics", "lsa_selftest_labels", "lsa_reset_working_keypoints", "lsa_undistort", "lsa_working_time_range",
+    "lsa_download_match", "lsa_upload_match", "lsa_download_knn", "lsa_overlap", "lsa_accumulate", "lsa_mailbox_active", "lsa_solve", "lsa_solve_device", "lsa_solve_device_fallbacks", "lsa_solve_device_begin", "lsa_solve_device_end", "lsa_solve_device_drop", "lsa_icp_gate", "lsa_icp_link", "lsa_solve_device_begin_linked", "lsa_icp_link_peek", "lsa_icp_link_expected", "lsa_icp_post", "lsa_icp_cancel", "lsa_icp_abandon", "lsa_icp_abandon_loop", "lsa_loc_handover_arm", "lsa_loc_handover_start", "lsa_match_types_handover", "lsa_loc_handover_commit", "lsa_loc_handover_drop",
+    "lsa_device_grid_submap_ahead_ready", "lsa_device_grid_submap_ahead_check_handover", "lsa_debug_set", "lsa_solve_device_shape", "lsa_accumulate_shape", "lsa_match_types_gated", "lsa_solve_device_trace", "lsa_registration_error", "lsa_selftest_math", "lsa_selftest_numerics", "lsa_selftest_labels", "lsa_reset_working_keypoints", "lsa_undistort", "lsa_working_time_range",
     "lsa_working_bbox", "lsa_working_bboxes", "lsa_localization_begin", "lsa_arm_localization_boxes", "lsa_keypoint_bboxes_begin", "lsa_keypoint_bboxes_begin_interp", "lsa_keypoint_boxes_predicted_mark", "lsa_keypoint_boxes_predicted", "lsa_keypoint_time_range", "lsa_keypoint_bboxes_end", "lsa_download_transformed", "lsa_stage_transformed", "lsa_staged_transformed", "lsa_transform_frame", "lsa_profile_enable", "lsa_profile_select", "lsa_profile_reset",
     "lsa_profile_get", "lsa_slam_create", "lsa_slam_destroy", "lsa_slam_last_error", "lsa_slam_set_param",
     "lsa_slam_get_param", "lsa_slam_reset", "lsa_slam_clear_maps", "lsa_slam_add_frame", "lsa_slam_store_frame", "lsa_slam_add_stored_frame", "lsa_slam_hint_next_stored_frame", "lsa_slam_hint_next_frame", "lsa_upload_frame_begin", "lsa_upload_frame_ready", "lsa_upload_frame_adopt", "lsa_upload_frame_forget", "lsa_profile_event_overhead_us", "lsa_upload_robosense_frame", "lsa_pin_host_memory", "lsa_unpin_host_memory", "lsa_collect_garbage", "lsa_uploads_adopted", "lsa_extract_prefetch_uploaded",
diff --git a/lidarslam_amd/csrc/host/lsa_slam_core.cpp b/lidarslam_amd/csrc/host/lsa_slam_core.cpp
--- a/lidarslam_amd/csrc/host/lsa_slam_core.cpp
+++ b/lidarslam_amd/csrc/host/lsa_slam_core.cpp
@@ -605,6 +605,8 @@
   double FrameStats::*lmSeconds;
   int FrameStats::*iterations;
   bool countSkippedEvals;
+  const lsa_loc_handover_t* handover;
+  bool firstMatchEnqueued;
 };
 struct SlamCore::IcpUndistortion
 {
@@ -635,6 +637,10 @@
   bool chain = aheadOk && ICPAhead >= 2 && spec.maxIter <= kChainMax && spec.linksOk;
   bool ahead = aheadOk && !chain && spec.gatesOk;
   if (ahead || chain) lsa_icp_abandon(Ctx);
+  HandoverStarted = HandoverSearched = HandoverGaveUp = false;
+  LoopChained = 0;
+  const bool handover = chain && spec.handover && lsa_loc_handover_arm(Ctx, spec.handover) == LSA_OK;
+  bool handoverDead = false;
   unsigned chained = 0;
   long long chainSerial[kChainMax][3] = {};
   bool enqueuedAhead = false;
@@ -652,9 +658,11 @@
     }
     if (all || icpIter + 1 < chained)
     {
-      lsa_icp_abandon(Ctx);
+      if (all) lsa_icp_abandon(Ctx);
+      else lsa_icp_abandon_loop(Ctx);
       chained = 0;
     }
+    if (all) HandoverStarted = HandoverSearched = false;
   };
   struct AtExit { decltype(callOffRest)& callOffRest; bool failed; ~AtExit() { callOffRest(failed); } } atExit{callOffRest, true};
 
@@ -703,7 +711,8 @@
     }
     else if (!enqueuedAhead)
     {
-      if (const int rc = matchInLine(); rc < 0) return rc;
+      if (spec.firstMatchEnqueued && icpIter == 0) takeSerials(spec.matchSerial);
+      else if (const int rc = matchInLine(); rc < 0) return rc;
       if (chain)
       {
         double prior[6];
@@ -759,9 +768,11 @@
         }
       }
     }
+    LoopChained = handover && !handoverDead ? chained : 0;
     if (const int rc = enqueued(icpIter); rc < 0) return rc;
     if (!begun) ArmLookaheadInterlude();
-    Stats.*spec.icpSeconds += ticp.Stop();
+    Stats.*spec.icpSeconds += ticp.Stop() - HandoverSeconds;
+    HandoverSeconds = 0.;
     (Stats.*spec.iterations)++;
 
     Tick tlm;
@@ -787,7 +798,7 @@
         rc = optimizer.Solve(summary);
       }
       if (rc < 0) return Fail(rc, "LocalOptimizer::End / Solve");
-      if (rc == 1) { ticket = -1; ahead = false; chained = 0; }
+      if (rc == 1) { ticket = -1; ahead = false; chained = 0; handoverDead = true; HandoverStarted = HandoverSearched = false; }
       if (irc < 0) return irc;
     }
     else
@@ -809,6 +820,7 @@
     if (rc < 0) return rc;
     if (last)
     {
+      if (summary.skipped) handoverDead = true;
       if (const int frc = summary.skipped ? LSA_OK : finished(optimizer); frc < 0) return frc;
       break;
     }
@@ -827,6 +839,11 @@
       undistortion.pending = false;
   }
   atExit.failed = false;
+  if (handover && (handoverDead || !HandoverStarted))
+  {
+    lsa_loc_handover_drop(Ctx);
+    HandoverStarted = HandoverSearched = false;
+  }
   return LSA_OK;
 }
 
@@ -891,6 +908,19 @@
   spec.lmSeconds = &FrameStats::ego_lm;
   spec.iterations = &FrameStats::ego_iters;
   spec.countSkippedEvals = true;
+  lsa_loc_handover_t handover;
+  std::memset(&handover, 0, sizeof(handover));
+  if (LocalizationStartAhead && ICPAhead >= 2 && spec.maxIter <= kChainMax && DeviceMapsInUse() && LocalizationStartFused && MapUpdate != MappingMode::NONE && !KeepMatchDebug)
+  {
+    handover.undistort = Undistortion ? 1 : 0;
+    if (Undistortion) LSA_TRY(lsa_keypoint_time_range(Ctx, LSA_SET_RAW_CURRENT, &handover.t0, &handover.t1));
+    handover.have_log = LogTrajectory.empty() ? 0 : 1;
+    handover.prev_time = LogTrajectory.empty() ? 0. : LogTrajectory.back().time;
+    handover.cur_time = StampToSec(CurrentStamp);
+    handover.max_extrapolation_ratio = MaxExtrapolationRatio;
+    std::memcpy(handover.previous_world, Tworld.m, sizeof(handover.previous_world));
+    spec.handover = &handover;
+  }
   auto enqueued = [&](unsigned icpIter) -> int {
     if (icpIter == 0 && BuildTargetsAhead)
     {
@@ -898,6 +928,7 @@
       AheadWorker.Submit([this] { AheadStatus = PrepareNextEgoMotionTargets(); });
     }
     if (!SpecPending) LSA_TRY(StageSpeculativeSubMaps());
+    if (LoopChained == spec.maxIter && !HandoverStarted && !HandoverGaveUp && !SpecPending && !DevSpecRunning.load(std::memory_order_acquire)) LSA_TRY(StartLocalizationAhead());
     return LSA_OK;
   };
   auto solved = [&]() -> int { return SpecPending ? FinishSubMapSpeculation() : LSA_OK; };
@@ -918,7 +949,24 @@
   Tworld = PreviousTworld * Trelative;
   const bool oneLaunch = LocalizationStartFused && DeviceMapsInUse() && MapUpdate != MappingMode::NONE;
   bool boxesEnqueued = false;
-  if (oneLaunch)
+  const bool handover = HandoverStarted;
+  HandoverStarted = false;
+  struct HandoverGuard { lsa_ctx* ctx; bool pending; ~HandoverGuard() { if (pending) lsa_icp_abandon(ctx); } } handoverGuard{Ctx, handover};
+  if (handover)
+  {
+    Tick t;
+    if (Undistortion)
+    {
+      double t0, t1;
+      LSA_TRY(lsa_keypoint_time_range(Ctx, LSA_SET_RAW_CURRENT, &t0, &t1));
+      Pose d0, d1;
+      InitUndistortion(t0, t1);
+      RefineUndistortion(&d0, &d1);
+    }
+    boxesEnqueued = true;
+    Stats.undistort += t.Stop();
+  }
+  else if (oneLaunch)
   {
     Tick t;
     Pose d0 = Pose::Identity(), d1 = Pose::Identity();
@@ -979,13 +1027,14 @@
     bool need[3], checking[3] = {false, false, false}, any = false;
     for (int k = 0; k < 3; ++k)
     {
-      need[k] = UseKeypoints[k] && !lsa_device_grid_submap_valid(DevMaps[k]);
+      need[k] = handover ? HandoverNeed[k] : UseKeypoints[k] && !lsa_device_grid_submap_valid(DevMaps[k]);
+      checking[k] = handover && HandoverChecking[k];
       any = any || need[k];
     }
     if (any && MapUpdate != MappingMode::NONE && !boxesEnqueued) LSA_TRY(lsa_keypoint_bboxes_begin(Ctx, LSA_SET_WORKING, Tworld.m));
     for (int k = 0; k < 3; ++k)
     {
-      if (!need[k]) continue;
+      if (!need[k] || checking[k]) continue;
       lsa_set_target_cell_size(Ctx, LSA_TARGET_MAP, k, static_cast<float>((k == LSA_EDGE ? KnnCellScaleMapsEdges : KnnCellScaleMaps) * LocalMaps[k]->GetLeafSize()));
       if (MapUpdate == MappingMode::NONE) LSA_TRY(lsa_device_grid_build_submap_begin(DevMaps[k], nullptr, nullptr, -1, LSA_TARGET_MAP, k));
       else
@@ -1005,6 +1054,9 @@
       LSA_TRY(lsa_device_grid_build_submap_begin_for_keypoints(DevMaps[k], k, KeypointCounts[k] / 2, LSA_TARGET_MAP, k));
     }
     for (bool& b : DevSpec) b = false;
+    bool searched = handover && HandoverSearched;
+    for (int k = 0; k < 3; ++k) searched = searched && !need[k];
+    HandoverSearched = searched;
     for (int k = 0; k < 3; ++k)
       if (need[k]) LSA_TRY(lsa_device_grid_build_submap_end(DevMaps[k]));
     Stats.submap += t.Stop();
@@ -1075,9 +1127,24 @@
     Stats.submap += t.Stop();
   }
 
+  if (handover)
+  {
+    handoverGuard.pending = false;
+    if (HandoverSearched && DeviceMapsInUse())
+    {
+      LSA_TRY(lsa_loc_handover_commit(Ctx));
+      LocStartsAhead++;
+    }
+    else
+    {
+      lsa_loc_handover_drop(Ctx);
+      HandoverSearched = false;
+    }
+  }
   const bool refined = Undistortion == UNDISTORTION_REFINED;
   IcpLoopSpec spec = {};
   spec.name = "loc";
+  spec.firstMatchEnqueued = handover && HandoverSearched;
   spec.target = LSA_TARGET_MAP;
   spec.set = LSA_SET_WORKING;
   for (int k = 0; k < 3; ++k)
@@ -1138,6 +1205,54 @@
   };
   if (const int rc = RunIcpLoop(spec, Tworld, top, kNothing, kNothing, skipped, accepted, finished); rc < 0) return rc;
   if (KeepMatchDebug) return DownloadMatchDebug(LSA_SET_WORKING, 7u, LocDebug);
+  return LSA_OK;
+}
+
+int SlamCore::StartLocalizationAhead()
+{
+  HandoverGaveUp = true;
+  Tick t;
+  struct AtExit { SlamCore* c; Tick* t; ~AtExit() { c->HandoverSeconds = t->Stop(); } } atExit{this, &t};
+  for (auto& w : MapWorker) w.Wait();
+  if (DevSpecStatus < 0) return LSA_OK;
+  for (int k = 0; k < 3; ++k)
+    if (MapJobFailed[k]) return LSA_OK;
+  unsigned mask = 0, spare = 0;
+  for (int k = 0; k < 3; ++k)
+  {
+    HandoverChecking[k] = false;
+    HandoverNeed[k] = UseKeypoints[k] && !lsa_device_grid_submap_valid(DevMaps[k]);
+    if (UseKeypoints[k]) mask |= 1u << k;
+    if (!HandoverNeed[k]) continue;
+    lsa_set_target_cell_size(Ctx, LSA_TARGET_MAP, k, static_cast<float>((k == LSA_EDGE ? KnnCellScaleMapsEdges : KnnCellScaleMaps) * LocalMaps[k]->GetLeafSize()));
+    if (!DevSpec[k] || lsa_device_grid_submap_ahead_ready(DevMaps[k], KeypointCounts[k] / 2, LSA_TARGET_MAP, k) != 1) return LSA_OK;
+    spare |= 1u << k;
+  }
+  Stats.submap += t.Stop();
+  Tick tu;
+  LSA_TRY(lsa_loc_handover_start(Ctx));
+  HandoverGaveUp = false;
+  HandoverStarted = true;
+  Stats.undistort += tu.Stop();
+  Tick ts;
+  bool compared = true;
+  for (int k = 0; k < 3; ++k)
+  {
+    if (!HandoverNeed[k]) continue;
+    const int rc = lsa_device_grid_submap_ahead_check_handover(DevMaps[k], k, KeypointCounts[k] / 2, LSA_TARGET_MAP, k);
+    if (rc < 0) return Fail(rc, "lsa_device_grid_submap_ahead_check_handover");
+    HandoverChecking[k] = rc == 1;
+    compared = compared && rc == 1;
+  }
+  Stats.submap += ts.Stop();
+  if (!compared) return LSA_OK;
+  Tick tm;
+  lsa_match_params_t mp = LocMatchParams();
+  mp.saturation_distance = (1 - 0.) * LocalizationInitSaturationDistance + 0. * LocalizationFinalSaturationDistance;
+  const int rc = lsa_match_types_handover(Ctx, LSA_TARGET_MAP, mask, spare, &mp);
+  if (rc < 0) return Fail(rc, "lsa_match_types_handover");
+  HandoverSearched = rc == 0;
+  Stats.loc_icp += tm.Stop();
   return LSA_OK;
 }
 
@@ -1750,6 +1865,7 @@
   X("MapsOnDevice", MapsOnDevice, bool)                                                                \
   X("SubMapsAhead", SubMapsAhead, bool)                                                                \
   X("SubMapsAheadAdaptive", SubMapsAheadAdaptive, bool)                                                \
+  X("LocalizationStartAhead", LocalizationStartAhead, int)                                             \
   X("LocalizationStartFused", LocalizationStartFused, bool)                                            \
   X("WorkerPrewake", WorkerPrewake, bool)                                                              \
   X("ICPAhead", ICPAhead, int)                                                                         \
@@ -1932,6 +2048,7 @@
   if (name == "UploadsAdopted") { *v = Ctx ? lsa_uploads_adopted(Ctx) : 0; return LSA_OK; }
   if (name == "DeviceSolveFallbacks") { *v = Ctx ? lsa_solve_device_fallbacks(Ctx) : 0; return LSA_OK; }
   if (name == "IcpGateTimeouts") { *v = IcpGateTimeouts; return LSA_OK; }
+  if (name == "LocStartsAhead") { *v = LocStartsAhead; return LSA_OK; }
   if (name == "TargetsBuiltAheadAdopted") { *v = Ctx ? lsa_prepared_targets_adopted(Ctx) : 0; return LSA_OK; }
   if (name == "SubMapsStagedAheadAdopted") { *v = Ctx ? lsa_staged_targets_adopted(Ctx) : 0; return LSA_OK; }
   if (name == "MapAddThreads") { *v = LocalMaps[LSA_PLANE]->GetAddThreads(); return LSA_OK; }
diff --git a/lidarslam_amd/csrc/host/lsa_slam_core.h b/lidarslam_amd/csrc/host/lsa_slam_core.h
--- a/lidarslam_amd/csrc/host/lsa_slam_core.h
+++ b/lidarslam_amd/csrc/host/lsa_slam_core.h
@@ -202,6 +202,15 @@
   unsigned TotalMatchedKeypoints = 0;
   unsigned NbrFrameProcessed = 0;
   unsigned SubMapSpecHitsTotal = 0;
+  int LocalizationStartAhead = 1;
+  unsigned LocStartsAhead = 0;
+  bool HandoverStarted = false;
+  bool HandoverSearched = false;
+  bool HandoverGaveUp = false;
+  bool HandoverNeed[3] = {false, false, false}, HandoverChecking[3] = {false, false, false};
+  double HandoverSeconds = 0.;
+  unsigned LoopChained = 0;
+  int StartLocalizationAhead();
   int KfCounter = 0;
   FrameStats Stats;
   std::deque<StampedPose> LogTrajectory;
diff --git a/lidarslam_amd/csrc/lsa_ctx.h b/lidarslam_amd/csrc/lsa_ctx.h
--- a/lidarslam_amd/csrc/lsa_ctx.h
+++ b/lidarslam_amd/csrc/lsa_ctx.h
@@ -35,6 +35,7 @@
 constexpr int kAccumVals = 29;
 constexpr int kGateRing = 8;
 constexpr int kGateWords = 64;
+constexpr int kHandoverBlock = kGateRing;
 constexpr int kGateGranules = 128;
 
 struct GridDesc
@@ -210,6 +211,16 @@
   unsigned gate_seq = 0;
   int gate_current = -1;
   struct GateSaved { double sat[3]; int hist_pos[3]; long long hist_serial[3]; int k[3]; bool valid[3]; unsigned mask; bool used; bool link; unsigned seq; } gate_saved[lsa::kGateRing] = {};
+  struct Handover
+  {
+    bool armed = false, started = false, searched = false;
+    lsa_loc_handover_t params = {};
+    unsigned mask = 0;
+    double sat[3] = {0, 0, 0};
+    int k[3] = {0, 0, 0}, knn_n[3] = {0, 0, 0}, knn_k[3] = {0, 0, 0}, hist_pos[3] = {0, 0, 0};
+    long long hist_serial[3] = {0, 0, 0};
+    int last_match_type = 0;
+  } handover;
   double* motion_dev = nullptr;
   int debug_gate_give_up_every = 0;
   int debug_lm_give_up_block = -1;
diff --git a/lidarslam_amd/csrc/lsa_ctx.hip b/lidarslam_amd/csrc/lsa_ctx.hip
--- a/lidarslam_amd/csrc/lsa_ctx.hip
+++ b/lidarslam_amd/csrc/lsa_ctx.hip
@@ -192,8 +192,8 @@
   if (ctx->lm_mailbox && hipHostMalloc((void**)&ctx->gate_host, (size_t)kGateRing * kGateGranules * sizeof(unsigned long long), hipHostMallocCoherent | hipHostMallocMapped) == hipSuccess)
   {
     std::memset(ctx->gate_host, 0, (size_t)kGateRing * kGateGranules * sizeof(unsigned long long));
-    if (hipMalloc((void**)&ctx->gate_dev, (size_t)kGateRing * kGateWords * sizeof(unsigned long long)) != hipSuccess ||
-        hipMemset(ctx->gate_dev, 0, (size_t)kGateRing * kGateWords * sizeof(unsigned long long)) != hipSuccess)
+    if (hipMalloc((void**)&ctx->gate_dev, (size_t)(kGateRing + 1) * kGateWords * sizeof(unsigned long long)) != hipSuccess ||
+        hipMemset(ctx->gate_dev, 0, (size_t)(kGateRing + 1) * kGateWords * sizeof(unsigned long long)) != hipSuccess)
     {
       (void)hipHostFree(ctx->gate_host);
       ctx->gate_host = nullptr;
diff --git a/lidarslam_amd/csrc/lsa_device_grid.hip b/lidarslam_amd/csrc/lsa_device_grid.hip
--- a/lidarslam_amd/csrc/lsa_device_grid.hip
+++ b/lidarslam_amd/csrc/lsa_device_grid.hip
@@ -924,14 +924,16 @@
   for (int d = 0; d < 3; ++d) { st[kStPred + d] = lo[d]; st[kStPred + 3 + d] = hi[d]; }
 }
 __global__ void k_box_check(const unsigned* __restrict__ words, int grid_size, float resolution, double resolution_d, int* __restrict__ st, u64* __restrict__ host_out,
-                            unsigned tag)
+                            unsigned tag, u64* __restrict__ go)
 {
   if (threadIdx.x != 0 || blockIdx.x != 0) return;
+  if (go && *go != 1ull && *go != 3ull) return;
   int lo[3], hi[3];
   box_voxels(words, grid_size, resolution, resolution_d, st, lo, hi);
   bool same = true;
   for (int d = 0; d < 3; ++d) same = same && lo[d] == st[kStPred + d] && hi[d] == st[kStPred + 3 + d];
   if (same) st[kStUpdated] = 0;
+  else if (go) *go = 3ull;
   __hip_atomic_store(host_out, ((u64)tag << 32) | (same ? 1u : 0u), __ATOMIC_RELAXED, __HIP_MEMORY_SCOPE_SYSTEM);
 }
 
@@ -1984,12 +1986,12 @@
   }
   return g->ahead_phase;
 }
-int lsa_device_grid_submap_ahead_take_begin(lsa_device_grid* g, int box_type, int min_nb_points, int slot, int type)
+static int take_begin(lsa_device_grid* g, int box_type, int min_nb_points, int slot, int type, bool handover, bool enqueue)
 {
   if (!g || box_type < 0 || box_type > 2 || slot < 0 || slot > 1 || type < 0 || type > 2)
     return g ? g->ctx->fail(LSA_E_ARG, "lsa_device_grid_submap_ahead_take: bad argument") : LSA_E_ARG;
   lsa_ctx* ctx = g->ctx;
-  g->take_pending = false;
+  if (enqueue) g->take_pending = false;
   if (g->ahead_phase == 1)
   {
     const int rc = lsa_device_grid_submap_ahead_poll(g);
@@ -1997,16 +1999,28 @@
   }
   const bool fits = g->ahead_phase == 2 && g->ahead_type == type && g->ahead_min == min_nb_points && g->sub_target < 0 &&
                     ctx->target[9 + type].cell_hint == ctx->target[slot * 3 + type].cell_hint;
-  g->ahead_phase = 0;
+  if (!enqueue) return fits ? 1 : 0;
+  if (!handover) g->ahead_phase = 0;
   if (!fits) return 0;
   G_HIP(hipSetDevice(ctx->device));
   G_HIP(hipStreamWaitEvent(ctx->stream, ctx->ev_map_ahead[type], 0));
   const unsigned tag = ++g->ahead_tag;
   const unsigned* words = lsa::current_box_words(ctx) + 6 * box_type;
-  hipLaunchKernelGGL(k_box_check, dim3(1), dim3(64), 0, ctx->stream, words, g->GridSize, (float)g->VoxelResolution, g->VoxelResolution, g->st, g->host_ahead + 1, tag);
+  hipLaunchKernelGGL(k_box_check, dim3(1), dim3(64), 0, ctx->stream, words, g->GridSize, (float)g->VoxelResolution, g->VoxelResolution, g->st, g->host_ahead + 1, tag,
+                     handover ? reinterpret_cast<u64*>(ctx->gate_dev + (size_t)kHandoverBlock * kGateWords) : nullptr);
   g->take_pending = true;
   g->take_slot = slot;
   return 1;
+}
+int lsa_device_grid_submap_ahead_take_begin(lsa_device_grid* g, int box_type, int min_nb_points, int slot, int type)
+{
+  return take_begin(g, box_type, min_nb_points, slot, type, false, true);
+}
+int lsa_device_grid_submap_ahead_ready(lsa_device_grid* g, int min_nb_points, int slot, int type) { return take_begin(g, 0, min_nb_points, slot, type, true, false); }
+int lsa_device_grid_submap_ahead_check_handover(lsa_device_grid* g, int box_type, int min_nb_points, int slot, int type)
+{
+  if (g && !g->ctx->gate_dev) return g->ctx->fail(LSA_E_STATE, "lsa_device_grid_submap_ahead_check_handover: no hand-over block");
+  return take_begin(g, box_type, min_nb_points, slot, type, true, true);
 }
 int lsa_device_grid_submap_ahead_take_end(lsa_device_grid* g, int* taken)
 {
@@ -2014,6 +2028,7 @@
   *taken = 0;
   if (!g->take_pending) return LSA_OK;
   g->take_pending = false;
+  g->ahead_phase = 0;
   lsa_ctx* ctx = g->ctx;
   const int type = g->ahead_type, slot = g->take_slot;
   const unsigned tag = g->ahead_tag;
diff --git a/lidarslam_amd/csrc/lsa_lm.hip b/lidarslam_amd/csrc/lsa_lm.hip
--- a/lidarslam_amd/csrc/lsa_lm.hip
+++ b/lidarslam_amd/csrc/lsa_lm.hip
@@ -34,6 +34,9 @@
   Rigid previous_world;
   double motion0[16];
   double* motion_dev;
+  IcpGate* handover;
+  int handover_undistort;
+  double handover_t0, handover_t1;
   lsa_sensor_terms_t sensors;
   int sensors_on;
 };
@@ -475,6 +478,52 @@
   for (int i = 0; i < 3; ++i) { o[10 + i] = m.Trans0[i]; o[13 + i] = m.Trans1[i]; }
 }
 
+__device__ void leave_handover(const LmParams& p, const LmState& lm, bool failed)
+{
+  using namespace posemath;
+  const bool next = !failed && !lm.skipped && lm.successful != 1;
+  if (p.leave && next) return;
+  IcpGate* g = p.handover;
+  const int lane = threadIdx.x & 63;
+  if (failed || lm.skipped)
+  {
+    if (lane == 0) g->go = 0ull;
+    return;
+  }
+  const double half = lm.x[3 + (lane < 6 ? lane % 3 : 0)] * 0.5;
+  const double v = lane < 3 ? lsa_cos(half) : lsa_sin(half);
+  const double cx = lane_value(v, 0), cy = lane_value(v, 1), cz = lane_value(v, 2);
+  const double sx = lane_value(v, 3), sy = lane_value(v, 4), sz = lane_value(v, 5);
+  double x[6];
+#pragma unroll
+  for (int a = 0; a < 6; ++a) x[a] = lm.x[a];
+  const Pose previous = FromRigid(p.previous_world);
+  const Pose T = previous * FromXYZRPYTrig(x, cx, sx, cy, sy, cz, sz);
+  if (!p.handover_undistort)
+  {
+    if (lane != 0) return;
+    g->in.pose = ToRigid(T);
+    g->go = 1ull;
+    return;
+  }
+  WithinFrameMotion m;
+  m.SetTimes(p.handover_t0, p.handover_t1);
+  m.SetTransforms(Pose::Identity(), Pose::Identity());
+  if (m.GetTimeRange() < 1e-6) m.SetTimes(0., 0.);
+  const Pose mine = InterpolateScanPose(p.clock, previous, T, lane == 1 ? m.Time1 : m.Time0);
+  Pose worldToBaseEnd = Pose::Identity();
+#pragma unroll
+  for (int i = 0; i < 3; ++i)
+#pragma unroll
+    for (int j = 0; j < 4; ++j) worldToBaseEnd(i, j) = lane_value(mine(i, j), 1);
+  if (lane != 0) return;
+  Pose d0, d1;
+  RefineUndistortionFrom(m, mine, worldToBaseEnd, T, d0, d1);
+  g->in.ic = MakeInterpConst(d0, d1, m.Time0, m.Time1);
+  g->in.pose = ToRigid(T);
+  g->go = 1ull;
+}
+
 __global__ __launch_bounds__(kLmThreads) void k_lm_solve(LmParams p, u64* __restrict__ xchg, u64* __restrict__ mailbox, unsigned out_tag, unsigned long long* trace)
 {
   __shared__ Shared sh;
@@ -555,6 +604,7 @@
     for (int i = 0; i < 4; ++i) trace[8 + i] += sh.sub[i];
   }
   if (p.leave && threadIdx.x >= 64 && threadIdx.x < 192) leave_link(p, sh.lm, failed, (threadIdx.x >> 6) - 1);
+  if (p.handover && threadIdx.x >= 192 && threadIdx.x < 256) leave_handover(p, sh.lm, failed);
   if (threadIdx.x < 2 * kResCount)
   {
     const LmState& lm = sh.lm;
@@ -660,7 +710,8 @@
 
 extern "C" {
 
-static int solve_device_begin(lsa_ctx* ctx, unsigned type_mask, const double prior[6], int two_d_mode, int lm_max_iter, int min_matches, int leave_ticket, const lsa_icp_link_t* link)
+static int solve_device_begin(lsa_ctx* ctx, unsigned type_mask, const double prior[6], int two_d_mode, int lm_max_iter, int min_matches, int leave_ticket, const lsa_icp_link_t* link,
+                              bool linked = false)
 {
   if (!ctx) return LSA_E_ARG;
   if (leave_ticket >= 0 && (leave_ticket >= kGateRing || !link || !ctx->gate_dev || !ctx->gate_saved[leave_ticket].used || !ctx->gate_saved[leave_ticket].link))
@@ -701,6 +752,23 @@
     p.clock.max_ratio = link->max_extrapolation_ratio;
     row_major_to_rt(link->previous_world, p.previous_world.R, p.previous_world.t);
     std::memcpy(p.motion0, link->motion, sizeof(p.motion0));
+  }
+  p.handover = nullptr;
+  p.handover_undistort = 0;
+  p.handover_t0 = p.handover_t1 = 0.;
+  if (linked && ctx->handover.armed && !ctx->handover.started)
+  {
+    if (link && link->refine_undistortion) return ctx->fail(LSA_E_STATE, "lsa_solve_device_begin_linked: a loop that refines its undistortion cannot leave a hand-over");
+    const lsa_loc_handover_t& h = ctx->handover.params;
+    p.handover = reinterpret_cast<IcpGate*>(ctx->gate_dev + (size_t)kHandoverBlock * kGateWords);
+    p.handover_undistort = h.undistort ? 1 : 0;
+    p.handover_t0 = h.t0;
+    p.handover_t1 = h.t1;
+    p.clock.have_log = h.have_log ? 1 : 0;
+    p.clock.prev_time = h.prev_time;
+    p.clock.cur_time = h.cur_time;
+    p.clock.max_ratio = h.max_extrapolation_ratio;
+    row_major_to_rt(h.previous_world, p.previous_world.R, p.previous_world.t);
   }
   p.sensors = ctx->sensor_terms;
   p.sensors_on = (ctx->sensor_terms.wheel || ctx->sensor_terms.gravity) ? 1 : 0;
@@ -735,7 +803,7 @@
 int lsa_solve_device_begin_linked(lsa_ctx* ctx, unsigned type_mask, const double prior[6], int two_d_mode, int lm_max_iter, int min_matches, int leave_ticket, const lsa_icp_link_t* link)
 {
   if (ctx && (int)ctx->lm_pending.size() >= kLmMailRing - 1) return ctx->fail(LSA_E_STATE, "lsa_solve_device_begin_linked: too many solves in flight");
-  return solve_device_begin(ctx, type_mask, prior, two_d_mode, lm_max_iter, min_matches, leave_ticket, link);
+  return solve_device_begin(ctx, type_mask, prior, two_d_mode, lm_max_iter, min_matches, leave_ticket, link, true);
 }
 
 int lsa_solve_device_drop(lsa_ctx* ctx)
@@ -976,6 +1044,23 @@
 int lsa_icp_abandon(lsa_ctx* ctx)
 {
   if (!ctx) return LSA_E_ARG;
+  (void)lsa_icp_abandon_loop(ctx);
+  return lsa_loc_handover_drop(ctx);
+}
+
+int lsa_loc_handover_arm(lsa_ctx* ctx, const lsa_loc_handover_t* h)
+{
+  if (!ctx || !h) return ctx ? ctx->fail(LSA_E_ARG, "lsa_loc_handover_arm: bad argument") : LSA_E_ARG;
+  if (!ctx->gate_dev || !ctx->motion_dev) return ctx->fail(LSA_E_STATE, "lsa_loc_handover_arm: no device memory for the links");
+  (void)lsa_loc_handover_drop(ctx);
+  ctx->handover.params = *h;
+  ctx->handover.armed = true;
+  return LSA_OK;
+}
+
+int lsa_icp_abandon_loop(lsa_ctx* ctx)
+{
+  if (!ctx) return LSA_E_ARG;
   while (true)
   {
     int youngest = -1;
diff --git a/lidarslam_amd/csrc/lsa_match.hip b/lidarslam_amd/csrc/lsa_match.hip
--- a/lidarslam_amd/csrc/lsa_match.hip
+++ b/lidarslam_amd/csrc/lsa_match.hip
@@ -66,7 +66,7 @@
   return LSA_OK;
 }
 
-static int match_prepare(lsa_ctx* ctx, int slot, int type, int query_set, const lsa_match_params_t* p, hipStream_t st, MatchPrep& out)
+static int match_prepare(lsa_ctx* ctx, int slot, int type, int query_set, const lsa_match_params_t* p, hipStream_t st, MatchPrep& out, bool spare = false)
 {
   const int nq = ctx->kp_n[query_set][type];
   MatchBuf& mb = ctx->match[type];
@@ -81,7 +81,7 @@
   mb.valid = true;
   ctx->last_match_type = type;
   if (nq == 0) return 0;
-  const int ti = slot * 3 + type;
+  const int ti = spare ? 9 + type : slot * 3 + type;
   Target& t = ctx->target[ti];
   if (t.m == 0)
   {
@@ -130,7 +130,7 @@
 }
 
 static int match_types_impl(lsa_ctx* ctx, int slot, unsigned type_mask, int query_set, const lsa_match_params_t* p, const double pose[16], int* histograms,
-                            const InterpConst* undistort, int gate = -1, bool gate_undistorts = false)
+                            const InterpConst* undistort, int gate = -1, bool gate_undistorts = false, unsigned spare_mask = 0u)
 {
   if (!ctx || !p || (!pose && gate < 0) || slot < 0 || slot > 1 || (type_mask & ~7u) || query_set < 0 || query_set > 2)
     return ctx ? ctx->fail(LSA_E_ARG, "lsa_match_types: bad argument") : LSA_E_ARG;
@@ -157,7 +157,7 @@
     int np = 0;
     for (int i = 0; i < nt; ++i)
     {
-      if (gate >= 0)
+      if (gate >= 0 && gate < kGateRing)
       {
         lsa_ctx::GateSaved& sv = ctx->gate_saved[gate];
         const int k = types[i];
@@ -165,7 +165,7 @@
         sv.sat[k] = ctx->match[k].sat; sv.k[k] = ctx->match[k].k; sv.valid[k] = ctx->match[k].valid;
         sv.hist_pos[k] = ctx->hist_pos[k]; sv.hist_serial[k] = ctx->hist_serial[k];
       }
-      const int rc = match_prepare(ctx, slot, types[i], query_set, p, ctx->stream, preps[np]);
+      const int rc = match_prepare(ctx, slot, types[i], query_set, p, ctx->stream, preps[np], (spare_mask >> types[i]) & 1u);
       if (rc < 0) return rc;
       if (rc > 0) ++np;
     }
@@ -246,6 +246,73 @@
   for (int k = 0; k < 3; ++k)
     if (((type_mask >> k) & 1u) && ctx->kp_n[query_set][k] > 0 && ctx->target[slot * 3 + k].m <= 0) return 1;
   return match_types_impl(ctx, slot, type_mask, query_set, p, nullptr, nullptr, nullptr, ctx->gate_current, undistort != 0);
+}
+
+int lsa_match_types_handover(lsa_ctx* ctx, int slot, unsigned type_mask, unsigned spare_mask, const lsa_match_params_t* p)
+{
+  if (!ctx || !p || slot < 0 || slot > 1 || (type_mask & ~7u) || (spare_mask & ~type_mask))
+    return ctx ? ctx->fail(LSA_E_ARG, "lsa_match_types_handover: bad argument") : LSA_E_ARG;
+  lsa_ctx::Handover& h = ctx->handover;
+  if (!h.started || h.searched) return ctx->fail(LSA_E_STATE, "lsa_match_types_handover: no localization started behind a hand-over (lsa_loc_handover_start)");
+  if (!ctx->fused_match || !ctx->fused_model) return 1;
+  for (int k = 0; k < 3; ++k)
+    if (((type_mask >> k) & 1u) && ctx->kp_n[LSA_SET_WORKING][k] > 0)
+    {
+      if (ctx->target[((spare_mask >> k) & 1u) ? 9 + k : slot * 3 + k].m <= 0) return 1;
+      if (type_params(*p, k).bad) return 1;
+    }
+  lsa_ctx::Handover before;
+  for (int k = 0; k < 3; ++k)
+  {
+    const MatchBuf& mb = ctx->match[k];
+    before.k[k] = mb.k; before.knn_n[k] = mb.knn_n; before.knn_k[k] = mb.knn_k; before.sat[k] = mb.sat;
+    before.hist_pos[k] = ctx->hist_pos[k]; before.hist_serial[k] = ctx->hist_serial[k];
+  }
+  bool valid_before[3] = {ctx->match[0].valid, ctx->match[1].valid, ctx->match[2].valid};
+  before.last_match_type = ctx->last_match_type;
+  const int rc = match_types_impl(ctx, slot, type_mask, LSA_SET_WORKING, p, nullptr, nullptr, nullptr, kHandoverBlock, false, spare_mask);
+  h.mask = type_mask;
+  h.last_match_type = ctx->last_match_type;
+  ctx->last_match_type = before.last_match_type;
+  for (int k = 0; k < 3; ++k)
+  {
+    MatchBuf& mb = ctx->match[k];
+    h.k[k] = mb.k; h.knn_n[k] = mb.knn_n; h.knn_k[k] = mb.knn_k; h.sat[k] = mb.sat;
+    h.hist_pos[k] = ctx->hist_pos[k]; h.hist_serial[k] = ctx->hist_serial[k];
+    mb.k = before.k[k]; mb.knn_n = before.knn_n[k]; mb.knn_k = before.knn_k[k]; mb.sat = before.sat[k]; mb.valid = valid_before[k];
+    ctx->hist_pos[k] = before.hist_pos[k]; ctx->hist_serial[k] = before.hist_serial[k];
+  }
+  if (rc) return rc;
+  h.searched = true;
+  return LSA_OK;
+}
+
+int lsa_loc_handover_commit(lsa_ctx* ctx)
+{
+  if (!ctx) return LSA_E_ARG;
+  lsa_ctx::Handover& h = ctx->handover;
+  if (!h.searched) return ctx->fail(LSA_E_STATE, "lsa_loc_handover_commit: no search enqueued behind the hand-over");
+  for (int k = 0; k < 3; ++k)
+  {
+    if (!((h.mask >> k) & 1u)) continue;
+    MatchBuf& mb = ctx->match[k];
+    mb.k = h.k[k]; mb.knn_n = h.knn_n[k]; mb.knn_k = h.knn_k[k]; mb.sat = h.sat[k]; mb.valid = true;
+    ctx->hist_pos[k] = h.hist_pos[k]; ctx->hist_serial[k] = h.hist_serial[k];
+  }
+  ctx->last_match_type = h.last_match_type;
+  h.armed = h.started = h.searched = false;
+  return LSA_OK;
+}
+
+int lsa_loc_handover_drop(lsa_ctx* ctx)
+{
+  if (!ctx) return LSA_E_ARG;
+  lsa_ctx::Handover& h = ctx->handover;
+  if (h.searched)
+    for (int k = 0; k < 3; ++k)
+      if ((h.mask >> k) & 1u) { ctx->hist_pos[k] = h.hist_pos[k]; ctx->hist_serial[k] = h.hist_serial[k]; }
+  h.armed = h.started = h.searched = false;
+  return LSA_OK;
 }
 
 int lsa_download_match(lsa_ctx* ctx, int type, uint8_t* status, double* weights, double* records, int capacity)
diff --git a/lidarslam_amd/csrc/lsa_transform.hip b/lidarslam_amd/csrc/lsa_transform.hip
--- a/lidarslam_amd/csrc/lsa_transform.hip
+++ b/lidarslam_amd/csrc/lsa_transform.hip
@@ -285,6 +285,69 @@
   }
 }
 
+__global__ __launch_bounds__(256) void k_loc_start_handover(StageOut s, int undistort, const IcpGate* __restrict__ block, unsigned* __restrict__ bits)
+{
+  __shared__ unsigned slo[4][3], shi[4][3];
+  __shared__ IcpInputs gin;
+  __shared__ unsigned long long go;
+  const int t = blockIdx.y;
+  const int n = s.n[t];
+  if ((int)(blockIdx.x * blockDim.x) >= n) return;
+  const int i = blockIdx.x * blockDim.x + threadIdx.x;
+  float4 a = {0.f, 0.f, 0.f, 0.f}, b = {0.f, 0.f, 0.f, 0.f};
+  if (i < n)
+  {
+    a = s.in[t][2 * (size_t)i];
+    b = s.in[t][2 * (size_t)i + 1];
+  }
+  {
+    constexpr int words = (int)(sizeof(IcpInputs) / 8);
+    static_assert(words + 1 <= 256 && offsetof(IcpGate, in) == 8, "one word per thread, go in front");
+    const unsigned long long* src = reinterpret_cast<const unsigned long long*>(block);
+    if ((int)threadIdx.x < words) reinterpret_cast<unsigned long long*>(&gin)[threadIdx.x] = src[1 + threadIdx.x];
+    else if ((int)threadIdx.x == words) go = src[0];
+  }
+  __syncthreads();
+  if (go != 1ull) return;
+  unsigned lo[3] = {~0u, ~0u, ~0u}, hi[3] = {0u, 0u, 0u};
+  if (i < n)
+  {
+    if (undistort)
+    {
+      Rigid U;
+      interp_eval(gin.ic, point_time(b), U);
+      double ox, oy, oz;
+      rigid_apply(U, (double)a.x, (double)a.y, (double)a.z, ox, oy, oz);
+      a.x = (float)ox; a.y = (float)oy; a.z = (float)oz;
+    }
+    s.out[t][2 * (size_t)i] = a;
+    s.out[t][2 * (size_t)i + 1] = b;
+    double ox, oy, oz;
+    rigid_apply(gin.pose, (double)a.x, (double)a.y, (double)a.z, ox, oy, oz);
+    const float v[3] = {(float)ox, (float)oy, (float)oz};
+    for (int d = 0; d < 3; ++d)
+      if (v[d] == v[d]) lo[d] = hi[d] = f2ou(v[d]);
+  }
+  for (int d = 0; d < 3; ++d)
+    for (int sft = 32; sft > 0; sft >>= 1)
+    {
+      const unsigned l2 = __shfl_down(lo[d], sft), h2 = __shfl_down(hi[d], sft);
+      lo[d] = l2 < lo[d] ? l2 : lo[d];
+      hi[d] = h2 > hi[d] ? h2 : hi[d];
+    }
+  if ((threadIdx.x & 63) == 0)
+    for (int d = 0; d < 3; ++d) { slo[threadIdx.x >> 6][d] = lo[d]; shi[threadIdx.x >> 6][d] = hi[d]; }
+  __syncthreads();
+  if (threadIdx.x < 3)
+  {
+    const int d = threadIdx.x;
+    unsigned l = slo[0][d], h = shi[0][d];
+    for (int w = 1; w < 4; ++w) { l = slo[w][d] < l ? slo[w][d] : l; h = shi[w][d] > h ? shi[w][d] : h; }
+    atomicMin(&bits[6 * t + d], l);
+    atomicMax(&bits[6 * t + 3 + d], h);
+  }
+}
+
 InterpConst make_interp(const double H0[16], const double H1[16], double t0, double t1)
 {
   posemath::Pose a, b;
@@ -415,6 +478,41 @@
   if (box_pose) row_major_to_rt(box_pose, T.R, T.t);
   ProfScope ps(ctx, "undistort", (double)total * (H0 ? 64 : 64));
   hipLaunchKernelGGL(k_loc_start, dim3((nmax + 255) / 256, 3), dim3(256), 0, ctx->stream, so, H0 ? 1 : 0, c, box_pose ? 1 : 0, T, lsa::loc_box_words(ctx));
+  return LSA_OK;
+}
+
+int lsa_loc_handover_start(lsa_ctx* ctx)
+{
+  if (!ctx) return LSA_E_ARG;
+  if (!ctx->handover.armed || !ctx->gate_dev) return ctx->fail(LSA_E_STATE, "lsa_loc_handover_start: no hand-over armed (lsa_loc_handover_arm)");
+  LSA_HIP(ctx, hipSetDevice(ctx->device));
+  StageOut so;
+  int nmax = 0, total = 0;
+  for (int k = 0; k < 3; ++k)
+  {
+    const int n = ctx->kp_n[LSA_SET_RAW_CURRENT][k];
+    ctx->kp_n[LSA_SET_WORKING][k] = n;
+    so.in[k] = reinterpret_cast<const float4*>(ctx->kp[LSA_SET_RAW_CURRENT][k]);
+    so.out[k] = reinterpret_cast<float4*>(ctx->kp[LSA_SET_WORKING][k]);
+    so.n[k] = n;
+    ctx->bbox_n[k] = n;
+    nmax = std::max(nmax, n);
+    total += std::max(n, 0);
+  }
+  ctx->kp_time_valid[LSA_SET_WORKING] = ctx->kp_time_valid[LSA_SET_RAW_CURRENT];
+  ctx->kp_time[LSA_SET_WORKING][0] = ctx->kp_time[LSA_SET_RAW_CURRENT][0];
+  ctx->kp_time[LSA_SET_WORKING][1] = ctx->kp_time[LSA_SET_RAW_CURRENT][1];
+  ctx->loc_boxes = true;
+  const int rc = lsa_arm_localization_boxes(ctx);
+  if (rc) return rc;
+  ctx->loc_armed = false;
+  ctx->bbox_pending = true;
+  ctx->bbox_copied = false;
+  ctx->handover.started = true;
+  if (nmax <= 0) return LSA_OK;
+  ProfScope ps(ctx, "undistort", (double)total * 64);
+  hipLaunchKernelGGL(k_loc_start_handover, dim3((nmax + 255) / 256, 3), dim3(256), 0, ctx->stream, so, ctx->handover.params.undistort ? 1 : 0,
+                     reinterpret_cast<const IcpGate*>(ctx->gate_dev + (size_t)kHandoverBlock * kGateWords), lsa::loc_box_words(ctx));
   return LSA_OK;
 }
 
```

Result: slower. 1333 frames/s (-4.4%).
